# tsnorri/founder-sequences

Hardware: AMD Instinct MI355X
Metric: alignment cells/s (m*n/T) through pBWT+DP (higher is better)
Workload: dtype u32

## Files before the change

### founder-sequences_amd/__init__.py

```python
import ctypes as C
import os

import numpy as np

_HERE = os.path.dirname(os.path.abspath(__file__))
LIB_PATH = os.path.join(_HERE, "libfseq_hip.so")

FSEQ_OK, FSEQ_E_ARG, FSEQ_E_NO_REDUCTION, FSEQ_E_HIP, FSEQ_E_OOM, FSEQ_E_UNSUPPORTED = range(6)


class FseqError(RuntimeError):
    def __init__(self, code, msg):
        super().__init__("fseq error %d: %s" % (code, msg))
        self.code = code


class NoReduction(FseqError):
    """generate_context.cc:192-200: max segment size equals the number of input sequences."""


class Params(C.Structure):
    _fields_ = [("m", C.c_uint32), ("n", C.c_uint64), ("segment_length", C.c_uint64),
                ("pbwt_sample_rate", C.c_uint64), ("block_len", C.c_uint32), ("list_cap", C.c_uint32),
                ("device", C.c_int32)]
# ... 103 lines not shown
                ("junctions_linked", C.c_uint64), ("junctions_novel", C.c_uint64), ("walks", C.c_uint64), ("rows_on_graph", C.c_uint64),
                ("mismatches", C.c_uint64), ("ms_device", C.c_double)]


class GraphNearestInfo(C.Structure):
    _fields_ = [("batches", C.c_uint64), ("packed_words", C.c_uint64), ("query_words", C.c_uint64), ("bits", C.c_uint32), ("reserved", C.c_uint32)]


class DpListsInfo(C.Structure):
    _fields_ = [("unproven", C.c_uint32), ("dp_chunks", C.c_uint32), ("dp_sweeps", C.c_uint32), ("launches", C.c_uint32)]


class MergeListsInfo(C.Structure):
    _fields_ = [("overflow", C.c_uint32), ("tau_separate", C.c_uint32), ("threshold_launches", C.c_uint32), ("count_launches", C.c_uint32)]


class LengthScanSummary(C.Structure):
    _fields_ = [("lists_built", C.c_uint32), ("lists_folded", C.c_uint32), ("short_entries", C.c_uint32), ("retries", C.c_uint32),
                ("ms_phase_a", C.c_double), ("ms_phase_b", C.c_double), ("ms_total", C.c_double)]


LENGTH_SCAN_DTYPE = np.dtype([("segment_length", "<u8"), ("max_segment_size", "<u4"), ("short_path", "<u4"), ("lists", "<u4"), ("list_cap", "<u4"),
                              ("dp_chunks", "<u4"), ("reserved", "<u4"), ("ms_device", "<f8")])
SCAN_LISTS_BUILT, SCAN_LISTS_FOLDED, SCAN_LISTS_NONE = 0, 1, 2

JOIN_SCORE_DTYPE = np.dtype([("rb", "<u8"), ("weight", "<u8"), ("supported", "<u4"), ("unsupported", "<u4"), ("gaps", "<u4"), ("rows_through", "<u4")])
JOIN_SCORE_MAX_SLOTS = 4096
JOIN_SCORE_GAP = 0xFFFF

GRAPH_NODE_DTYPE = np.dtype([("lb", "<u8"), ("rb", "<u8"), ("segment", "<u4"), ("cls", "<u4"), ("rep_row", "<u4"), ("rows", "<u4")])
GRAPH_EDGE_DTYPE = np.dtype([("from", "<u4"), ("to", "<u4"), ("rows", "<u4"), ("junction", "<u4")])
GRAPH_PATHS = 1
GRAPH_NONE = 0xFFFFFFFF
GRAPH_THREAD_ROW_DTYPE = np.dtype([("columns_matched", "<u8"), ("longest_walk_columns", "<u8"), ("segments_matched", "<u4"), ("junctions_linked", "<u4"),
                                   ("junctions_novel", "<u4"), ("walks", "<u4"), ("longest_walk_segments", "<u4"), ("reserved", "<u4")])
GRAPH_THREAD_SEGMENT_DTYPE = np.dtype([("matched", "<u4"), ("linked", "<u4"), ("novel", "<u4"), ("reserved", "<u4")])
GRAPH_THREAD_MAX_CLASSES = 4096
GRAPH_NEAREST_ROW_DTYPE = np.dtype([("columns_admitted", "<u8"), ("longest_walk_columns", "<u8"), ("mismatches_admitted", "<u8"), ("mismatches", "<u8"),
                                    ("segments_admitted", "<u4"), ("segments_exact", "<u4"), ("junctions_linked", "<u4"), ("junctions_novel", "<u4"),
                                    ("walks", "<u4"), ("longest_walk_segments", "<u4"), ("max_distance", "<u4"), ("reserved", "<u4")])
GRAPH_NEAREST_SEGMENT_DTYPE = np.dtype([("mismatches", "<u8"), ("admitted", "<u4"), ("exact", "<u4"), ("linked", "<u4"), ("novel", "<u4"),
                                        ("max_distance", "<u4"), ("reserved", "<u4")])
GRAPH_NEAREST_BATCH_BYTES = 256 << 20

MATCH_PIECE_DTYPE = np.dtype([("lb", "<u8"), ("rb", "<u8"), ("row", "<u4"), ("n_founders", "<u4")])
MATCH_MAX_FOUNDERS = 2048

SEGMENT_DTYPE = np.dtype([("lb", "<u8"), ("rb", "<u8"), ("segment_size", "<u4"), ("reserved", "<u4")])
DPARG_DTYPE = np.dtype([("lb", "<u8"), ("rb", "<u8"), ("segment_max_size", "<u4"), ("segment_size", "<u4")])

EXPORTS = [
    "fseq_abi_version", "fseq_strerror", "fseq_create", "fseq_destroy", "fseq_last_error",
    "fseq_set_rows", "fseq_set_matrix", "fseq_set_device_columns", "fseq_generate_synthetic", "fseq_get_matrix",
    "fseq_run_segmentation", "fseq_get_traceback", "fseq_get_segments", "fseq_boundary_state",
    "fseq_short_path_runs", "fseq_join_greedy", "fseq_greedy_match_host", "fseq_write_founders", "fseq_write_founders_device", "fseq_debug_dp", "fseq_debug_block_state", "fseq_debug_column_list", "fseq_get_timings",
    "fseq_rowshard_xbuf_words", "fseq_rowshard_rows", "fseq_rowshard_pbwt",
    "fseq_debug_rmq", "fseq_shard_xbuf_words", "fseq_set_shard", "fseq_shard_columns", "fseq_shard_owner",
    "fseq_set_device_columns_packed", "fseq_debug_dp_schedule", "fseq_run_segmentation_batch", "fseq_join_bipartite", "fseq_join_random", "fseq_bipartite_match_host", "fseq_random_join_host", "fseq_write_segments",
    "fseq_set_progress", "fseq_step_max", "fseq_current_step", "fseq_set_memory_budget", "fseq_write_segments_host", "fseq_get_join_profile", "fseq_debug_set_tuning",
    "fseq_shard_abort", "fseq_debug_dp_owned", "fseq_debug_clock", "fseq_debug_ranges",
    "fseq_set_list_memory", "fseq_debug_list_windows",
    "fseq_match_founders", "fseq_match_founder_rows", "fseq_get_match", "fseq_write_match",
    "fseq_identity_columns", "fseq_create_without_identity_columns", "fseq_get_identity_columns", "fseq_write_identity_columns", "fseq_write_founders_restored", "fseq_match_founders_restored",
    "fseq_input_begin", "fseq_input_chunk_columns", "fseq_input_scan", "fseq_input_columns", "fseq_input_end", "fseq_set_rows_streamed", "fseq_debug_device_bytes", "fseq_debug_packed_columns",
    "fseq_debug_join_path", "fseq_debug_pass2_paths", "fseq_debug_class_columns", "fseq_debug_bipartite_path",
    "fseq_debug_pass2_step", "fseq_debug_chain_launch", "fseq_debug_chain_launch_wg", "fseq_debug_red_plan", "fseq_debug_column_sources", "fseq_debug_red_cls_direct",
    "fseq_write_segments_device", "fseq_random_join_classes_host", "fseq_debug_segments_file", "fseq_debug_random_path",
    "fseq_set_segment_length", "fseq_scan_segment_lengths", "fseq_debug_scan_plan", "fseq_debug_relump_lists",
    "fseq_match_rows", "fseq_debug_match_split",
    "fseq_create_without_rows", "fseq_get_held_out", "fseq_match_held_out", "fseq_debug_held_out_columns", "fseq_debug_row_split_plan",
    "fseq_debug_dp_lists_check", "fseq_debug_dp_on_lists", "fseq_debug_merge_on_lists", "fseq_debug_traceback_parts",
    "fseq_create_without_identity_columns_held", "fseq_match_held_out_restored", "fseq_match_rows_restored", "fseq_get_match_exceptions",
    "fseq_get_segments_restored", "fseq_write_segments_restored", "fseq_debug_restored_bounds",
    "fseq_input_scan_identity", "fseq_input_reduce", "fseq_input_kept_columns", "fseq_input_columns_kept", "fseq_input_end_kept",
    "fseq_set_rows_streamed_without_identity_columns", "fseq_debug_input_kept_range", "fseq_debug_alphabet",
    "fseq_join_score", "fseq_join_score_host", "fseq_debug_join_score_path", "fseq_debug_join_score",
    "fseq_block_graph", "fseq_write_block_graph", "fseq_debug_graph_file",
    "fseq_debug_local_pass",
    "fseq_graph_thread_rows", "fseq_graph_thread_held_out", "fseq_debug_graph_thread",
    "fseq_graph_nearest_rows", "fseq_graph_nearest_held_out", "fseq_debug_graph_nearest_info", "fseq_debug_graph_nearest_plan", "fseq_debug_graph_nearest",
    "fseq_write_block_graph_restored", "fseq_graph_thread_rows_restored", "fseq_graph_thread_held_out_restored",
    "fseq_debug_chain_launch_wg_keys", "fseq_debug_pass2_step_keys",
    "fseq_debug_chain_plan", "fseq_debug_chain_plan_sharded", "fseq_debug_phase_b",
]
DEBUG_EXPORTS = ["fseq_debug_dp", "fseq_debug_dp_owned", "fseq_debug_clock", "fseq_debug_ranges", "fseq_debug_block_state", "fseq_debug_column_list", "fseq_debug_rmq", "fseq_debug_dp_schedule", "fseq_debug_set_tuning",
                 "fseq_debug_list_windows", "fseq_debug_device_bytes", "fseq_debug_packed_columns", "fseq_debug_join_path", "fseq_debug_pass2_paths",
                 "fseq_debug_class_columns", "fseq_debug_bipartite_path", "fseq_debug_pass2_step", "fseq_debug_chain_launch", "fseq_debug_chain_launch_wg", "fseq_debug_red_plan", "fseq_debug_column_sources", "fseq_debug_red_cls_direct",
                 "fseq_debug_segments_file", "fseq_debug_random_path", "fseq_debug_scan_plan", "fseq_debug_relump_lists", "fseq_debug_match_split",
                 "fseq_debug_held_out_columns", "fseq_debug_row_split_plan", "fseq_debug_dp_lists_check", "fseq_debug_dp_on_lists",
                 "fseq_debug_merge_on_lists", "fseq_debug_traceback_parts",
                 "fseq_debug_restored_bounds", "fseq_debug_input_kept_range", "fseq_debug_alphabet",
                 "fseq_debug_join_score_path", "fseq_debug_join_score", "fseq_debug_graph_file", "fseq_debug_local_pass",
                 "fseq_debug_graph_thread", "fseq_debug_graph_nearest_info", "fseq_debug_graph_nearest_plan", "fseq_debug_graph_nearest",
                 "fseq_debug_chain_launch_wg_keys", "fseq_debug_pass2_step_keys",
                 "fseq_debug_chain_plan", "fseq_debug_chain_plan_sharded", "fseq_debug_phase_b"]

FSEQ_E_PEER = 6
P2_RUN_CAP = 8832
CW_RUN_CAP = 16384
STAGE_TRACEBACK, STAGE_MERGE, STAGE_SAMPLES = 0, 1, 2
PROGRESS_FN = C.CFUNCTYPE(None, C.c_void_p, C.c_int, C.c_uint64, C.c_uint64)

JOIN_GREEDY, JOIN_BIPARTITE, JOIN_RANDOM = 0, 1, 2

ALLREDUCE_FN = C.CFUNCTYPE(C.c_int, C.c_void_p, C.c_uint64, C.c_uint64, C.c_int)

_lib = None


def load_library():
    global _lib
    if _lib is not None:
        return _lib
    if not os.path.exists(LIB_PATH):
        raise ImportError("%s is missing: run `python __graft_entry__.py build` (hipcc --offload-arch=gfx950); "
                          "there is no CPU fallback for the segmentation path" % LIB_PATH)
    L = C.CDLL(LIB_PATH)
    vp, u64, sz = C.c_void_p, C.c_uint64, C.c_size_t
    L.fseq_abi_version.restype = C.c_uint32
    L.fseq_strerror.restype = C.c_char_p
    L.fseq_strerror.argtypes = [C.c_int]
    L.fseq_create.argtypes = [C.POINTER(Params), C.POINTER(vp)]
    L.fseq_destroy.argtypes = [vp]
    L.fseq_destroy.restype = None
    L.fseq_last_error.restype = C.c_char_p
    L.fseq_last_error.argtypes = [vp]
    L.fseq_set_rows.argtypes = [vp, C.POINTER(vp)]
    L.fseq_set_matrix.argtypes = [vp, vp, sz, sz]
    L.fseq_set_device_columns.argtypes = [vp, vp, sz, C.c_uint32]
    L.fseq_set_device_columns_packed.argtypes = [vp, vp, sz, C.c_uint32, C.c_uint32]
    L.fseq_generate_synthetic.argtypes = [vp, C.POINTER(SynthSpec)]
    L.fseq_get_matrix.argtypes = [vp, u64, u64, vp, sz, sz]
    L.fseq_run_segmentation.argtypes = [vp, C.POINTER(Result)]
    L.fseq_get_traceback.argtypes = [vp, vp]
    L.fseq_get_segments.argtypes = [vp, vp]
    L.fseq_boundary_state.argtypes = [vp, u64, vp, vp]
    L.fseq_short_path_runs.argtypes = [vp, vp, vp]
    L.fseq_join_greedy.argtypes = [vp, vp]
    L.fseq_greedy_match_host.argtypes = [C.c_uint32, C.c_uint32, u64, vp, vp, vp, vp, vp]
    L.fseq_write_founders.argtypes = [vp, C.POINTER(vp), vp, C.c_char_p]
    L.fseq_write_founders_device.argtypes = [vp, vp, C.c_char_p]
    L.fseq_run_segmentation_batch.argtypes = [vp, sz, vp, vp]
    L.fseq_debug_dp_schedule.argtypes = [u64, u64, u64, vp, vp, vp, vp]
    L.fseq_join_bipartite.argtypes = [vp, vp]
    L.fseq_join_random.argtypes = [vp, C.c_uint32, vp]
    L.fseq_bipartite_match_host.argtypes = [C.c_uint32, C.c_uint32, u64, vp, vp, vp, vp, vp, vp]
    L.fseq_random_join_host.argtypes = [C.c_uint32, C.c_uint32, u64, vp, vp, vp, vp, C.c_uint32, vp]
    L.fseq_write_segments.argtypes = [vp, C.POINTER(vp), C.c_int, C.c_char_p]
    L.fseq_debug_dp.argtypes = [vp, vp, vp, vp]
    L.fseq_debug_block_state.argtypes = [vp, u64, vp, vp]
    L.fseq_debug_column_list.argtypes = [vp, u64, vp, vp, vp, vp, vp]
    L.fseq_get_timings.argtypes = [vp, C.POINTER(Timings)]
    L.fseq_debug_rmq.argtypes = [C.c_int, vp, C.c_uint32, vp, vp, C.c_uint32, vp, vp]
    L.fseq_shard_xbuf_words.restype = u64
    L.fseq_shard_xbuf_words.argtypes = [vp, C.c_uint32]
    L.fseq_set_shard.argtypes = [vp, C.c_uint32, C.c_uint32, vp, u64, ALLREDUCE_FN, vp]
    L.fseq_shard_columns.argtypes = [vp, C.POINTER(u64), C.POINTER(u64)]
    L.fseq_shard_owner.argtypes = [vp, u64, C.POINTER(C.c_uint32)]
    L.fseq_rowshard_xbuf_words.restype = u64
    L.fseq_rowshard_xbuf_words.argtypes = [C.c_uint32, C.c_uint32, C.c_uint32]
    L.fseq_rowshard_rows.argtypes = [C.c_uint32, C.c_uint32, C.c_uint32, C.c_uint32, C.POINTER(C.c_uint32), C.POINTER(C.c_uint32)]
    L.fseq_rowshard_pbwt.argtypes = [vp, vp, vp, C.POINTER(C.c_uint32), C.POINTER(C.c_uint32), C.POINTER(C.c_double), C.POINTER(u64)]
    L.fseq_write_segments_host.argtypes = [vp, C.POINTER(vp), C.c_int, vp, vp, C.c_char_p]
    L.fseq_get_join_profile.argtypes = [vp, C.POINTER(JoinProfile)]
    L.fseq_debug_set_tuning.argtypes = [vp, C.c_char_p, C.c_char_p]
    L.fseq_set_progress.argtypes = [vp, PROGRESS_FN, vp]
    L.fseq_step_max.restype = u64
    L.fseq_step_max.argtypes = [vp]
    L.fseq_current_step.restype = u64
    L.fseq_current_step.argtypes = [vp]
    L.fseq_set_memory_budget.argtypes = [vp, u64]
    L.fseq_set_list_memory.argtypes = [vp, u64]
    L.fseq_debug_list_windows.argtypes = [vp, C.POINTER(u64), C.POINTER(u64), C.POINTER(C.c_uint32), C.POINTER(C.c_uint32)]
    L.fseq_shard_abort.argtypes = [vp, C.c_int]
    L.fseq_debug_dp_owned.argtypes = [vp, C.POINTER(u64), C.POINTER(u64), C.POINTER(C.c_int), C.POINTER(C.c_int)]
    L.fseq_debug_clock.argtypes = [vp, C.POINTER(C.c_double), C.POINTER(C.c_uint32)]
    L.fseq_debug_ranges.argtypes = [C.POINTER(u64), C.POINTER(u64), C.POINTER(C.c_int)]
    L.fseq_match_founders.argtypes = [vp, vp, u64, C.POINTER(MatchSummary)]
    L.fseq_match_founder_rows.argtypes = [vp, C.POINTER(vp), C.c_uint32, u64, C.POINTER(MatchSummary)]
    L.fseq_get_match.argtypes = [vp, vp, vp]
    L.fseq_write_match.argtypes = [vp, C.c_char_p]
    L.fseq_match_rows.argtypes = [vp, vp, C.POINTER(vp), C.c_uint32, C.POINTER(vp), C.c_uint32, u64, C.POINTER(MatchSummary)]
    L.fseq_debug_match_split.argtypes = [vp, C.POINTER(MatchSplitInfo)]
    L.fseq_identity_columns.argtypes = [vp, vp, C.POINTER(IdentitySummary)]
    L.fseq_create_without_identity_columns.argtypes = [vp, C.POINTER(Params), C.POINTER(vp), C.POINTER(IdentitySummary)]
    L.fseq_get_identity_columns.argtypes = [vp, vp, vp]
    L.fseq_write_identity_columns.argtypes = [vp, C.c_char_p]
    L.fseq_write_founders_restored.argtypes = [vp, vp, C.c_char_p]
    L.fseq_match_founders_restored.argtypes = [vp, vp, u64, C.POINTER(MatchSummary)]
    L.fseq_input_begin.argtypes = [vp, vp, C.c_uint32, u64]
    L.fseq_input_chunk_columns.restype = u64
    L.fseq_input_chunk_columns.argtypes = [vp]
    L.fseq_input_scan.argtypes = [vp, u64, u64, C.POINTER(vp)]
    L.fseq_input_columns.argtypes = [vp, u64, u64, C.POINTER(vp)]
    L.fseq_input_end.argtypes = [vp]
    L.fseq_set_rows_streamed.argtypes = [vp, C.POINTER(vp), u64]
    L.fseq_debug_device_bytes.argtypes = [vp, C.POINTER(u64), C.POINTER(u64), C.c_int]
    L.fseq_debug_packed_columns.argtypes = [vp, u64, u64, vp, C.POINTER(u64), C.POINTER(C.c_uint32)]
    L.fseq_debug_join_path.argtypes = [vp, C.POINTER(C.c_int)]
    L.fseq_debug_bipartite_path.argtypes = [vp, C.POINTER(C.c_int)]
    L.fseq_debug_pass2_paths.argtypes = [vp] + [C.POINTER(C.c_uint32)] * 4 + [vp]
    L.fseq_debug_class_columns.argtypes = [vp, C.POINTER(C.c_uint32), C.POINTER(C.c_uint32), C.c_uint32, C.POINTER(C.c_uint32), C.POINTER(C.c_uint32), C.POINTER(u64), vp, u64]
    L.fseq_debug_column_sources.argtypes = [vp, C.POINTER(C.c_uint32), C.POINTER(C.c_uint32), C.c_uint32, C.POINTER(C.c_uint32)]
    L.fseq_debug_red_cls_direct.argtypes = [C.c_uint32, C.c_uint32, C.c_uint32, u64, C.c_uint32, C.c_uint32, C.c_uint32, C.POINTER(u64), C.POINTER(u64), C.POINTER(C.c_int)]
    L.fseq_debug_pass2_step.argtypes = [C.c_int, C.c_uint32, C.c_uint32, vp, vp, vp, C.c_uint32, C.c_uint32, vp, vp, vp, vp, C.c_uint32, C.c_uint32, vp, vp, vp]
    L.fseq_debug_chain_launch.argtypes = [C.c_int, C.c_uint32, C.c_uint32, C.c_uint32, u64, vp, vp, vp, C.c_uint32, C.c_uint32, vp, vp, vp, vp, vp, vp, vp]
    L.fseq_debug_chain_launch_wg.argtypes = [C.c_int, C.c_uint32, C.c_uint32, C.c_uint32, u64, vp, vp, vp, C.c_uint32, C.c_uint32, vp, vp, C.c_uint32, C.c_uint32, vp, vp, vp, vp, vp, vp]
    L.fseq_debug_chain_launch_wg_keys.argtypes = L.fseq_debug_chain_launch_wg.argtypes + [vp, vp]
    L.fseq_debug_pass2_step_keys.argtypes = [C.c_int, C.c_uint32, C.c_uint32, vp, vp, vp, C.c_uint32, C.c_uint32, vp, vp, vp, vp, C.c_uint32, C.c_uint32, vp, vp, vp, vp, vp, vp]
    L.fseq_debug_red_plan.argtypes = [C.c_uint32, C.c_uint32, C.c_uint32, C.c_int, C.c_uint32, C.c_uint32, C.c_uint32, vp, vp, C.c_int, C.c_int] + [vp] * 11
    L.fseq_write_segments_device.argtypes = [vp, C.c_int, C.c_char_p]
    L.fseq_random_join_classes_host.argtypes = [C.c_uint32, C.c_uint32, u64, vp, vp, vp, C.c_uint32, vp]
    L.fseq_debug_segments_file.argtypes = [vp] + [C.POINTER(u64)] * 4
    L.fseq_debug_random_path.argtypes = [vp, C.POINTER(C.c_int)]
    L.fseq_set_segment_length.argtypes = [vp, u64]
    L.fseq_scan_segment_lengths.argtypes = [vp, vp, sz, C.POINTER(LengthScanSummary)]
    L.fseq_debug_scan_plan.argtypes = [u64, vp, C.c_uint32, vp, C.POINTER(C.c_uint32), vp, C.POINTER(C.c_uint32)]
    L.fseq_debug_relump_lists.argtypes = [C.c_int, u64, C.c_uint32, C.c_uint32, u64, u64, vp, vp]
    L.fseq_create_without_rows.argtypes = [vp, vp, C.c_uint32, C.POINTER(Params), C.POINTER(vp), C.POINTER(HoldOutSummary)]
    L.fseq_get_held_out.argtypes = [vp, vp, vp]
    L.fseq_match_held_out.argtypes = [vp, vp, C.POINTER(vp), C.c_uint32, u64, C.POINTER(MatchSummary)]
    L.fseq_create_without_identity_columns_held.argtypes = [vp, C.POINTER(Params), C.POINTER(vp), C.POINTER(IdentitySummary)]
    L.fseq_match_held_out_restored.argtypes = [vp, vp, u64, C.POINTER(MatchSummary)]
    L.fseq_match_rows_restored.argtypes = [vp, vp, C.POINTER(vp), C.c_uint32, u64, C.POINTER(MatchSummary)]
    L.fseq_get_match_exceptions.argtypes = [vp, vp, vp, C.POINTER(u64)]
    L.fseq_debug_held_out_columns.argtypes = [vp, u64, u64, vp, C.POINTER(u64), C.POINTER(C.c_uint32)]
    L.fseq_debug_row_split_plan.argtypes = [C.c_uint32, C.c_uint32, vp, C.c_uint32, vp, vp, vp, C.POINTER(C.c_uint32), C.POINTER(C.c_uint32)]
    L.fseq_debug_dp_lists_check.argtypes = [C.c_uint32, u64, u64, C.c_uint32, vp, vp, C.POINTER(u64), C.POINTER(C.c_uint32)]
    L.fseq_debug_dp_on_lists.argtypes = [vp, C.c_uint32, vp, vp, vp, C.c_uint32, vp, vp, vp, C.POINTER(DpListsInfo)]
    L.fseq_debug_merge_on_lists.argtypes = [vp, C.c_uint32, vp, vp, vp, vp, vp, C.c_uint32, vp, C.c_uint32, vp, C.POINTER(u64), vp, C.POINTER(u64), vp,
                                            C.POINTER(u64), C.POINTER(MergeListsInfo)]
    L.fseq_debug_traceback_parts.argtypes = [C.c_int, u64, u64, vp, vp, vp, vp, C.c_uint32, vp, vp, C.POINTER(u64), vp, vp, C.POINTER(u64)]
    L.fseq_debug_local_pass.argtypes = [C.c_int, C.c_uint32, C.c_uint32, vp, vp, vp, vp]
    L.fseq_get_segments_restored.argtypes = [vp, vp]
    L.fseq_write_segments_restored.argtypes = [vp, C.c_int, C.c_char_p]
    L.fseq_debug_restored_bounds.argtypes = [vp, u64, u64, vp, vp, u64, vp, vp]
    L.fseq_input_scan_identity.argtypes = [vp, u64, u64, C.POINTER(vp)]
    L.fseq_input_reduce.argtypes = [vp, C.POINTER(Params), C.POINTER(IdentitySummary)]
    L.fseq_input_kept_columns.argtypes = [vp, u64, u64, C.POINTER(u64)]
    L.fseq_input_columns_kept.argtypes = [vp, u64, u64, C.POINTER(vp)]
    L.fseq_input_end_kept.argtypes = [vp, C.POINTER(vp)]
    L.fseq_set_rows_streamed_without_identity_columns.argtypes = [vp, C.POINTER(vp), u64, C.POINTER(Params), C.POINTER(vp), C.POINTER(IdentitySummary)]
    L.fseq_debug_alphabet.argtypes = [vp, C.POINTER(C.c_uint32), C.POINTER(C.c_uint32), vp]
    L.fseq_debug_input_kept_range.argtypes = [vp, u64, u64, u64, C.POINTER(u64), C.POINTER(u64)]
    L.fseq_join_score.argtypes = [vp, vp, vp, vp, vp, C.POINTER(JoinScoreSummary)]
    L.fseq_join_score_host.argtypes = [C.c_uint32, C.c_uint32, u64, vp, vp, vp, vp, vp, vp, vp, vp, C.POINTER(JoinScoreSummary)]
    L.fseq_debug_join_score_path.argtypes = [vp, C.POINTER(C.c_int)]
    L.fseq_debug_join_score.argtypes = [C.c_int, C.c_uint32, C.c_uint32, C.c_uint32, vp, vp, vp, vp, vp, vp, C.POINTER(JoinScoreSummary)]
    L.fseq_block_graph.argtypes = [vp, vp, vp, vp, C.POINTER(GraphSummary)]
    L.fseq_write_block_graph.argtypes = [vp, C.c_uint32, C.c_int, C.c_char_p]
    L.fseq_debug_graph_file.argtypes = [vp, C.POINTER(GraphFileStats)]
    L.fseq_graph_thread_rows.argtypes = [vp, C.POINTER(vp), C.c_uint32, vp, vp, vp, vp, C.POINTER(GraphThreadSummary)]
    L.fseq_graph_thread_held_out.argtypes = [vp, vp, vp, vp, vp, C.POINTER(GraphThreadSummary)]
    L.fseq_debug_graph_thread.argtypes = [vp, C.POINTER(GraphThreadInfo)]
    L.fseq_graph_nearest_rows.argtypes = [vp, C.POINTER(vp), C.c_uint32, C.c_uint32, vp, vp, vp, vp, vp, vp, C.POINTER(GraphNearestSummary)]
    L.fseq_graph_nearest_held_out.argtypes = [vp, C.c_uint32, vp, vp, vp, vp, vp, vp, C.POINTER(GraphNearestSummary)]
    L.fseq_debug_graph_nearest_info.argtypes = [vp, C.POINTER(GraphNearestInfo)]
    L.fseq_debug_graph_nearest_plan.argtypes = [vp, vp, vp, u64, C.c_uint32, u64, vp, vp, C.POINTER(u64)]
    L.fseq_debug_graph_nearest.argtypes = [C.c_int, vp, u64, C.c_uint32, u64, C.c_uint32, vp, vp, vp, vp, C.c_uint32, C.c_uint32, vp, u64, C.c_uint32,
                                           C.c_uint32, C.c_uint32, u64, vp, vp, vp, C.POINTER(GraphNearestInfo)]
    L.fseq_debug_chain_plan.argtypes = [C.c_uint32, C.c_int, C.c_uint32, C.c_uint32, C.c_int, C.c_uint32, u64, C.c_uint32, C.POINTER(ChainPlan)]
    L.fseq_debug_chain_plan_sharded.argtypes = [C.c_uint32, C.c_uint32, C.c_uint32, C.c_uint32, C.c_int, C.c_uint32, C.c_int, u64, C.c_uint32, C.POINTER(ChainPlan)]
    L.fseq_debug_phase_b.argtypes = [vp, C.POINTER(PhaseBInfo)]
    L.fseq_write_block_graph_restored.argtypes = [vp, C.c_uint32, C.c_int, C.c_char_p]
    L.fseq_graph_thread_rows_restored.argtypes = [vp, C.POINTER(vp), C.c_uint32, vp, vp, vp, vp, C.POINTER(GraphThreadSummary)]
    L.fseq_graph_thread_held_out_restored.argtypes = [vp, vp, vp, vp, vp, C.POINTER(GraphThreadSummary)]
    _lib = L
    return L


def synth_threshold(mu):
    if mu <= 0.0:
        return 0
    if mu >= 1.0:
        return 0xFFFFFFFFFFFFFFFF
    return int(mu * 18446744073709551616.0)


def greedy_match_host(m, max_segment_size, lb, rb, a, d):
    L = load_library()
    lb = np.ascontiguousarray(lb, dtype=np.uint64)
    rb = np.ascontiguousarray(rb, dtype=np.uint64)
    a = np.ascontiguousarray(a, dtype=np.uint32)
    d = np.ascontiguousarray(d, dtype=np.uint32)
# ... 1188 lines not shown
        f, w = C.c_int(), C.c_int()
        self._check(self.L.fseq_debug_dp_owned(self.h, C.byref(a), C.byref(b), C.byref(f), C.byref(w)))
        return a.value, b.value, bool(f.value), bool(w.value)

    def debug_clock(self):
        g, n = C.c_double(), C.c_uint32()
        self._check(self.L.fseq_debug_clock(self.h, C.byref(g), C.byref(n)))
        return g.value, n.value

    def debug_block_state(self, b):
        a = np.zeros(self.m, dtype=np.uint32)
        d = np.zeros(self.m, dtype=np.uint32)
        self._check(self.L.fseq_debug_block_state(self.h, b, a.ctypes.data, d.ctypes.data))
        return a, d

    def debug_column_list(self, col):
        cap = self.m + 2
        v = np.zeros(cap, dtype=np.uint32)
        c = np.zeros(cap, dtype=np.uint32)
        ne, c0, comp = C.c_uint32(), C.c_uint32(), C.c_uint32()
        self._check(self.L.fseq_debug_column_list(self.h, col, v.ctypes.data, c.ctypes.data,
                                                  C.byref(ne), C.byref(c0), C.byref(comp)))
        return v[:ne.value].copy(), c[:ne.value].copy(), c0.value, bool(comp.value)

    def debug_dp_on_lists(self, list_cap, ent, hdr, cuts=()):
        ent, hdr = _dp_lists(ent, hdr)
        if ent.shape[0] != self.n or ent.shape[1] != ((int(list_cap) + 3) & ~1):
            raise FseqError(FSEQ_E_ARG, "DP on lists: ent is [n][(list_cap + 3) & ~1][2]")
        cuts = np.ascontiguousarray(cuts, dtype=np.uint32)
        k = self.n - self.segment_length + 1
        lb, mx, sz = (np.zeros(k, dtype=np.uint32) for _ in range(3))
        info = DpListsInfo()
        self.result = None
        self._check(self.L.fseq_debug_dp_on_lists(self.h, int(list_cap), ent.ctypes.data, hdr.ctypes.data, cuts.ctypes.data if len(cuts) else None,
                                                  len(cuts), lb.ctypes.data, mx.ctypes.data, sz.ctypes.data, C.byref(info)))
        return lb, mx, sz, {k_: getattr(info, k_) for k_, _ in DpListsInfo._fields_}

    def debug_merge_on_lists(self, list_cap, ent, hdr, lb, max_size, size, separate=False, col_splits=()):
        ent, hdr = _dp_lists(ent, hdr)
        if ent.shape[0] != self.n or ent.shape[1] != ((int(list_cap) + 3) & ~1):
            raise FseqError(FSEQ_E_ARG, "merge on lists: ent is [n][(list_cap + 3) & ~1][2]")
        lb, max_size, size = _dp_arrays(self.n, self.segment_length, lb, max_size, size)
        splits = np.ascontiguousarray(col_splits, dtype=np.uint64)
        room = self.n // self.segment_length + 2
        tb = np.zeros(room, dtype=DPARG_DTYPE)
        tau = np.zeros((room, 2), dtype=np.uint32)
        seg = np.zeros(room, dtype=SEGMENT_DTYPE)
        n_tb, n_tau, n_seg = C.c_uint64(), C.c_uint64(), C.c_uint64()
        info = MergeListsInfo()
        self.result = None
        self._check(self.L.fseq_debug_merge_on_lists(self.h, int(list_cap), ent.ctypes.data, hdr.ctypes.data, lb.ctypes.data, max_size.ctypes.data,
                                                     size.ctypes.data, 1 if separate else 0, splits.ctypes.data if len(splits) else None, len(splits),
                                                     tb.ctypes.data, C.byref(n_tb), tau.ctypes.data, C.byref(n_tau), seg.ctypes.data, C.byref(n_seg),
                                                     C.byref(info)))
        return (tb[:n_tb.value].copy(), tau[:n_tau.value].copy(), seg[:n_seg.value].copy(),
                {k_: getattr(info, k_) for k_, _ in MergeListsInfo._fields_})

    def set_tuning(self, name, value="1"):
        self._check(self.L.fseq_debug_set_tuning(self.h, name.encode(), None if value is None else str(value).encode()))

    def join_profile(self):
        jp = JoinProfile()
        self._check(self.L.fseq_get_join_profile(self.h, C.byref(jp)))
        return {k: getattr(jp, k) for k, _ in JoinProfile._fields_}

    def join_path(self):
        path = C.c_int()
        self._check(self.L.fseq_debug_join_path(self.h, C.byref(path)))
        return path.value

    def bipartite_path(self):
        path = C.c_int()
        self._check(self.L.fseq_debug_bipartite_path(self.h, C.byref(path)))
        return path.value

    def pass2_paths(self):
        v = [C.c_uint32() for _ in range(4)]
        hist = np.zeros(19, dtype=np.uint32)
        self._check(self.L.fseq_debug_pass2_paths(self.h, *[C.byref(x) for x in v], hist.ctypes.data))
        out = dict(zip(("by_runs", "by_sort", "copies", "max_runs"), (x.value for x in v)))
        out["runs_hist"] = [int(x) for x in hist]
        return out

    def phase_b(self):
        info = PhaseBInfo()
        self._check(self.L.fseq_debug_phase_b(self.h, C.byref(info)))
        out = {f: int(getattr(info, f)) for f in ("cus", "nblocks", "fan", "resident", "fit", "p2_groups", "p2_groups_took_keys", "p2_groups_gathered")}
        out["hand_armed"], out["stats_kept"] = bool(info.hand_armed), bool(info.stats_kept)
        out["launches"] = _chain_launches(info.launches, info.n_launches)
        s = [int(x) for x in info.cw_stats]
        out["cw_stats"] = dict(by_runs=s[0], by_sort=s[1], from_identity=s[2], max_runs=s[3], runs_hist=s[4:]) if info.stats_kept else None
        return out

    def class_column_sources(self):
        a, b = C.c_uint32(), C.c_uint32()
        self._check(self.L.fseq_debug_class_columns(self.h, C.byref(a), C.byref(b), 0xFFFFFFFF, None, None, None, None, 0))
        return {"from_classes": a.value, "from_alignment": b.value}

    def column_sources(self, block=None):
        a, b, s = C.c_uint32(), C.c_uint32(), C.c_uint32()
        self._check(self.L.fseq_debug_column_sources(self.h, C.byref(a), C.byref(b), 0xFFFFFFFF if block is None else block, C.byref(s)))
        out = {"staged": a.value, "gathered": b.value}
        if block is not None:
            out["block_staged"] = bool(s.value)
        return out

    def class_columns(self, block):
        have, nkeys, ldc = C.c_uint32(), C.c_uint32(), C.c_uint64()
        self._check(self.L.fseq_debug_class_columns(self.h, None, None, block, C.byref(have), C.byref(nkeys), C.byref(ldc), None, 0))
        if not have.value:
            return None, ldc.value, nkeys.value
        t = self.timings()
        cols = min(t["block_len"], self.n - block * t["block_len"])
        out = np.zeros((cols, ldc.value), dtype=np.uint8)
        self._check(self.L.fseq_debug_class_columns(self.h, None, None, block, C.byref(have), C.byref(nkeys), C.byref(ldc), out.ctypes.data, out.nbytes))
        return out, ldc.value, nkeys.value

    def timings(self):
        t = Timings()
        self._check(self.L.fseq_get_timings(self.h, C.byref(t)))
        return {k: getattr(t, k) for k, _ in Timings._fields_}
```

### founder-sequences_amd/csrc/fseq_ctx.hpp

```cpp
#pragma once

#include "../../include/fseq.h"
#include "../../include/fseq_debug.h"
#include "fseq_types.hpp"
#include "fseq_chainplan.hpp"

#include <hip/hip_runtime.h>

#include <algorithm>
#include <array>
#include <atomic>
#include <chrono>
#include <climits>
#include <cmath>
#include <cstdio>
#include <cstring>
#include <string>
#include <thread>
#include <unordered_map>
#include <vector>

namespace fseq {

struct KernelSet {
	uint32_t T, E, sigma, cap;
	size_t lds_colblock, lds_snap;
	uint32_t scan_shift;
	void (*rank)(hipStream_t st, uint32_t grid, size_t lds, PhaseAArgs const &keys);
	void (*snap)(hipStream_t st, uint32_t grid, size_t lds, SnapArgs const &tasks);
	size_t (*columns_lds)(uint32_t B);
	void (*columns)(hipStream_t st, uint32_t grid, size_t lds, ColumnsArgs const &cols);
	uint32_t (*columns_resident)(size_t lds);
	size_t lds_chain;
	void (*chain)(hipStream_t st, uint32_t grid, size_t lds, ChainMultiArgs const &chains, uint32_t keyed);
	hipError_t (*prepare)();
	hipError_t (*prepare_columns)(size_t lds_columns);
};

template <typename K>
inline hipError_t allow_lds(K kernel, size_t bytes)
{
	if (bytes <= 64 * 1024) return hipSuccess;
	return hipFuncSetAttribute(reinterpret_cast<void const *>(kernel), hipFuncAttributeMaxDynamicSharedMemorySize, (int) bytes);
}

struct Stream2Config { uint32_t T, E, key_shift; size_t (*lds)(uint32_t colbytes); hipError_t (*prepare)(size_t lds);
	void (*launch)(hipStream_t st, uint32_t grid, size_t lds, ColumnsArgs const &cols);
	uint32_t (*resident)(size_t lds);
	void (*launch_snap)(hipStream_t st, uint32_t grid, size_t lds, SnapArgs const &tasks); };
struct ReducedSet {
	uint32_t T, E, rows, values;
	bool pk, ew;
	size_t (*lds)(uint32_t B, uint32_t symcap);
	hipError_t (*prepare)(size_t lds);
	void (*launch)(hipStream_t st, uint32_t grid, size_t lds, ColumnsArgs const &cols, RedArgs const &red);
	uint32_t (*resident)(size_t lds);
};
int reduced_config_count();
bool reduced_config(int index, ReducedSet *out);
struct ChainSnapSet {
	size_t lds;
	hipError_t (*prepare)();
	void (*launch)(hipStream_t st, uint32_t grid, size_t lds, SnapArgs const &tasks, RedArgs const &red);
};
bool select_chain_snap(uint32_t T, uint32_t E, ChainSnapSet *out);

bool select_kernels(uint32_t m, uint32_t sigma, KernelSet *out);
Stream2Config stream2_config();
void launch_blockkeys(hipStream_t st, uint32_t grid, size_t lds, PhaseAArgs const &keys);
hipError_t prepare_blockkeys(uint32_t T, size_t lds, bool debug);
uint32_t blocktrie_threads(uint32_t m, bool stream);
size_t blocktrie_lds(uint32_t T);
hipError_t launch_blocktrie(hipStream_t st, uint32_t groups, PhaseAArgs const &keys);
hipError_t launch_reduce_prep(hipStream_t, uint32_t grid, RedPrepArgs const &);
void launch_reduce_check(hipStream_t, uint32_t const *cnt, uint32_t const *planned, uint32_t count, uint32_t *flags);
void launch_reduce_msa(hipStream_t st, MsaArgs const &A, ReducedMsaArgs const &red, bool gather_only);
bool launch_reduce_cls(hipStream_t st, MsaArgs const &A, ReducedMsaArgs const &red, ClassColumnArgs const &classes);

inline double now_ms()
{
	using namespace std::chrono;
	return duration<double, std::milli>(steady_clock::now().time_since_epoch()).count();
}


}

struct Tuning {
	bool debug = false;
	bool dp_serial = false;
	int  dp_spec_win = 0, dp_spec_rounds = 0, dp_spec_max_sweeps = 0;
	bool stream_plain_scan = false;
	bool plain_scan = false;
	bool occurrence_keys = false;
	bool phase_a_classic = false;
	int  chain_fan = 0;
	bool blockkeys_wide = false;
	bool blockkeys_single = false;
	bool no_dense_columns = false;
	bool no_blocktrie = false;
	bool blocktrie_always = false;
	int  blockkeys_cap = 0;
	bool ss_unpacked = false;
	bool ss_absolute = false;
	bool poison_lists = false;
	bool join_host = false;
	bool join_wide = false;
	bool join_bip_wide = false;
	int  join_bip_slabs = 0;
	int  segfile_batch = 0;
	int  graph_batch = 0;
	bool shard_dp_full = false;
	int  shard_dp_window = 0;
	int  inject_failure_rank = -1;
	std::string sync_phases;
	bool check_phase_a = false;
	bool no_reduced = false;
	int  reduced_margin = -1;
	bool reduced_always = false;
	bool reduced_msa_gather = false;
	int  reduced_cap = 0;
	bool class_gather = false;
	int  class_columns = 1;
	int  p2_run_cap = -1;
	int  chain_run_cap = -1;
	int  p2_keys = 0;
	int  chain_wg = 0;
	bool scan_rebuild = false;
	int  match_split = 0;
	int  match_overlap = 0;
	int  match_stage = 0;
	int  graph_thread_key_bits = 0;
	int  graph_nearest_batch = 0;

	struct Knob {
		char const *name;
		bool Tuning::*flag;
		int Tuning::*num;
		int lo, off;
		std::string Tuning::*str;
	};
	static std::vector<Knob> const &knobs()
	{
		static std::vector<Knob> const table = {
			{"FSEQ_DEBUG", &Tuning::debug, nullptr, 0, 0, nullptr},
			{"FSEQ_DP_SERIAL", &Tuning::dp_serial, nullptr, 0, 0, nullptr},
			{"FSEQ_DP_SPEC_WIN", nullptr, &Tuning::dp_spec_win, 1, 0, nullptr},
			{"FSEQ_DP_SPEC_ROUNDS", nullptr, &Tuning::dp_spec_rounds, 1, 0, nullptr},
			{"FSEQ_DP_SPEC_MAX_SWEEPS", nullptr, &Tuning::dp_spec_max_sweeps, 1, 0, nullptr},
			{"FSEQ_STREAM_PLAIN_SCAN", &Tuning::stream_plain_scan, nullptr, 0, 0, nullptr},
			{"FSEQ_PLAIN_SCAN", &Tuning::plain_scan, nullptr, 0, 0, nullptr},
			{"FSEQ_OCCURRENCE_KEYS", &Tuning::occurrence_keys, nullptr, 0, 0, nullptr},
			{"FSEQ_PHASE_A_CLASSIC", &Tuning::phase_a_classic, nullptr, 0, 0, nullptr},
			{"FSEQ_CHAIN_FAN", nullptr, &Tuning::chain_fan, 2, 0, nullptr},
			{"FSEQ_BLOCKKEYS_WIDE", &Tuning::blockkeys_wide, nullptr, 0, 0, nullptr},
			{"FSEQ_BLOCKKEYS_SINGLE", &Tuning::blockkeys_single, nullptr, 0, 0, nullptr},
			{"FSEQ_NO_DENSE_COLUMNS", &Tuning::no_dense_columns, nullptr, 0, 0, nullptr},
			{"FSEQ_NO_BLOCKTRIE", &Tuning::no_blocktrie, nullptr, 0, 0, nullptr},
			{"FSEQ_BLOCKTRIE_ALWAYS", &Tuning::blocktrie_always, nullptr, 0, 0, nullptr},
			{"FSEQ_BLOCKKEYS_CAP", nullptr, &Tuning::blockkeys_cap, 2048, 0, nullptr},
			{"FSEQ_SS_UNPACKED", &Tuning::ss_unpacked, nullptr, 0, 0, nullptr},
			{"FSEQ_SS_ABSOLUTE", &Tuning::ss_absolute, nullptr, 0, 0, nullptr},
			{"FSEQ_POISON_LISTS", &Tuning::poison_lists, nullptr, 0, 0, nullptr},
			{"FSEQ_JOIN_HOST", &Tuning::join_host, nullptr, 0, 0, nullptr},
			{"FSEQ_JOIN_WIDE", &Tuning::join_wide, nullptr, 0, 0, nullptr},
			{"FSEQ_JOIN_BIP_WIDE", &Tuning::join_bip_wide, nullptr, 0, 0, nullptr},
			{"FSEQ_JOIN_BIP_SLABS", nullptr, &Tuning::join_bip_slabs, 1, 0, nullptr},
			{"FSEQ_SEGFILE_BATCH", nullptr, &Tuning::segfile_batch, 1, 0, nullptr},
			{"FSEQ_GRAPH_BATCH", nullptr, &Tuning::graph_batch, 1, 0, nullptr},
			{"FSEQ_SHARD_DP_FULL", &Tuning::shard_dp_full, nullptr, 0, 0, nullptr},
			{"FSEQ_SHARD_DP_WINDOW", nullptr, &Tuning::shard_dp_window, 64, 0, nullptr},
			{"FSEQ_INJECT_FAILURE_RANK", nullptr, &Tuning::inject_failure_rank, INT_MIN, -1, nullptr},
			{"FSEQ_SYNC_PHASES", nullptr, nullptr, 0, 0, &Tuning::sync_phases},
			{"FSEQ_CHECK_PHASE_A", &Tuning::check_phase_a, nullptr, 0, 0, nullptr},
			{"FSEQ_NO_REDUCED", &Tuning::no_reduced, nullptr, 0, 0, nullptr},
			{"FSEQ_REDUCED_MARGIN", nullptr, &Tuning::reduced_margin, 0, -1, nullptr},
			{"FSEQ_REDUCED_ALWAYS", &Tuning::reduced_always, nullptr, 0, 0, nullptr},
			{"FSEQ_REDUCED_MSA_GATHER", &Tuning::reduced_msa_gather, nullptr, 0, 0, nullptr},
			{"FSEQ_REDUCED_CAP", nullptr, &Tuning::reduced_cap, 1, 0, nullptr},
			{"FSEQ_P2_RUN_CAP", nullptr, &Tuning::p2_run_cap, 0, -1, nullptr},
			{"FSEQ_CHAIN_RUN_CAP", nullptr, &Tuning::chain_run_cap, 0, -1, nullptr},
			{"FSEQ_CHAIN_WG", nullptr, &Tuning::chain_wg, 0, 0, nullptr},
			{"FSEQ_P2_KEYS", nullptr, &Tuning::p2_keys, 0, 0, nullptr},
			{"FSEQ_CLASS_COLUMNS", nullptr, &Tuning::class_columns, 0, 1, nullptr},
			{"FSEQ_CLASS_GATHER", &Tuning::class_gather, nullptr, 0, 0, nullptr},
			{"FSEQ_SCAN_REBUILD", &Tuning::scan_rebuild, nullptr, 0, 0, nullptr},
			{"FSEQ_MATCH_SPLIT", nullptr, &Tuning::match_split, 1, 0, nullptr},
			{"FSEQ_MATCH_OVERLAP", nullptr, &Tuning::match_overlap, 1, 0, nullptr},
			{"FSEQ_MATCH_STAGE_BYTES", nullptr, &Tuning::match_stage, 64, 0, nullptr},
			{"FSEQ_GRAPH_THREAD_KEY_BITS", nullptr, &Tuning::graph_thread_key_bits, 1, 0, nullptr},
			{"FSEQ_GRAPH_NEAREST_BATCH", nullptr, &Tuning::graph_nearest_batch, 1, 0, nullptr},
		};
		return table;
	}

	void apply(Knob const &k, char const *value)
	{
		bool const on = value != nullptr;
		if (k.flag) this->*k.flag = on;
		else if (k.num) this->*k.num = on ? std::max(k.lo, atoi(value)) : k.off;
		else this->*k.str = on ? value : "";
	}

	bool set(char const *name, char const *value)
	{
		for (Knob const &k : knobs())
			if (!strcmp(k.name, name)) { apply(k, value); return true; }
		return false;
	}

	void from_environment()
	{
		for (Knob const &k : knobs())
			if (char const *v = getenv(k.name)) apply(k, v);
	}
};

struct fseq_ctx;

namespace fseq {

template <typename T>
struct DevBuf {
	T *base = nullptr;
	size_t cap = 0;
	ptrdiff_t shift = 0;
	operator T *() const { return base ? reinterpret_cast<T *>(reinterpret_cast<char *>(base) - shift) : nullptr; }
	template <typename U> U *as() const { return reinterpret_cast<U *>(static_cast<T *>(*this)); }
	void rebase(ptrdiff_t elements) { shift = elements * (ptrdiff_t) sizeof(T); }
	int alloc(fseq_ctx *c, size_t count);
	bool try_alloc(fseq_ctx *c, size_t count);
	int ensure(fseq_ctx *c, size_t count) { return cap >= count ? FSEQ_OK : alloc(c, count); }
	int alloc_range(fseq_ctx *c, size_t lo, size_t hi, size_t per)
	{
		int const rc = alloc(c, (hi > lo ? hi - lo : 0) * per);
		rebase((ptrdiff_t) (lo * per));
		return rc;
	}
	void release(fseq_ctx *c);
};

template <typename T>
struct DevTemp : DevBuf<T> {
	fseq_ctx *const c;
	explicit DevTemp(fseq_ctx *c_) : c(c_) {}
	DevTemp(DevTemp const &) = delete;
	~DevTemp() { this->release(c); }
	int alloc(size_t count) { return DevBuf<T>::alloc(c, count); }
};

template <typename... B>
inline void release_all(fseq_ctx *c, B &...bufs) { (bufs.release(c), ...); }

}

struct Shard {
	bool on = false;
	uint32_t rank = 0, world = 1;
	uint32_t *xbuf = nullptr;
	uint64_t xwords = 0;
	fseq_allreduce_fn fn = nullptr;
	void *user = nullptr;
// ... 83 lines not shown
	DevBuf<uint32_t> d_bstate_a, d_bstate_d;
	DevBuf<uint32_t> d_cshist;
	int dev_cus = -1;
	int cw_resident = 0;
	DevBuf<uint16_t> d_p2keys;
	DevBuf<uint32_t> d_p2keys_flag;
	bool p2keys_live = false;
	uint32_t p2_hand[2]{};
	DevBuf<uint32_t> d_cw_stats;
	std::vector<fseq::ChainLaunch> pb_launches;
	uint32_t pb_cw_stats[fseq::CW_STATS]{};
	bool pb_cw_stats_have = false;
	bool pb_hand = false;
	uint64_t pb_fit = 0;
	uint32_t p2_groups = 0;
	DevBuf<uint32_t> d_hrank, d_hkeyd, d_hnkeys, d_hstate_a, d_hstate_d;
	struct ChainLevel { uint32_t count = 0; uint64_t cols = 0; DevBuf<uint32_t> rank, keyd, nkeys, state_a, state_d; };
	std::vector<ChainLevel> levels;
	uint32_t chain_fan = 0;
	uint32_t shard_k = 0, shard_q = 0;
	uint32_t chain_G = 0, n_super = 0;
	uint32_t chain_G2 = 0, n_hyper = 0;
	DevBuf<uint2> d_ent;
	DevBuf<uint4> d_hdr;
	uint32_t X = 0, stride = 0;
	uint32_t X_hint = 0;
	struct Dp {
		DevBuf<uint32_t> M, LB, SZ, Tb, Tbv;
		DevBuf<unsigned long long> K;
		uint32_t tstride = 0;
		operator fseq::DpArrays() const { return fseq::DpArrays{M, LB, SZ, Tb, Tbv, K, tstride}; }
	} dp;
	DevBuf<uint32_t> d_Mprev;
	DevBuf<uint32_t> d_spec;
	DevBuf<fseq::PathWords> d_flags;
	DevBuf<uint32_t> d_recent;
	uint64_t dp_size = 0;
	DevBuf<uint64_t> d_cols;
	DevBuf<uint2> d_grp;
	DevBuf<uint64_t> d_src;
	uint32_t snap_stride = 16;
	DevBuf<uint32_t> d_ss_a, d_ss_d;
	uint32_t ss_pack = 0;
	bool ss_ids = false;
	DevBuf<uint32_t> d_bs_w;
	DevBuf<uint8_t> d_bs_h;
	DevBuf<uint32_t> d_wgblk;
	DevBuf<uint2> d_wggrp;
	DevBuf<uint32_t> d_snap_a, d_snap_d;

	DevBuf<uint32_t> d_red_cnt, d_red_vmin, d_red_rows, d_red_leaf, d_red_a, d_red_d;
	DevBuf<uint32_t> d_red_invalid, d_red_blocks;
	uint32_t red_cap = 0;
	DevBuf<uint8_t> d_red_msa;
	size_t red_ld = 0;
	DevBuf<uint8_t> d_cls;
	DevBuf<uint32_t> d_cls_have;
	size_t cls_ld = 0;
	bool cls_on = false;
	bool cls_every = false;
	bool cls_read = false;
	DevBuf<uint32_t> d_red_src;
	bool cls_staged = false;
	struct Red {
		fseq::RedPlan plan;
		std::vector<uint8_t> cls_config;
		struct Memory {
			std::vector<uint8_t> force;
			bool plan_holds = false;
			uint32_t plan_X = 0;
			bool declined = false;
			uint32_t declined_X = 0;
			bool cls_unread = false;
			void forget_plan() { plan_holds = false; }
			void forget_verdicts() { plan_holds = false; declined = false; cls_unread = false; }
			void forget_input() { forget_verdicts(); force.clear(); }
		} memory;
	} red;
	bool red_active = false;
	DevBuf<uint32_t> d_red_cls, d_red_headd, d_red_ncls, d_red_taskblk, d_red_wgtasks;
	DevBuf<uint32_t> d_red_p2grp;
	uint32_t p2_stats[fseq::P2_STATS]{};
	bool p2_stats_have = false;
	DevBuf<uint32_t> d_red_ss_a, d_red_ss_d;
	uint32_t red_ss_stride = 0, red_ss_cap = 0;
	uint32_t *h_red_pin = nullptr;
	size_t red_pin_words = 0;
	bool red_direct = false;
	DevBuf<uint32_t> d_red_cnt_plan;
	hipStream_t red_st[2]{};
	struct RedEvents {
		hipEvent_t fork = nullptr;
		hipEvent_t join_stream2 = nullptr, join_side0 = nullptr, join_side1 = nullptr;
		std::array<hipEvent_t *, 3> joins() { return {&join_stream2, &join_side0, &join_side1}; }
		std::array<hipEvent_t *, 4> all() { return {&fork, &join_stream2, &join_side0, &join_side1}; }
	} red_ev;
	uint8_t *h_red_pin2 = nullptr;
	size_t red_pin2_bytes = 0;

	bool have_result = false;
	bool scan_lists = false;
	fseq_result res{};
	DevBuf<uint4> d_tb;
	std::vector<fseq_dp_arg> traceback;
	std::vector<fseq_segment> segments;
	std::vector<uint32_t> sp_first, sp_len;
	fseq_timings tm{};
	struct PathEvents {
		hipEvent_t a_begin = nullptr, a_end_b_begin = nullptr, b_end = nullptr;
		hipEvent_t c_begin = nullptr, c_end = nullptr, dp_begin = nullptr, dp_end = nullptr;
		hipEvent_t pass2_begin = nullptr, pass2_end = nullptr;
		hipEvent_t dp_reset = nullptr;
		std::array<hipEvent_t *, 9> timed() { return {&a_begin, &a_end_b_begin, &b_end, &c_begin, &c_end, &dp_begin, &dp_end, &pass2_begin, &pass2_end}; }
	} ev;
	hipStream_t stream2 = nullptr;
	uint8_t *h_pin = nullptr;
	size_t pin_cap = 0, pin_used = 0;

	struct Match {
		DevBuf<uint8_t> fcols;
		DevBuf<uint32_t> cnt;
		DevBuf<uint64_t> off;
		DevBuf<fseq_match_piece> pieces;
		DevBuf<uint32_t> sets;
		DevBuf<uint8_t> qrows;
		DevBuf<uint32_t> split;
		DevBuf<uint64_t> exc_off;
		DevBuf<uint32_t> exc_cols;
		uint64_t exc_total = 0;
		int exc_from = 0;
		uint32_t exc_rows = 0;
		bool have = false;
		fseq_match_summary sum{};
		fseq_match_split_info split_info{};
		hipEvent_t ev[4]{};
	} match;
	void free_match()
	{
		fseq::release_all(this, match.fcols, match.cnt, match.off, match.pieces, match.sets, match.qrows, match.split, match.exc_off, match.exc_cols);
		for (auto &e : match.ev) if (e) { (void) hipEventDestroy(e); e = nullptr; }
		match.have = false;
		match.exc_from = 0;
	}

	struct Identity {
		bool have = false;
		uint64_t n_src = 0, identity = 0;
		DevBuf<uint8_t> mask;
		DevBuf<uint32_t> kept;
		DevBuf<uint8_t> ref;
	} idn;
	void free_identity()
	{
		fseq::release_all(this, idn.mask, idn.kept, idn.ref);
		idn.have = false;
	}

	struct HeldOut {
		bool have = false;
		uint32_t m_src = 0, n_held = 0;
		size_t ld = 0;
		DevBuf<uint8_t> cols;
		std::vector<uint32_t> kept_rows, held_rows;
		bool have_exc = false;
		DevBuf<uint64_t> exc_off;
		DevBuf<uint32_t> exc_cols;
		uint64_t exc_total = 0;
// ... 144 lines not shown
```

### founder-sequences_amd/csrc/fseq_kernels.hpp

```cpp
#pragma once

#include "fseq_core.hpp"
#include "fseq_types.hpp"

#include <type_traits>

namespace fseq {

constexpr uint32_t PAD_KEY = 0xFFFFFFFFu;

struct Carver {
	char *p;
	template <typename U> __device__ __host__ U *take(size_t n)
	{
		U *r = reinterpret_cast<U *>(p);
		p += (n * sizeof(U) + 15) & ~size_t(15);
		return r;
	}
};

__host__ __device__ inline size_t carve_bytes(size_t n, size_t elem) { return (n * elem + 15) & ~size_t(15); }

struct SynthArgs {
	uint64_t seed;
// ... 537 lines not shown
		uint32_t total;
		uint32_t r = block_excl_add<T>(nf, sscr, &total);
		size_t const ob = (size_t) grp * m;
#pragma unroll
		for (int e = 0; e < E; ++e)
		{
			uint32_t const pos = p0 + e;
			if (pos < m)
			{
				bool const first = (pos == 0 || d[e] > kstart);
				r += first ? 1u : 0u;
				out_rank[ob + a[e]] = r - 1u;
				if (first) out_keyd[ob + r - 1u] = d[e];
			}
		}
		if (tid == 0) out_nkeys[grp] = total;
	}
}

#ifndef FSEQ_PW_MAX_E
#define FSEQ_PW_MAX_E 8
#endif
__host__ __device__ constexpr bool columns_pairwise(int T, int E, int SIGMA, bool PK = false)
{
	if (PK && T == 512 && E == 15) return false;
	return SIGMA == 4 && ((E >= 2 && E <= FSEQ_PW_MAX_E && !(T >= 1024 && E >= 7 && !PK)) || (PK && E >= 9 && T * E <= 10240));
}

__host__ __device__ constexpr bool columns_packed(int T, int E, int SIGMA, bool PK)
{
	if (!PK && T >= 1024 && E == 7) return false;
	return SIGMA == 4 && !columns_pairwise(T, E, SIGMA, PK);
}

__host__ __device__ constexpr bool columns_lookup(int T, int E, int SIGMA, bool PK) { return columns_pairwise(T, E, SIGMA, PK) || (SIGMA == 4 && PK && T * E <= 10240); }
__host__ __device__ constexpr size_t columns_run_words(int T, int E, int SIGMA, bool PK) { return (columns_pairwise(T, E, SIGMA, PK) || (PK && T == 512 && E == 15)) ? 5 * (size_t) T : columns_lookup(T, E, SIGMA, PK) ? 4 * (size_t) T : 0; }

constexpr int SLIM_T = 512, SLIM_E = 15, SLIM_VALUES = 4096;
__host__ __device__ constexpr bool columns_slim(int T, int E, bool PK) { return PK && T == SLIM_T && E == SLIM_E; }
__host__ __device__ constexpr size_t columns_value_cap(int T, int E, bool PK) { return columns_slim(T, E, PK) ? (size_t) SLIM_VALUES : (size_t) T * E; }
__host__ __device__ constexpr int columns_min_waves(int T, int E, bool PK) { return columns_slim(T, E, PK) ? 4 : (PK && T == 512) ? 6 : 4; }

template <int T, int E, int SIGMA, bool PK>
__host__ __device__ inline size_t columns_lds_bytes(uint32_t B)
{
	constexpr size_t CAP = (size_t) T * E, VCAP = columns_value_cap(T, E, PK);
	return 2 * carve_bytes(CAP, PK ? 2 : 4) + 2 * carve_bytes(CAP, 1) + carve_bytes(PK ? (VCAP + B + 9) / 2 : VCAP + B + 8, 4) + carve_bytes(VCAP, 4)
	     + carve_bytes(1, sizeof(StepScratch<T, SIGMA>)) + carve_bytes(T / WAVE + 1, 4) + (columns_run_words(T, E, SIGMA, PK) ? carve_bytes(columns_run_words(T, E, SIGMA, PK), 4) : 0);
}

template <bool PK> __device__ __forceinline__ uint32_t cnt_get(uint32_t const *cnt_l, uint32_t i)
{
	return PK ? ((cnt_l[i >> 1] >> ((i & 1u) * 16u)) & 0xFFFFu) : cnt_l[i];
}
template <bool PK> __device__ __forceinline__ void cnt_inc(uint32_t *cnt_l, uint32_t i)
{
	if (PK) atomicAdd(&cnt_l[i >> 1], 1u << ((i & 1u) * 16u)); else atomicAdd(&cnt_l[i], 1u);
}
template <bool PK> __device__ __forceinline__ void cnt_dec(uint32_t *cnt_l, uint32_t i)
{
	if (PK) atomicSub(&cnt_l[i >> 1], 1u << ((i & 1u) * 16u)); else atomicSub(&cnt_l[i], 1u);
}

template <int T>
__device__ __forceinline__ void bitonic_sort_lds(uint32_t *sb, uint32_t N2)
{
	for (uint32_t k = 2; k <= N2; k <<= 1)
	{
		for (uint32_t j = k >> 1, lj = (uint32_t) __builtin_ctz(k) - 1u; j > 0; j >>= 1, --lj)
		{
			for (uint32_t i = threadIdx.x; i < N2 / 2; i += T)
			{
				uint32_t const lo = ((i >> lj) << (lj + 1u)) | (i & (j - 1u));
				uint32_t const hi = lo + j;
				bool const asc = (lo & k) == 0;
				uint32_t const x = sb[lo], y = sb[hi];
				if ((x > y) == asc) { sb[lo] = y; sb[hi] = x; }
			}
			__syncthreads();
		}
	}
}

template <int T, int E, int SIGMA, bool PK, bool EW, bool DENSE, bool RED>
__device__ __forceinline__ void columns_body(char *smem,
	uint8_t const *__restrict__ msa, size_t ld, uint32_t m, uint64_t n, uint32_t B, uint32_t N2,
	uint32_t const *__restrict__ bstate_a, uint32_t const *__restrict__ bstate_d,
	uint32_t L, uint32_t X, uint32_t stride, uint2 *__restrict__ ent, uint4 *__restrict__ hdr, uint32_t npass, uint32_t bsh,
	uint32_t snap_stride, uint32_t *__restrict__ ss_a, uint32_t *__restrict__ ss_d, uint32_t block0,
	uint32_t *done_host, uint32_t epoch, uint32_t const *__restrict__ colmask, RedArgs const &red, uint32_t const *__restrict__ blocklist = nullptr)
{
	FSEQ_CLOCK_STAMP(blockIdx.x, 0);
	constexpr uint32_t CAP = T * E, VCAP = (uint32_t) columns_value_cap(T, E, PK);
	static_assert(VCAP == CAP || RED, "a value table smaller than the rows: the reduced kernel, which can refuse a block");
	uint32_t const blk = RED ? red.blocks[blockIdx.x] : (blocklist ? blocklist[blockIdx.x] : blockIdx.x + block0);
	uint32_t red_vmin = 0, red_deficit = 0, t_first = 0, t_count = 0, t_next = 0;
	bool const red_snap = RED && red.cls != nullptr;
	if constexpr (RED)
	{
		m = red.cnt[blk];
		if (m == RED_NONE || m > (EW ? (uint32_t) (T - 64) * E : CAP)) return;
		red_vmin = red.vmin[blk];
		red_deficit = red.m_true - m;
		N2 = 2; while (N2 < m + 1u) N2 <<= 1;
		if (red_snap) { t_first = red.wg_tasks[3u * blockIdx.x]; t_count = red.wg_tasks[3u * blockIdx.x + 1u]; }
	}
	bool const red_exact = RED && red_vmin <= 1u;
	bool red_cls = false;
	uint32_t red_nkeys = 0;
	if constexpr (RED)
	{
		if (red.cls_have != nullptr) red_cls = __builtin_amdgcn_readfirstlane(red.cls_src[blk] & red.cls_have[blk]) != 0u;
		if (red_cls) red_nkeys = __builtin_amdgcn_readfirstlane(red.nkeys[blk]);
	}
	using AT = std::conditional_t<PK, uint16_t, uint32_t>;
	Carver cv{smem};
	AT *a_l = cv.take<AT>(CAP);
	AT *d_l = cv.take<AT>(CAP);
	uint8_t *sym0 = cv.take<uint8_t>(RED ? red.symcap : CAP);
	uint8_t *sym1 = cv.take<uint8_t>(RED ? red.symcap : CAP);
	uint32_t *cnt_l = cv.take<uint32_t>(PK ? (VCAP + B + 9) / 2 : VCAP + B + 8);
	uint32_t *V_l = cv.take<uint32_t>(VCAP);
	StepScratch<T, SIGMA> &scr = *cv.take<StepScratch<T, SIGMA>>(1);
	uint32_t *sscr = cv.take<uint32_t>(T / WAVE + 1);
	constexpr bool PW = columns_pairwise(T, E, SIGMA, PK);
	constexpr bool LU = columns_lookup(T, E, SIGMA, PK);
	constexpr bool PL = columns_packed(T, E, SIGMA, PK);
	uint32_t *runs = LU ? cv.take<uint32_t>(columns_run_words(T, E, SIGMA, PK)) : nullptr;
	uint32_t const tid = threadIdx.x;
	uint32_t const p0 = EW ? (tid >= 64u ? (tid - 64u) * E : 0x7FFF0000u) : tid * E;
	bool const rows = !EW || tid >= 64u;
	uint64_t const kblk = (uint64_t) blk * B;
	uint64_t const k0 = red_snap ? (uint64_t) red.wg_tasks[3u * blockIdx.x + 2u] : kblk;
	uint64_t const kend = red_snap ? (uint64_t) red.task_rb[t_first + t_count - 1u] : ((k0 + B < n) ? k0 + B : n);
	uint32_t const nb = (uint32_t) (kend - k0);

	uint32_t a[E], d[E];
	{
		bool const from_ss = RED && k0 != kblk;
		size_t const ob = from_ss ? (size_t) (k0 / red.ss_stride) * red.ss_cap : RED ? (size_t) blk * red.cap : (size_t) blk * m;
		uint32_t const *const sa = from_ss ? red.ss_a : RED ? red.a : bstate_a, *const sd = from_ss ? red.ss_d : RED ? red.d : bstate_d;
#pragma unroll
		for (int e = 0; e < E; ++e)
		{
			uint32_t const pos = p0 + e;
			a[e] = pos < m ? sa[ob + pos] : 0u;
			d[e] = pos < m ? sd[ob + pos] : 0u;
		}
	}

	uint32_t *sb = reinterpret_cast<uint32_t *>(a_l);
	uint32_t D0 = 0;
	bool have_values = false;
	if constexpr (RED)
	{
		uint32_t &hash_fail = scr.has[0];
		uint32_t const avail = (uint32_t) ((reinterpret_cast<char *>(V_l) - reinterpret_cast<char *>(sb)) / 4);
		uint32_t NT = N2;
		while (NT > avail) NT >>= 1;
		uint32_t const hshift = 32u - (uint32_t) __builtin_ctz(NT);
		for (uint32_t i = tid; i < NT; i += T) sb[i] = PAD_KEY;
		if (tid == 0) hash_fail = 0u;
		__syncthreads();
		auto insert = [&](uint32_t v) {
			uint32_t h = (v * 2654435761u) >> hshift;
			for (uint32_t probes = 0; probes < 64u; ++probes)
			{
				uint32_t const old = atomicCAS(&sb[h], PAD_KEY, v);
				if (old == PAD_KEY || old == v) return;
				h = (h + 1u) & (NT - 1u);
			}
			hash_fail = 1u;
		};
#pragma unroll
		for (int e = 0; e < E; ++e)
			if (p0 + e < m) insert(d[e]);
		if (red_exact && tid == 0) insert(0u);
		__syncthreads();
		if (hash_fail == 0u)
		{
			uint32_t const per = (NT + T - 1) / T, start = tid * per;
			uint32_t mine = 0;
			for (uint32_t q = 0; q < per; ++q) mine += (start + q < NT && sb[start + q] != PAD_KEY) ? 1u : 0u;
			uint32_t w = block_excl_add<T>(mine, sscr, &D0);
			uint32_t N2s = 2;
			while (N2s < D0) N2s <<= 1;
			if (N2s <= VCAP)
			{
				for (uint32_t q = 0; q < per; ++q)
					if (start + q < NT && sb[start + q] != PAD_KEY) V_l[w++] = sb[start + q];
				for (uint32_t i = D0 + tid; i < N2s; i += T) V_l[i] = PAD_KEY;
				__syncthreads();
				bitonic_sort_lds<T>(V_l, N2s);
				have_values = true;
			}
		}
		__syncthreads();
		if constexpr (VCAP < CAP)
		{
			if (!have_values)
			{
				if (tid == 0) { red.invalid[blk] = RED_WIDE; red.any_invalid[0] = 1u; }
				return;
			}
		}
	}
	if (!have_values)
	{
	for (uint32_t i = tid; i < N2; i += T) sb[i] = PAD_KEY;
	__syncthreads();
#pragma unroll
	for (int e = 0; e < E; ++e)
		if (p0 + e < m) sb[p0 + e] = d[e];
	if (RED && red_exact && tid == 0) sb[m] = 0u;
	__syncthreads();
	bitonic_sort_lds<T>(sb, N2);
	{
		uint32_t const per = (N2 + T - 1) / T;
		uint32_t const start = tid * per;
		uint32_t nflag = 0;
		for (uint32_t q = 0; q < per; ++q)
		{
			uint32_t const i = start + q;
			if (i < N2)
			{
				uint32_t const v = sb[i];
				nflag += (v != PAD_KEY && (i == 0 || v != sb[i - 1])) ? 1u : 0u;
			}
		}
		uint32_t w = block_excl_add<T>(nflag, sscr, &D0);
		for (uint32_t q = 0; q < per; ++q)
		{
			uint32_t const i = start + q;
			if (i < N2)
			{
				uint32_t const v = sb[i];
				if (v != PAD_KEY && (i == 0 || v != sb[i - 1])) V_l[w++] = v;
			}
		}
	}
	}
	__syncthreads();
	for (uint32_t i = tid; i < (PK ? (D0 + nb + 9u) / 2u : D0 + nb + 8u); i += T) cnt_l[i] = 0;
	__syncthreads();

	uint32_t id[E];
#pragma unroll
	for (int e = 0; e < E; ++e)
	{
		id[e] = 0;
		if (p0 + e < m)
		{
			uint32_t lo = 0, hi = D0;
			uint32_t const key = d[e];
			while (lo < hi)
			{
				uint32_t const mid = (lo + hi) >> 1;
				if (V_l[mid] < key) lo = mid + 1; else hi = mid;
			}
			id[e] = lo;
			cnt_inc<PK>(cnt_l, lo);
		}
	}
#pragma unroll
	for (int e = 0; e < E; ++e)
		if (rows) { a_l[p0 + e] = (AT) a[e]; d_l[p0 + e] = (AT) id[e]; }

	bool const has_chunk = !RED && tid * 16u < sym_bytes(m, bsh);
	uint4 nxt = make_uint4(0, 0, 0, 0);
	if (nb && has_chunk)
	{
		nxt = *reinterpret_cast<uint4 const *>(msa + k0 * ld + tid * 16u);
		*reinterpret_cast<uint4 *>(sym0 + tid * 16u) = nxt;
	}
	uint32_t const red_colbytes = RED ? (red.direct ? red.colbytes : red_cls ? min((uint32_t) red.cls_ld, (sym_bytes(red_nkeys, bsh) + 15u) & ~15u) : sym_bytes(m, bsh)) : 0u;
	uint8_t const *const red_msa = red_cls ? red.cls_msa : msa;
	size_t const red_ld = red_cls ? red.cls_ld : ld;
	auto red_stage = [&](uint64_t k, uint8_t *dstb) {
		uint8_t const *const col = red_msa + k * red_ld;
		for (uint32_t cb = 0; cb < red_colbytes; cb += (uint32_t) T * 16u)
		{
			uint32_t const off = cb + tid * 16u;
			if (cb + wave_id() * 1024u < red_colbytes)
				lds_dma16(col + (off < red_colbytes ? off : 0u), __builtin_amdgcn_readfirstlane((uint32_t) (uintptr_t) (dstb + cb + wave_id() * 1024u)));
		}
	};
	if (RED && nb) { red_stage(k0, sym0); asm volatile("s_waitcnt vmcnt(0)" ::: "memory"); }
	if (RED && red_cls && k0 == kblk)
	{
		__syncthreads();
		uint32_t const *const leaf = red.leaf + (size_t) blk * red.cap;
		for (uint32_t idx = tid; idx < m; idx += T) a_l[idx] = (AT) leaf[a_l[idx]];
	}
	__syncthreads();

	bool const zero_present = (V_l[0] == 0u);
	constexpr bool CARRY_OK = PK && E >= 9 && !columns_slim(T, E, PK);
	bool const carry = CARRY_OK && npass == 2u && bsh == 1u && ((RED && red.direct) ? red.m_true : red_cls ? red_nkeys : m) <= 16384u;
#ifdef FSEQ_KC_STAMPS
	long long kc_work = 0, kc_wait = 0, kc_last = clock64();
	KcStamps kcs{{0, 0, 0, 0, 0, 0, 0, 0}, clock64()};
#endif

	for (uint32_t j = 0; j < nb; ++j)
	{
		uint8_t const *symc = (j & 1u) ? sym1 : sym0;
		uint8_t *symn = (j & 1u) ? sym0 : sym1;
		bool const more = j + 1 < nb;
		if (more && has_chunk)
			nxt = *reinterpret_cast<uint4 const *>(msa + (k0 + j + 1) * ld + tid * 16u);
		if (RED && more) red_stage(k0 + j + 1, symn);
		bool dense = false;
		uint32_t remap = 0;
		if (DENSE && colmask && npass == 2u && bsh == 1u)
		{
			uint32_t const pm = __builtin_amdgcn_readfirstlane(colmask[k0 + j]);
			if (__popc(pm) <= 4)
			{
				dense = true;
				uint32_t idx = 0;
#pragma unroll
				for (uint32_t cde = 0; cde < 16; ++cde) { remap |= (idx & 3u) << (2u * cde); idx += (pm >> cde) & 1u; }
			}
		}

		for (uint32_t pass = 0; pass < npass; ++pass)
		{
			bool const last_pass = (DENSE && dense) || pass + 1 == npass;
			uint32_t s[E], dst[E], dnew[E], hi[CARRY_OK ? E : 1];
			if (rows) read_chunk<T, E>(a_l, d_l, a, d, p0);
			if (carry && pass == 0)
			{
#pragma unroll
				for (int e = 0; e < E; ++e)
				{
					uint32_t const sy = (symc[a[e] >> 1] >> ((a[e] & 1u) * 4u)) & 15u;
					s[e] = (p0 + e < m) ? ((DENSE && dense) ? ((remap >> (2u * sy)) & 3u) : (sy & 3u)) : (uint32_t) SIGMA;
					hi[e] = (DENSE && dense) ? 0u : (sy >> 2);
				}
			}
			else if (DENSE && dense)
			{
#pragma unroll
				for (int e = 0; e < E; ++e)
				{
					uint32_t const sy = (symc[a[e] >> 1] >> ((a[e] & 1u) * 4u)) & 15u;
					s[e] = (p0 + e < m) ? ((remap >> (2u * sy)) & 3u) : (uint32_t) SIGMA;
					if (CARRY_OK) hi[e] = 0;
				}
			}
			else if (carry)
			{
#pragma unroll
				for (int e = 0; e < E; ++e)
				{
					s[e] = (p0 + e < m) ? (a[e] >> 14) : (uint32_t) SIGMA;
					a[e] &= 0x3FFFu;
					hi[e] = 0;
				}
			}
			else
			{
#pragma unroll
				for (int e = 0; e < E; ++e) { s[e] = (p0 + e < m) ? sym_digit(symc, a[e], bsh, pass) : (uint32_t) SIGMA; if (CARRY_OK) hi[e] = 0; }
			}

#ifdef FSEQ_KC_STAMPS
			kcs.last = clock64();
			partition_step<T, E, SIGMA, false, EW, 16, PW, LU, false, PL>(d, s, D0 + j, scr, dst, dnew, nullptr, runs, &kcs);
#else
			partition_step<T, E, SIGMA, false, EW, 16, PW, LU, false, PL>(d, s, D0 + j, scr, dst, dnew, nullptr, runs);
#endif

#pragma unroll
			for (int e = 0; e < E; ++e)
			{
				if (p0 + e < m)
				{
					a_l[dst[e]] = (AT) (CARRY_OK ? (a[e] | (hi[CARRY_OK ? e : 0] << 14)) : a[e]);
					d_l[dst[e]] = (AT) dnew[e];
					if (dnew[e] != d[e])
					{
						cnt_dec<PK>(cnt_l, d[e]);
						cnt_inc<PK>(cnt_l, dnew[e]);
					}
				}
			}
			if (last_pass && more && has_chunk)
				*reinterpret_cast<uint4 *>(symn + tid * 16u) = nxt;
			if (RED && last_pass && more) asm volatile("s_waitcnt vmcnt(0)" ::: "memory");
#ifdef FSEQ_KC_STAMPS
			{ long long const t_ = clock64(); kc_work += t_ - kc_last; kc_last = t_; }
			__syncthreads();
			{ long long const t_ = clock64(); kc_wait += t_ - kc_last; kc_last = t_; }
#else
			__syncthreads();
#endif
			if (DENSE && dense) break;
		}

		if (ss_a && (k0 + j + 1) % snap_stride == 0)
		{
			size_t const ob = (size_t) ((k0 + j + 1) / snap_stride) * m;
#pragma unroll
			for (int i = 0; i < E; ++i)
			{
				uint32_t idx = tid + i * T;
				asm volatile("" : "+v"(idx));
				if (idx < m)
				{
					uint32_t const vid = d_l[idx];
					ss_a[ob + idx] = a_l[idx];
					ss_d[ob + idx] = vid < D0 ? V_l[vid] : (uint32_t) (k0 + (vid - D0) + 1u);
				}
			}
		}

		if (RED && !red_snap && red.ss_a && (k0 + j + 1u) % red.ss_stride == 0u && j + 1u < nb)
		{
			size_t const ob = (size_t) ((k0 + j + 1u) / red.ss_stride) * red.ss_cap;
			for (uint32_t idx = tid; idx < m; idx += T)
			{
				uint32_t const vid = d_l[idx];
				red.ss_a[ob + idx] = a_l[idx];
				red.ss_d[ob + idx] = vid < D0 ? V_l[vid] : (uint32_t) (k0 + (vid - D0) + 1u);
			}
		}
		if (RED && red_snap)
		{
			if (t_next < t_count && red.task_rb[t_first + t_next] == k0 + j + 1u)
			{
				uint32_t const task = t_first + t_next;
				uint32_t id_in = D0;
				if (k0 != kblk)
				{
					uint32_t lo = 0, hi = D0;
					while (lo < hi) { uint32_t const mid = (lo + hi) >> 1; if (V_l[mid] <= (uint32_t) kblk) lo = mid + 1; else hi = mid; }
					id_in = lo;
				}
				uint32_t nf = 0;
				if (rows)
				{
#pragma unroll
					for (int e = 0; e < E; ++e) nf += (p0 + e < m && (uint32_t) d_l[p0 + e] >= id_in) ? 1u : 0u;
				}
				uint32_t total;
				uint32_t r = block_excl_add<T>(nf, sscr, &total);
				size_t const ot = (size_t) task * red.cap;
				uint32_t const *const key_of = red.direct ? red.rank + (size_t) blk * red.m_true : red.leaf + (size_t) blk * red.cap;
				if (rows)
				{
#pragma unroll
					for (int e = 0; e < E; ++e)
					{
						uint32_t const pos = p0 + e;
						if (pos < m)
						{
							uint32_t const vid = d_l[pos];
							bool const first = vid >= id_in;
							r += first ? 1u : 0u;
							uint32_t lf = a_l[pos];
							if (!red_cls) lf = key_of[lf];
							red.cls[ot + lf] = r - 1u;
							if (first) red.headd[ot + r - 1u] = vid < D0 ? V_l[vid] : (uint32_t) (k0 + (vid - D0) + 1u);
						}
					}
				}
				if (tid == 0) red.ncls[task] = total;
				++t_next;
			}
			continue;
		}

		if (wave_id() == 0)
		{
			__builtin_amdgcn_s_setprio(3);
#ifdef FSEQ_KC_STAMPS
			long long const kc_l0 = clock64();
#endif
			uint32_t const lane = lane_id();
			uint64_t const k = k0 + j;
			uint32_t const thr = (k + 2 > (uint64_t) L) ? (uint32_t) (k + 2 - L) : 0u;
			uint2 *out = ent + k * (size_t) stride;
			constexpr int IPL = (RED && T >= 256) ? 8 : 4;
			int32_t const top = (int32_t) (D0 + j);
			uint32_t cumN = 0, nent = 1, R = 0;
			int32_t const id_lo = (RED && red_exact) ? 1 : 0;
			bool red_stopped = false, red_bad = false;
			for (int32_t base = top | (IPL - 1); base >= id_lo; base -= 64 * IPL)
			{
				uint32_t c[IPL], v[IPL];
				uint32_t lane_c = 0, lane_o = 0, lane_rc = 0;
				bool cand[IPL];
#ifdef FSEQ_KC_STAMPS
				kcs.acc[4] += 1;
#endif
				int32_t const hi = base - IPL * (int32_t) lane;
				int32_t const lo = hi - (IPL - 1);
				uint32_t cw[IPL], vw[IPL];
#pragma unroll
				for (int q = 0; q < IPL; ++q) { cw[q] = 0; vw[q] = 0; }
				if (hi >= 0)
				{
					if constexpr (PK)
					{
						uint32_t w[IPL / 2];
						lds_read_words<IPL / 2>(cnt_l + ((uint32_t) lo >> 1), w);
#pragma unroll
						for (int q = 0; q < IPL; ++q) cw[q] = (q & 1) ? (w[q >> 1] >> 16) : (w[q >> 1] & 0xFFFFu);
					}
					else
						lds_read_words<IPL>(cnt_l + lo, cw);
					if ((uint32_t) lo < D0) lds_read_words<IPL>(V_l + lo, vw);
				}
#pragma unroll
				for (int q = 0; q < IPL; ++q)
				{
					int32_t const i = hi - q;
					c[q] = (i >= id_lo) ? cw[IPL - 1 - q] : 0u;
					v[q] = (i < 0) ? 0u : (((uint32_t) i < D0) ? vw[IPL - 1 - q] : (uint32_t) (k0 + ((uint32_t) i - D0) + 1u));
					bool const nz = c[q] > 0;
					bool const rec = nz && v[q] >= thr;
					cand[q] = nz && !rec;
					lane_c += c[q];
					lane_o += cand[q] ? 1u : 0u;
					lane_rc += rec ? c[q] : 0u;
				}
#ifdef FSEQ_KC_STAMPS
				long long const kc_e1 = clock64();
#endif
				uint32_t const inc = wave_incl_add(lane_c | (lane_o << 16));
				uint32_t const r_tot = readlane_u32(wave_incl_add(lane_rc), 63);
				uint32_t const tot_o = readlane_u32(inc, 63) >> 16;
				uint32_t run_c = (inc & 0xFFFFu) - lane_c;
				uint32_t run_o = (inc >> 16) - lane_o;
				uint32_t lastP = 0;
				bool tk[IPL];
#ifdef FSEQ_KC_STAMPS
				long long const kc_e2 = clock64();
#endif
#pragma unroll
				for (int q = 0; q < IPL; ++q)
				{
					uint32_t const excN = cumN + run_c - r_tot;
					tk[q] = cand[q] && excN <= X;
					if (tk[q]) { out[nent + run_o] = make_uint2(v[q], c[q]); lastP = excN + c[q]; }
					if (RED && !red_exact) red_bad = red_bad || (tk[q] && v[q] < red_vmin);
					run_o += cand[q] ? 1u : 0u;
					run_c += c[q];
				}
#ifdef FSEQ_KC_STAMPS
				long long const kc_e3 = clock64();
				kcs.acc[0] += kc_e1 - kc_l0; kcs.acc[1] += kc_e2 - kc_e1; kcs.acc[2] += kc_e3 - kc_e2;
#endif
				uint32_t taken = 0;
#pragma unroll
				for (int q = 0; q < IPL; ++q) taken += (uint32_t) __popcll(__ballot(tk[q]));
				uint32_t mx = lastP;
				mx = max(mx, dpp_mov<DPP_ROW_SHR1, 0xF>(0u, mx));
				mx = max(mx, dpp_mov<DPP_ROW_SHR2, 0xF>(0u, mx));
				mx = max(mx, dpp_mov<DPP_ROW_SHR4, 0xF>(0u, mx));
				mx = max(mx, dpp_mov<DPP_ROW_SHR8, 0xF>(0u, mx));
				mx = max(mx, dpp_mov<DPP_ROW_BCAST15, 0xA>(0u, mx));
				mx = max(mx, dpp_mov<DPP_ROW_BCAST31, 0xC>(0u, mx));
				nent += taken;
				if (taken) cumN = readlane_u32(mx, 63);
				R += r_tot;
				if (taken != tot_o || cumN > X) { red_stopped = true; break; }
			}
			uint32_t cnt0 = zero_present ? cnt_get<PK>(cnt_l, 0u) : 0u;
			if constexpr (RED)
			{
				if (red_exact)
				{
					cnt0 += red_deficit;
					if (!red_stopped && cnt0)
					{
						if (thr == 0u) R += cnt0;
						else { if (lane == 0) out[nent] = make_uint2(0u, cnt0); ++nent; cumN += cnt0; }
					}
				}
				else
				{
					cnt0 = 0;
					if (__ballot(red_bad) != 0ull || (!red_stopped && red_deficit != 0u)) { if (lane == 0) { red.invalid[blk] = 1u; red.any_invalid[0] = 1u; } }
				}
			}
			uint32_t const cum = R + cumN;
			if (lane == 0)
			{
				out[0] = make_uint2((uint32_t) (k + 1), R);
				hdr[k] = make_uint4(nent, cnt0, cum == (RED ? red.m_true : m) ? 1u : 0u, cum);
			}
#ifdef FSEQ_KC_STAMPS
			kcs.acc[5] += clock64() - kc_l0;
			kcs.acc[6] += nent;
#endif
			__builtin_amdgcn_s_setprio(0);
		}
	}
#ifdef FSEQ_KC_STAMPS
	if (lane_id() == 0 && (blockIdx.x == 100 || blockIdx.x == 3000))
		printf("kc stamps block %u wave %u: work %lld wait %lld cycles per column (%u columns); step: to barrier 1 %lld, wait %lld, between %lld, wait 1b %lld\n",
		       blockIdx.x, wave_id(), kc_work / nb, kc_wait / nb, nb, kcs.acc[0] / nb, kcs.acc[1] / nb, kcs.acc[2] / nb, kcs.acc[3] / nb);
	if (lane_id() == 0 && wave_id() == 0 && (blockIdx.x == 100 || blockIdx.x == 3000))
		printf("kc stamps block %u list: %lld rounds x 100 per column, %lld cycles per column, %lld entries x 100 per column, X %u D0 %u; (last round, from the list's start) reads %lld scans %lld stores %lld\n", blockIdx.x, kcs.acc[4] * 100 / nb, kcs.acc[5] / nb, kcs.acc[6] * 100 / nb, X, D0, kcs.acc[0] / nb, kcs.acc[1] / nb, kcs.acc[2] / nb);
#endif
	FSEQ_CLOCK_STAMP(blockIdx.x, 1);
	if constexpr (!RED) publish_block_done(done_host, blk, epoch);
}

template <int T, int E, int SIGMA, bool PK, bool EW = false, bool DENSE = false>
__global__ __launch_bounds__(T, (PK && T == 512) ? 6 : 4) void k_columns(
	uint8_t const *__restrict__ msa, size_t ld, uint32_t m, uint64_t n, uint32_t B, uint32_t N2,
	uint32_t const *__restrict__ bstate_a, uint32_t const *__restrict__ bstate_d,
	uint32_t L, uint32_t X, uint32_t stride, uint2 *__restrict__ ent, uint4 *__restrict__ hdr, uint32_t npass, uint32_t bsh,
	uint32_t snap_stride, uint32_t *__restrict__ ss_a, uint32_t *__restrict__ ss_d, uint32_t block0,
	uint32_t *done_host, uint32_t epoch, uint32_t const *__restrict__ colmask = nullptr, uint32_t const *__restrict__ blocklist = nullptr)
{
	extern __shared__ __attribute__((aligned(16))) char smem[];
	columns_body<T, E, SIGMA, PK, EW, DENSE, false>(smem, msa, ld, m, n, B, N2, bstate_a, bstate_d, L, X, stride, ent, hdr, npass, bsh, snap_stride, ss_a, ss_d, block0,
	                                                 done_host, epoch, colmask, RedArgs{}, blocklist);
}

template <int T, int E, int SIGMA, bool PK, bool EW = false>
__global__ __launch_bounds__(T, columns_min_waves(T, E, PK)) void k_columns_red(
	uint8_t const *__restrict__ msa, size_t ld, uint64_t n, uint32_t B,
	uint32_t L, uint32_t X, uint32_t stride, uint2 *__restrict__ ent, uint4 *__restrict__ hdr, uint32_t npass, uint32_t bsh, RedArgs const red)
{
	extern __shared__ __attribute__((aligned(16))) char smem[];
	columns_body<T, E, SIGMA, PK, EW, false, true>(smem, msa, ld, 0u, n, B, 0u, nullptr, nullptr, L, X, stride, ent, hdr, npass, bsh, 0u, nullptr, nullptr, 0u,
	                                                nullptr, 0u, nullptr, red);
}

static __global__ __launch_bounds__(256) void k_boundary_recent(
	uint32_t const *__restrict__ bstate_d, uint32_t m, uint64_t n, uint32_t B, uint32_t L, uint32_t *__restrict__ out, uint32_t block0)
{
	uint64_t k = (uint64_t) (blockIdx.x + block0) * B;
	if (k > n) k = n;
	if (k < L) { if (threadIdx.x == 0) out[blockIdx.x] = 0xFFFFFFFFu; return; }
	uint32_t const thr = (uint32_t) (k - L);
	uint32_t const *d = bstate_d + (size_t) (blockIdx.x + block0) * m;
	uint32_t cnt = 0;
	for (uint32_t i = threadIdx.x; i < m; i += 256) cnt += d[i] > thr ? 1u : 0u;
	__shared__ uint32_t red[4];
	cnt = readlane_u32(wave_incl_add(cnt), 63);
	if (lane_id() == 0) red[wave_id()] = cnt;
	__syncthreads();
	if (threadIdx.x == 0) out[blockIdx.x] = red[0] + red[1] + red[2] + red[3];
}

static __global__ __launch_bounds__(256) void k_any_nonzero(uint32_t const *__restrict__ v, uint32_t count, uint32_t *__restrict__ out)
{
	uint32_t any = 0;
	for (uint32_t i = threadIdx.x; i < count; i += 256u) any |= v[i];
	__shared__ uint32_t red[4];
	bool const some = __ballot(any != 0u) != 0ull;
	if (lane_id() == 0) red[wave_id()] = some ? 1u : 0u;
	__syncthreads();
	if (threadIdx.x == 0) out[0] = red[0] | red[1] | red[2] | red[3];
}

static __global__ __launch_bounds__(64) void k_gather_lists(
	uint64_t const *__restrict__ cols, uint32_t stride, uint2 const *__restrict__ ent, uint4 const *__restrict__ hdr,
	uint2 *__restrict__ out_ent, uint4 *__restrict__ out_hdr)
{
	uint64_t const k = cols[blockIdx.x];
	uint4 const h = hdr[k];
	if (threadIdx.x == 0) out_hdr[blockIdx.x] = h;
	for (uint32_t i = threadIdx.x; i < h.x; i += 64)
		out_ent[(size_t) blockIdx.x * stride + i] = ent[k * (size_t) stride + i];
}

constexpr uint32_t TB_WIN = 8192;
constexpr uint32_t TB_TERM = 0xFFFFFFFFu;

__device__ __forceinline__ uint32_t tb_next(uint32_t lb, uint32_t t, uint32_t L) { return (lb >= L && lb - L < t) ? lb - L : TB_TERM; }

static __global__ __launch_bounds__(256) void k_tb_windows(uint32_t const *__restrict__ LB, uint32_t dp_size, uint32_t L,
                                                    uint32_t *__restrict__ exit_next, uint32_t *__restrict__ exit_cnt,
                                                    uint32_t vlo = 0, uint32_t vhi = 0xFFFFFFFFu)
{
	__shared__ uint32_t nx[2][TB_WIN];
	__shared__ uint16_t cn[2][TB_WIN];
	uint32_t const wbase = blockIdx.x * TB_WIN;
	if (wbase >= vhi || wbase + TB_WIN <= vlo) return;
	uint32_t const base = wbase;
	for (uint32_t i = threadIdx.x; i < TB_WIN; i += 256u)
	{
		uint32_t const t = base + i;
		nx[0][i] = t < dp_size ? tb_next(LB[t], t, L) : TB_TERM;
		cn[0][i] = 1;
	}
	__syncthreads();
	uint32_t const hops = TB_WIN / (L ? L : 1u) + 2u;
	uint32_t cur = 0;
	for (uint32_t span = 1; span < hops; span <<= 1)
	{
		for (uint32_t i = threadIdx.x; i < TB_WIN; i += 256u)
		{
			uint32_t j = nx[cur][i];
			uint32_t c = cn[cur][i];
			if (j != TB_TERM && j >= base && j >= vlo) { c += cn[cur][j - base]; j = nx[cur][j - base]; }
			nx[cur ^ 1u][i] = j;
			cn[cur ^ 1u][i] = (uint16_t) c;
		}
		cur ^= 1u;
		__syncthreads();
	}
	for (uint32_t i = threadIdx.x; i < TB_WIN; i += 256u)
		if (base + i < dp_size) { exit_next[base + i] = nx[cur][i]; exit_cnt[base + i] = cn[cur][i]; }
}

static __global__ __launch_bounds__(64) void k_tb_chain(uint32_t const *__restrict__ exit_next, uint32_t const *__restrict__ exit_cnt, uint32_t dp_size,
// ... 162 lines not shown
```

### founder-sequences_amd/csrc/fseq_path_pass2.hip

```cpp
#include "fseq_path.hpp"
#include "fseq_stream2.hpp"

namespace fseq {

namespace {

int pass2_sum_cells(fseq_ctx *c, LongRun &R, hipStream_t st)
{
	Shard const &sh = c->sh;
	if (!sh.on) return FSEQ_OK;
	uint32_t slots[2] = {(uint32_t) R.pass2_cells, (uint32_t) (R.pass2_cells >> 32)};
	std::vector<uint32_t> all(2 * sh.world);
	HIP_TRY(c, hipMemsetAsync(sh.xbuf, 0, all.size() * 4, st));
	HIP_TRY(c, hipMemcpyAsync(sh.xbuf + 2 * sh.rank, slots, 8, hipMemcpyHostToDevice, st));
	int rc;
	if ((rc = shard_exchange(c, all.size(), 0))) return rc;
	HIP_TRY(c, hipMemcpy(all.data(), sh.xbuf, all.size() * 4, hipMemcpyDeviceToHost));
	R.pass2_cells = 0;
	for (uint32_t g = 0; g < sh.world; ++g) R.pass2_cells += (uint64_t) all[2 * g] | ((uint64_t) all[2 * g + 1] << 32);
	c->sh.closed = true;
	return FSEQ_OK;
}

int long_pass2_reduced(fseq_ctx *c, LongRun &R)
{
	FSEQ_LONG_LOCALS(c);
	size_t const S2all = c->segments.size();
	if (!S2all) return FSEQ_OK;
	RedPlan const &plan = c->red.plan;
	ChainSnapSet cs{};
	if (!c->use_stream)
	{
		if (!select_chain_snap(ks.T, ks.E, &cs)) return fail(c, FSEQ_E_UNSUPPORTED, "pass 2: no chain step for this configuration");
		HIP_TRY(c, cs.prepare());
	}
	c->snap_slot.assign(S2all, -1);
	std::vector<uint64_t> rbs;
	std::vector<uint32_t> task_blk, ncls0;
	struct Wg { uint32_t blk, first, count, start; };
	std::vector<std::vector<Wg>> wgs((size_t) reduced_config_count());
	std::vector<uint64_t> o_rbs, o_srcs;
	std::vector<uint2> o_grp;
	std::vector<uint32_t> o_slot;
	uint64_t cells = 0;
	for (size_t si = 0; si < S2all; ++si)
	{
		uint64_t const rb = c->segments[si].rb;
		if (sharded)
		{
			uint32_t const owner = (uint32_t) std::min<uint64_t>(rb / ((uint64_t) sh.bpr * c->B), sh.active - 1u);
			if (owner != sh.rank) continue;
		}
		size_t const i = rbs.size();
		c->snap_slot[si] = (int64_t) i;
		rbs.push_back(rb);
		bool const border = rb % c->B == 0;
		uint32_t const blk = border ? (uint32_t) (rb / c->B) : (uint32_t) std::min<uint64_t>(rb / c->B, c->nblocks - 1u);
		task_blk.push_back(blk);
		ncls0.push_back(0u);
		if (border) continue;
		int const cf = blk < plan.config_snap_of.size() ? plan.config_snap_of[blk] : -1;
		if (cf >= 0 && plan.cnt[blk] != RED_NONE)
		{
			uint64_t start = c->red_ss_stride ? (rb - 1u) / c->red_ss_stride * c->red_ss_stride : 0u;
			if (start <= (uint64_t) blk * c->B || plan.full[blk]) start = (uint64_t) blk * c->B;
			auto &v = wgs[(size_t) cf];
			if (!v.empty() && v.back().blk == blk && v.back().start == (uint32_t) start) ++v.back().count;
			else v.push_back(Wg{blk, (uint32_t) i, 1u, (uint32_t) start});
		}
		else
		{
			ncls0[i] = 0xFFFFFFFFu;
			if (!o_srcs.empty() && o_srcs.back() == blk) ++o_grp.back().y;
			else { o_grp.push_back(make_uint2((uint32_t) o_rbs.size(), 1u)); o_srcs.push_back(blk); }
			o_rbs.push_back(rb); o_slot.push_back((uint32_t) i);
		}
	}
	size_t const S2 = rbs.size();
	if (!S2) { R.pass2_cells = 0; return pass2_sum_cells(c, R, st); }
	if ((rc = c->d_snap_a.ensure(c, S2 * (size_t) m))) return rc;
	if ((rc = c->d_snap_d.ensure(c, S2 * (size_t) m))) return rc;
	if ((rc = c->d_red_cls.ensure(c, S2 * (size_t) c->red_cap))) return rc;
	if ((rc = c->d_red_headd.ensure(c, S2 * (size_t) c->red_cap))) return rc;
	if ((rc = c->d_red_ncls.ensure(c, S2))) return rc;
	if ((rc = c->d_red_taskblk.ensure(c, S2))) return rc;
	if ((rc = c->d_red_wgtasks.ensure(c, 4 * S2 + 64))) return rc;
	if ((rc = c->d_red_p2grp.ensure(c, 2 * S2 + 2 + P2_STATS + P2_HAND))) return rc;
	if ((rc = c->d_cols.ensure(c, S2))) return rc;
	std::vector<uint32_t> p2grp;
	if (c->use_stream)
	{
		std::vector<uint2> g;
		for (size_t i = 0; i < S2; ++i)
		{
			if (i == 0 || task_blk[i] != task_blk[i - 1]) g.push_back(make_uint2((uint32_t) i, 0u));
			++g.back().y;
		}
		size_t k = 0;
		for (auto const &x : g)
		{
			bool mine = false;
			for (uint32_t t = x.x; t < x.x + x.y; ++t) mine = mine || ncls0[t] == 0u;
			if (mine) g[k++] = x;
		}
		g.resize(k);
		std::stable_sort(g.begin(), g.end(), [](uint2 const &x, uint2 const &y) { return x.y > y.y; });
		for (auto const &x : g) { p2grp.push_back(x.x); p2grp.push_back(x.y); }
		p2grp.push_back(0u);
		p2grp.insert(p2grp.end(), P2_STATS + P2_HAND, 0u);
	}
	std::vector<uint32_t> hb, hw;
	std::vector<RedLaunch> ls;
	for (size_t cf = 0; cf < wgs.size(); ++cf)
	{
		if (wgs[cf].empty()) continue;
		ls.push_back(RedLaunch{(int) cf, (uint32_t) hb.size(), (uint32_t) wgs[cf].size()});
		for (auto const &w : wgs[cf])
		{
			hb.push_back(w.blk); hw.push_back(w.first); hw.push_back(w.count); hw.push_back(w.start);
			cells += (rbs[w.first + w.count - 1u] - (uint64_t) w.start) * plan.cnt[w.blk];
		}
		if (c->tune.debug)
		{
			ReducedSet rs{};
			(void) reduced_config((int) cf, &rs);
			uint32_t tasks = 0;
			for (auto const &w : wgs[cf]) tasks += w.count;
			fprintf(stderr, "[fseq]   reduced pass 2: configuration of %u rows: %zu workgroups, %u tasks in blocks %u to %u (%u threads x %u rows)\n", rs.rows, wgs[cf].size(), tasks,
			        wgs[cf].front().blk, wgs[cf].back().blk, rs.T, rs.E);
		}
	}
	{
		size_t const need = S2 * 16 + hb.size() * 16 + p2grp.size() * 4 + 256 + (P2_STATS + P2_HAND) * 4;
		if (c->red_pin2_bytes < need)
		{
			if (c->h_red_pin2) (void) hipHostFree(c->h_red_pin2);
			c->h_red_pin2 = nullptr; c->red_pin2_bytes = 0;
			HIP_TRY(c, hipHostMalloc(reinterpret_cast<void **>(&c->h_red_pin2), need * 2, hipHostMallocDefault));
			c->red_pin2_bytes = need * 2;
		}
		uint8_t *pp = c->h_red_pin2;
		auto put = [&](void const *src, size_t bytes) { void *at = pp; memcpy(pp, src, bytes); pp += (bytes + 15) & ~size_t(15); return at; };
		HIP_TRY(c, hipMemcpyAsync(c->d_cols, put(rbs.data(), S2 * 8), S2 * 8, hipMemcpyHostToDevice, st));
		HIP_TRY(c, hipMemcpyAsync(c->d_red_taskblk, put(task_blk.data(), S2 * 4), S2 * 4, hipMemcpyHostToDevice, st));
		HIP_TRY(c, hipMemcpyAsync(c->d_red_ncls, put(ncls0.data(), S2 * 4), S2 * 4, hipMemcpyHostToDevice, st));
		if (!p2grp.empty())
			HIP_TRY(c, hipMemcpyAsync(c->d_red_p2grp, put(p2grp.data(), p2grp.size() * 4), p2grp.size() * 4, hipMemcpyHostToDevice, st));
		if (!hb.empty())
		{
			HIP_TRY(c, hipMemcpyAsync(c->d_red_wgtasks + 3 * S2, put(hb.data(), hb.size() * 4), hb.size() * 4, hipMemcpyHostToDevice, st));
			HIP_TRY(c, hipMemcpyAsync(c->d_red_wgtasks, put(hw.data(), hw.size() * 4), hw.size() * 4, hipMemcpyHostToDevice, st));
		}
	}
	uint32_t *const pin_stats = reinterpret_cast<uint32_t *>(c->h_red_pin2 + c->red_pin2_bytes - (P2_STATS + P2_HAND) * 4);
	c->p2_stats_have = false; c->p2_groups = 0;
	HIP_TRY(c, hipEventRecord(c->ev.pass2_begin, st));
	progress(c, FSEQ_STAGE_SAMPLES, 0, S2);
	RangeScope range_p2("fseq pass 2: boundary states (update_pbwt_task)");
	RedArgs RA;
	red_fill_args(c, RA);
	RA.task_rb = c->d_cols.as<unsigned long long const>();
	RA.cls = c->d_red_cls; RA.headd = c->d_red_headd; RA.ncls = c->d_red_ncls;
	RA.blocks = c->d_red_wgtasks + 3 * S2; RA.wg_tasks = c->d_red_wgtasks;
	if (!ls.empty())
	{
		std::stable_sort(ls.begin(), ls.end(), [](RedLaunch const &x, RedLaunch const &y) { return x.count > y.count; });
		if ((rc = red_launch_all(c, ls, RA, ListArgs{(uint32_t) L}))) return rc;
	}
	SnapArgs tasks;
	tasks.A = msa_args(c);
	tasks.bstate_a = c->d_bstate_a; tasks.bstate_d = c->d_bstate_d; tasks.task_blk = c->d_red_taskblk;
	tasks.snap_a = c->d_snap_a; tasks.snap_d = c->d_snap_d; tasks.ss.snap_stride = c->snap_stride; tasks.keyed = scan_keyed(c);
	if (!c->use_stream)
		cs.launch(st, (uint32_t) S2, cs.lds, tasks, RA);
	else
	{
		uint32_t const ngrp = (uint32_t) ((p2grp.size() - 1 - P2_STATS - P2_HAND) / 2);
		if (ngrp)
		{
			uint32_t *const stats = c->d_red_p2grp + 2 * (size_t) ngrp + 1;
			if ((rc = launch_chain_snap_grouped(c, ngrp, stats))) return rc;
			HIP_TRY(c, hipMemcpyAsync(pin_stats, stats, (P2_STATS + P2_HAND) * 4, hipMemcpyDeviceToHost, st));
			c->p2_stats_have = true; c->p2_groups = ngrp;
		}
	}
	for (size_t i = 0; i < S2; ++i)
		if (ncls0[i] == 0u && rbs[i] % c->B != 0) cells += (uint64_t) m * 4u;
	if (!o_grp.empty())
	{
		size_t const So = o_rbs.size();
		DevTemp<uint32_t> tmp_a(c), tmp_d(c);
		DevTemp<uint64_t> d_orb(c), d_osrc(c);
		DevTemp<uint2> d_ogrp(c);
		if ((rc = tmp_a.alloc(So * (size_t) m)) || (rc = tmp_d.alloc(So * (size_t) m)) ||
		    (rc = d_orb.alloc(So)) || (rc = d_osrc.alloc(o_srcs.size())) || (rc = d_ogrp.alloc(o_grp.size()))) return rc;
		HIP_TRY(c, hipMemcpyAsync(d_orb, o_rbs.data(), So * 8, hipMemcpyHostToDevice, st));
		HIP_TRY(c, hipMemcpyAsync(d_osrc, o_srcs.data(), o_srcs.size() * 8, hipMemcpyHostToDevice, st));
		HIP_TRY(c, hipMemcpyAsync(d_ogrp, o_grp.data(), o_grp.size() * sizeof(uint2), hipMemcpyHostToDevice, st));
		tasks.task_rb = d_orb; tasks.task_grp = d_ogrp; tasks.task_src = d_osrc; tasks.snap_a = tmp_a; tasks.snap_d = tmp_d;
		if (!c->use_stream) ks.snap(st, (uint32_t) o_grp.size(), ks.lds_snap, tasks);
		else launch_replay_stream(c, o_grp.size(), tasks);
		for (size_t j = 0; j < So; ++j)
		{
			HIP_TRY(c, hipMemcpyAsync(c->d_snap_a + (size_t) o_slot[j] * m, tmp_a + j * (size_t) m, (size_t) m * 4, hipMemcpyDeviceToDevice, st));
			HIP_TRY(c, hipMemcpyAsync(c->d_snap_d + (size_t) o_slot[j] * m, tmp_d + j * (size_t) m, (size_t) m * 4, hipMemcpyDeviceToDevice, st));
		}
		for (size_t g = 0; g < o_grp.size(); ++g) cells += (o_rbs[o_grp[g].x + o_grp[g].y - 1] - o_srcs[g] * c->B) * m;
		HIP_TRY(c, hipStreamSynchronize(st));
	}
	HIP_TRY(c, hipEventRecord(c->ev.pass2_end, st));
	HIP_TRY(c, hipGetLastError());
	HIP_TRY(c, hipStreamSynchronize(st));
	range_p2.end();
	if (c->p2_stats_have)
	{
		memcpy(c->p2_stats, pin_stats, sizeof(c->p2_stats));
		memcpy(c->p2_hand, pin_stats + P2_STATS, sizeof(c->p2_hand));
		if (c->tune.debug) fprintf(stderr, "[fseq] pass 2 chain steps: %u groups took the keys phase B handed over, %u gathered their own\n", c->p2_hand[0], c->p2_hand[1]);
	}
	progress(c, FSEQ_STAGE_SAMPLES, S2, S2);
	float f = 0;
	HIP_TRY(c, hipEventElapsedTime(&f, c->ev.pass2_begin, c->ev.pass2_end)); R.ms_p2 = f;
	R.pass2_cells = cells;
	return pass2_sum_cells(c, R, st);
}

}

int long_pass2(fseq_ctx *c, LongRun &R)
{
	FSEQ_LONG_LOCALS(c);
	c->p2_stats_have = false;
	if (c->red_active) return long_pass2_reduced(c, R);
	uint64_t &pass2_cells = R.pass2_cells;
	double &ms_p2 = R.ms_p2;
	size_t const S2 = c->segments.size();
	if (S2)
	{
		if ((rc = c->d_cols.ensure(c, S2))) return rc;
		std::vector<uint64_t> rbs, srcs;
		std::vector<uint2> grp;
		uint64_t const sstr = c->snap_stride;
		std::vector<uint64_t> starts;
		std::vector<uint32_t> grp_blk;
		c->snap_slot.assign(S2, -1);
		for (size_t i = 0; i < S2; ++i)
		{
			uint64_t const rb = c->segments[i].rb;
			if (sharded)
			{
				uint32_t const owner = (uint32_t) std::min<uint64_t>(rb / ((uint64_t) sh.bpr * c->B), sh.active - 1u);
				if (owner != sh.rank) continue;
			}
			c->snap_slot[i] = (int64_t) rbs.size();
			rbs.push_back(rb);
			uint64_t const blk = std::min<uint64_t>(rb / c->B, c->ss_ids ? c->nblocks - 1u : c->nblocks);
			uint64_t const q = rb / sstr;
			uint64_t src = blk, p0 = blk * c->B;
			if (c->d_ss_a && q >= 1 && q * sstr > p0) { src = q | (1ull << 63); p0 = q * sstr; }
			if (grp.empty() || srcs.back() != src) { grp.push_back(make_uint2((uint32_t) (rbs.size() - 1), 1u)); srcs.push_back(src); starts.push_back(p0); grp_blk.push_back((uint32_t) blk); }
			else ++grp.back().y;
		}
		for (size_t g = 0; g < grp.size(); ++g)
			pass2_cells += (rbs[grp[g].x + grp[g].y - 1] - starts[g]) * m;
		size_t const S2m = rbs.size();
		if ((rc = c->d_snap_a.ensure(c, S2m * (size_t) m))) return rc;
		if ((rc = c->d_snap_d.ensure(c, S2m * (size_t) m))) return rc;
		if ((rc = c->d_src.ensure(c, srcs.size()))) return rc;
		if ((rc = c->d_grp.ensure(c, grp.size()))) return rc;
		{
			if ((rc = pin_reserve(c, (srcs.size() + S2m + grp.size()) * 8 + 256))) return rc;
			uint64_t *const psrc = pin_take<uint64_t>(c, srcs.size());
			uint64_t *const prb = pin_take<uint64_t>(c, S2m);
			uint2 *const pgrp = pin_take<uint2>(c, grp.size());
			std::copy(srcs.begin(), srcs.end(), psrc);
			std::copy(rbs.begin(), rbs.end(), prb);
			std::copy(grp.begin(), grp.end(), pgrp);
			if (!srcs.empty()) HIP_TRY(c, hipMemcpyAsync(c->d_src, psrc, srcs.size() * 8, hipMemcpyHostToDevice, st));
			if (S2m) HIP_TRY(c, hipMemcpyAsync(c->d_cols, prb, S2m * 8, hipMemcpyHostToDevice, st));
			if (!grp.empty()) HIP_TRY(c, hipMemcpyAsync(c->d_grp, pgrp, grp.size() * sizeof(uint2), hipMemcpyHostToDevice, st));
		}
		HIP_TRY(c, hipEventRecord(c->ev.pass2_begin, st));
		progress(c, FSEQ_STAGE_SAMPLES, 0, S2);
		RangeScope range_p2("fseq pass 2: boundary states (update_pbwt_task)");
		SnapArgs tasks;
		tasks.A = msa_args(c);
		tasks.bstate_a = c->d_bstate_a; tasks.bstate_d = c->d_bstate_d; tasks.task_rb = c->d_cols; tasks.task_grp = c->d_grp; tasks.task_src = c->d_src;
		tasks.snap_a = c->d_snap_a; tasks.snap_d = c->d_snap_d; tasks.ss = stride_states(c); tasks.keyed = scan_keyed(c);
		if (!grp.empty() && c->use_stream && c->ss_ids)
		{
			std::vector<uint32_t> wgb;
			std::vector<uint2> wgg;
			std::vector<uint64_t> wgw;
			for (size_t g = 0; g < grp.size(); ++g)
			{
				if (wgb.empty() || wgb.back() != grp_blk[g]) { wgb.push_back(grp_blk[g]); wgg.push_back(make_uint2((uint32_t) g, 1u)); wgw.push_back(0); }
				else ++wgg.back().y;
				wgw.back() += rbs[grp[g].x + grp[g].y - 1] - starts[g] + 2;
			}
			{
				std::vector<uint32_t> order(wgb.size());
				for (uint32_t i = 0; i < order.size(); ++i) order[i] = i;
				std::stable_sort(order.begin(), order.end(), [&](uint32_t x, uint32_t y) { return wgw[x] > wgw[y]; });
				std::vector<uint32_t> b2(wgb.size());
				std::vector<uint2> g2(wgg.size());
				for (size_t i = 0; i < order.size(); ++i) { b2[i] = wgb[order[i]]; g2[i] = wgg[order[i]]; }
				wgb.swap(b2); wgg.swap(g2);
			}
			if ((rc = c->d_wgblk.ensure(c, wgb.size()))) return rc;
			if ((rc = c->d_wggrp.ensure(c, wgb.size()))) return rc;
			HIP_TRY(c, hipMemcpyAsync(c->d_wgblk, wgb.data(), wgb.size() * 4, hipMemcpyHostToDevice, st));
			HIP_TRY(c, hipMemcpyAsync(c->d_wggrp, wgg.data(), wgg.size() * sizeof(uint2), hipMemcpyHostToDevice, st));
			tasks.ws = c->d_ws; tasks.wg_block = c->d_wgblk; tasks.wg_groups = c->d_wggrp; tasks.bs_w = c->d_bs_w; tasks.bs_h = c->d_bs_h;
			c->s2.launch_snap(st, (uint32_t) wgb.size(), c->s2_lds, tasks);
			HIP_TRY(c, hipStreamSynchronize(st));
		}
		else if (c->use_stream) launch_replay_stream(c, grp.size(), tasks);
		else if (!grp.empty()) ks.snap(st, (uint32_t) grp.size(), ks.lds_snap, tasks);
		HIP_TRY(c, hipEventRecord(c->ev.pass2_end, st));
		HIP_TRY(c, hipGetLastError());
		HIP_TRY(c, hipStreamSynchronize(st));
		range_p2.end();
		progress(c, FSEQ_STAGE_SAMPLES, S2, S2);
		float f = 0;
		HIP_TRY(c, hipEventElapsedTime(&f, c->ev.pass2_begin, c->ev.pass2_end)); ms_p2 = f;
		if ((rc = pass2_sum_cells(c, R, st))) return rc;
	}

	return FSEQ_OK;
}

}
```

### founder-sequences_amd/csrc/fseq_path_reduced.hip

```cpp
#include "fseq_path.hpp"

namespace fseq {

namespace {

uint32_t red_symcap(uint32_t m, uint32_t bsh, ReducedSet const &rs, bool direct, size_t cls_ld = 0)
{
	uint32_t const bytes = direct ? sym_bytes(m, bsh) : std::max<uint32_t>(sym_bytes(rs.rows, bsh), (uint32_t) cls_ld);
	return (bytes + 1023u) & ~1023u;
}

bool columns_fit_reduced(uint32_t m, uint32_t B, uint32_t bsh, ReducedSet const &rs, bool direct)
{
	return rs.lds(B, red_symcap(m, bsh, rs, direct)) <= LDS_LIMIT && (uint64_t) rs.rows + B + 1u <= 65535u;
}

std::vector<RedConfig> red_configs(uint32_t m, uint32_t B, uint32_t bsh, bool direct, size_t cls_ld = 0)
{
	std::vector<RedConfig> out;
	for (int i = 0; i < reduced_config_count(); ++i)
	{
		ReducedSet rs;
		(void) reduced_config(i, &rs);
		RedConfig f{rs.rows, rs.values, rs.T, rs.E, rs.ew, columns_fit_reduced(m, B, bsh, rs, direct)};
		if (cls_ld && !direct && f.fits)
		{
			size_t const lds_rows = rs.lds(B, red_symcap(m, bsh, rs, false)), lds_cls = rs.lds(B, red_symcap(m, bsh, rs, false, cls_ld));
			if (lds_cls == lds_rows) f.cls = true;
			else if (lds_cls <= LDS_LIMIT && rs.prepare(lds_cls) == hipSuccess)
				f.cls = red_cls_direct(lds_cls, LDS_LIMIT, rs.resident(lds_rows), rs.resident(lds_cls));
		}
		out.push_back(f);
	}
	return out;
}

bool red_cls_stageable(fseq_ctx const *c)
{
	return c->cls_on && !c->red_direct && !c->tune.class_gather && ((uint64_t) c->cls_ld << c->bsh) <= 16384u;
}

bool red_needs_msa(fseq_ctx const *c)
{
	return !c->red_direct && !(red_cls_stageable(c) && c->cls_every && c->red.plan.gathered == 0u);
}

}

void red_fill_args(fseq_ctx *c, RedArgs &RA)
{
	RA.cnt = c->d_red_cnt; RA.vmin = c->d_red_vmin; RA.a = c->d_red_a; RA.d = c->d_red_d; RA.leaf = c->d_red_leaf;
	RA.invalid = c->d_red_invalid; RA.any_invalid = &red_flags(c)->unproven; RA.cap = c->red_cap; RA.m_true = c->p.m;
	RA.direct = c->red_direct ? 1u : 0u; RA.colbytes = sym_bytes(c->p.m, c->bsh); RA.rank = c->d_rank;
	RA.ss_a = c->d_red_ss_a; RA.ss_d = c->d_red_ss_d; RA.ss_stride = c->red_ss_stride; RA.ss_cap = c->red_ss_cap;
	RA.blocks = c->d_red_blocks;
	RA.cls_src = c->d_red_src; RA.nkeys = c->d_nkeys; RA.cls_msa = c->d_cls; RA.cls_ld = c->cls_ld;
}

namespace {


int red_ensure_block_buffers(fseq_ctx *c, uint32_t cap)
{
	FSEQ_LONG_LOCALS(c);
	uint32_t const nbk = c->nblocks;
	if (c->d_red_cnt && c->red_cap == cap) return FSEQ_OK;
	if ((rc = c->d_red_cnt.alloc(c, nbk))) return rc;
	if ((rc = c->d_red_cnt_plan.alloc(c, nbk))) return rc;
	if ((rc = c->d_red_vmin.alloc(c, nbk))) return rc;
	if ((rc = c->d_red_invalid.alloc(c, nbk + 2))) return rc;
	if ((rc = c->d_red_blocks.alloc(c, 3 * (size_t) nbk))) return rc;
	if ((rc = c->d_red_src.alloc(c, nbk))) return rc;
	if ((rc = c->d_red_rows.alloc_range(c, b_lo, b_hi, cap))) return rc;
	if ((rc = c->d_red_leaf.alloc_range(c, b_lo, b_hi, cap))) return rc;
	if ((rc = c->d_red_a.alloc_range(c, b_lo, b_hi, cap))) return rc;
	if ((rc = c->d_red_d.alloc_range(c, b_lo, b_hi, cap))) return rc;
	c->red_cap = cap;
	c->red.memory.forget_plan();
	return FSEQ_OK;
}

int red_ensure_host(fseq_ctx *c)
{
	size_t const words = 6 * (size_t) c->nblocks + 64;
	if (c->red_pin_words < words)
	{
		if (c->h_red_pin) (void) hipHostFree(c->h_red_pin);
		c->h_red_pin = nullptr; c->red_pin_words = 0;
		HIP_TRY(c, hipHostMalloc(reinterpret_cast<void **>(&c->h_red_pin), words * 4, hipHostMallocDefault));
		c->red_pin_words = words;
	}
	if (!c->red_ev.fork)
		for (hipEvent_t *evt : c->red_ev.all()) HIP_TRY(c, hipEventCreateWithFlags(evt, hipEventDisableTiming));
	return FSEQ_OK;
}

int red_launch_prep(fseq_ctx *c, uint32_t X, uint32_t cap)
{
	FSEQ_LONG_LOCALS(c);
	c->red_direct = !c->use_stream;
	RedPrepArgs A{};
	A.bstate_a = c->d_bstate_a; A.bstate_d = c->d_bstate_d; A.rank = c->d_rank; A.blocks = nullptr;
	A.m = m; A.B = c->B; A.L = (uint32_t) L; A.cap = cap; A.block0 = b_lo; A.leaf_only = 0; A.n = n; A.direct = c->red_direct ? 1u : 0u;
	A.Xp = X + (c->tune.reduced_margin >= 0 ? (uint32_t) c->tune.reduced_margin : X / 4u + 8u);
	A.cnt = c->d_red_cnt; A.vmin = c->d_red_vmin; A.rows = c->d_red_rows; A.leaf = c->d_red_leaf; A.a = c->d_red_a; A.d = c->d_red_d;
	A.invalid = c->d_red_invalid; A.flags = &red_flags(c)->unproven;
	HIP_TRY(c, launch_reduce_prep(st, my_blocks, A));
	return FSEQ_OK;
}

int red_reduce_msa(fseq_ctx *c)
{
	FSEQ_LONG_LOCALS(c);
	c->cls_staged = red_cls_stageable(c);
	if (!red_needs_msa(c)) { c->cls_read = true; return FSEQ_OK; }
	{
		uint32_t const max_rows = c->red.plan.max_rows;
		size_t const ldr = ((size_t) sym_bytes(max_rows ? max_rows : 1u, c->bsh) + 15) & ~size_t(15);
		uint64_t const k_lo = (uint64_t) b_lo * c->B, k_hi = std::min<uint64_t>(n, (uint64_t) b_hi * c->B);
		size_t const need = (size_t) (k_hi - k_lo) * ldr + 64;
		if (c->red_ld != ldr || c->d_red_msa.cap < need)
		{
			if ((rc = c->d_red_msa.ensure(c, need))) return rc;
			c->red_ld = ldr;
		}
		c->d_red_msa.rebase((ptrdiff_t) ((size_t) k_lo * c->red_ld));
	}
	ReducedMsaArgs D{c->d_red_msa, c->red_ld, c->d_red_cnt, c->d_red_rows, c->red_cap, c->d_red_blocks, c->red.plan.listed, c->red.plan.max_rows};
	if (c->cls_staged && c->red.plan.gathered == 0u) c->cls_read = true;
	else
	{
		D.skip = c->cls_staged ? (uint32_t const *) c->d_red_src : nullptr;
		c->cls_read = c->cls_on && launch_reduce_cls(st, msa_args(c), D, ClassColumnArgs{c->d_cls, c->cls_ld, c->d_cls_have, c->d_red_leaf, c->d_rank});
		D.skip = nullptr;
		if (!c->cls_read) c->cls_staged = false;
	}
	if (c->cls_read && c->cls_every) return FSEQ_OK;
	if (c->cls_read) { D.flag = c->d_cls_have; D.want = 0u; }
	launch_reduce_msa(st, msa_args(c), D, c->tune.reduced_msa_gather);
	return FSEQ_OK;
}

int red_queue_remembered(fseq_ctx *c)
{
	FSEQ_LONG_LOCALS(c);
	launch_reduce_check(st, c->d_red_cnt + b_lo, c->d_red_cnt_plan + b_lo, my_blocks, &red_flags(c)->unproven);
	if (!c->red_direct && (rc = red_reduce_msa(c))) return rc;
	c->tm.reduced_blocks = c->red.plan.reduced_blocks; c->tm.reduced_rows_mean = c->red.plan.rows_mean;
	return FSEQ_OK;
}

int red_read_counts(fseq_ctx *c, RedPlanInput &in)
{
	FSEQ_LONG_LOCALS(c);
	uint32_t const nbk = c->nblocks;
	fseq_ctx::Red::Memory &M = c->red.memory;
	M.forget_plan();
	uint32_t *const h_cnt = c->h_red_pin;
	HIP_TRY(c, hipMemcpyAsync(h_cnt + b_lo, c->d_red_cnt + b_lo, (size_t) my_blocks * 4, hipMemcpyDeviceToHost, st));
	HIP_TRY(c, hipMemcpyAsync(c->d_red_cnt_plan + b_lo, c->d_red_cnt + b_lo, (size_t) my_blocks * 4, hipMemcpyDeviceToDevice, st));
	uint32_t *const h_have = c->h_red_pin + 4 * (size_t) nbk;
	bool const ask_have = c->cls_on && !c->cls_every;
	if (ask_have) HIP_TRY(c, hipMemcpyAsync(h_have + b_lo, c->d_cls_have + b_lo, (size_t) my_blocks * 4, hipMemcpyDeviceToHost, st));
	HIP_TRY(c, hipStreamSynchronize(st));
	if (ask_have) c->cls_every = std::all_of(h_have + b_lo, h_have + b_hi, [](uint32_t h) { return h != 0u; });
	if (M.force.size() != nbk) M.force.assign(nbk, 0);
	in.m = m; in.nblocks = nbk; in.b_lo = b_lo; in.b_hi = b_hi;
	in.cnt.assign(nbk, RED_NONE);
	std::copy(h_cnt + b_lo, h_cnt + b_hi, in.cnt.begin() + b_lo);
	in.force = M.force;
	in.configs = red_configs(m, c->B, c->bsh, c->red_direct, red_cls_stageable(c) ? c->cls_ld : 0);
	in.reduced_always = c->tune.reduced_always;
	in.no_block_list = c->use_stream && !c->s2.T;
	return FSEQ_OK;
}

bool red_config_cls(fseq_ctx const *c, int config)
{
	return red_cls_stageable(c) && (size_t) config < c->red.cls_config.size() && c->red.cls_config[(size_t) config];
}

void red_report(fseq_ctx const *c, RedPlan const &P)
{
	uint32_t const m = c->p.m, my_blocks = P.reduced_blocks + P.nfull;
	fprintf(stderr, "[fseq] reduced phase C: %u of %u blocks on their representatives (mean %u of %u rows, most %u), %u on all rows\n", P.reduced_blocks, my_blocks,
	        P.rows_mean, m, P.max_rows, P.nfull);
	for (RedBin const &bin : P.bins)
	{
		uint64_t sr = 0;
		for (uint32_t i = 0; i < bin.count; ++i) sr += P.cnt[P.blocks[bin.first + i]];
		ReducedSet rs;
		(void) reduced_config(bin.config, &rs);
		bool const cls = red_config_cls(c, bin.config);
		size_t const lds = rs.lds(c->B, red_symcap(m, c->bsh, rs, c->red_direct, cls ? c->cls_ld : 0));
		uint32_t const res = rs.prepare(lds) == hipSuccess ? rs.resident(lds) : 0u;
		uint32_t staged = 0;
		for (uint32_t i = 0; i < bin.count; ++i) staged += P.from_cls[P.blocks[bin.first + i]];
		fprintf(stderr, "[fseq]   configuration of %u rows: %zu blocks, %llu representatives on average (%u threads x %u rows, %u distinct values, %zu bytes of LDS, %u workgroups per CU); columns: %s (%u of its blocks)\n",
		        rs.rows, (size_t) bin.count, (unsigned long long) (sr / bin.count), rs.T, rs.E, rs.values, lds, res,
		        c->red_direct ? "the alignment's own" : cls ? "phase A's class columns, staged by the kernel" : c->cls_on && c->tune.class_columns ? "the reduced alignment, gathered from the class columns" : "the reduced alignment, gathered from the alignment",
		        c->red_direct ? bin.count : cls ? staged : bin.count - staged);
	}
}

int red_size_buffers(fseq_ctx *c)
{
	FSEQ_LONG_LOCALS(c);
	uint32_t const max_rows = c->red.plan.max_rows;
	{
		uint32_t const stride_ = c->use_stream ? 32u : 16u;
		uint32_t const scap = (std::max(max_rows, 1u) + 63u) & ~63u;
		uint64_t const q_lo = (uint64_t) b_lo * c->B / stride_, q_hi = std::min<uint64_t>(n, (uint64_t) b_hi * c->B) / stride_;
		size_t const words = ((size_t) (q_hi - q_lo) + 2) * scap;
		if ((rc = c->d_red_ss_a.ensure(c, words))) return rc;
		if ((rc = c->d_red_ss_d.ensure(c, words))) return rc;
		c->red_ss_stride = stride_; c->red_ss_cap = scap;
		c->d_red_ss_a.rebase((ptrdiff_t) ((size_t) q_lo * scap));
		c->d_red_ss_d.rebase((ptrdiff_t) ((size_t) q_lo * scap));
	}
	return FSEQ_OK;
}

int red_upload_blocks(fseq_ctx *c)
{
	std::vector<uint32_t> const &blocks = c->red.plan.blocks;
	uint32_t *const h_blocks = c->h_red_pin + c->nblocks;
	std::copy(blocks.begin(), blocks.end(), h_blocks);
	HIP_TRY(c, hipMemcpyAsync(c->d_red_blocks, h_blocks, blocks.size() * 4, hipMemcpyHostToDevice, c->stream));
	uint32_t *const h_src = c->h_red_pin + 5 * (size_t) c->nblocks;
	std::copy(c->red.plan.from_cls.begin(), c->red.plan.from_cls.end(), h_src);
	HIP_TRY(c, hipMemcpyAsync(c->d_red_src, h_src, (size_t) c->nblocks * 4, hipMemcpyHostToDevice, c->stream));
	return FSEQ_OK;
}

}

int red_plan(fseq_ctx *c, uint32_t X, bool *use)
{
	FSEQ_LONG_LOCALS(c);
	fseq_ctx::Red::Memory &M = c->red.memory;
	*use = false;
	uint32_t cap = std::min<uint32_t>(m, 11264u);
	if (c->tune.reduced_cap) cap = std::min<uint32_t>(cap, (uint32_t) c->tune.reduced_cap);
	if ((rc = red_ensure_block_buffers(c, cap))) return rc;
	if (!my_blocks) return FSEQ_OK;
	if (M.declined && M.declined_X == X && !c->tune.reduced_always) return FSEQ_OK;
	if ((rc = red_ensure_host(c))) return rc;
	if ((rc = red_launch_prep(c, X, cap))) return rc;
	if (M.plan_holds && M.plan_X == X && M.force.size() == c->nblocks)
	{
		if ((rc = red_queue_remembered(c))) return rc;
		*use = true;
		return FSEQ_OK;
	}
	RedPlanInput in;
	if ((rc = red_read_counts(c, in))) return rc;
	c->red.plan = plan_reduced(in);
	c->red.cls_config.assign(in.configs.size(), 0);
	for (size_t i = 0; i < in.configs.size(); ++i) c->red.cls_config[i] = in.configs[i].cls ? 1 : 0;
	RedPlan const &plan = c->red.plan;
	c->tm.reduced_blocks = plan.reduced_blocks; c->tm.reduced_rows_mean = plan.rows_mean;
	if (c->tune.debug) red_report(c, plan);
	switch (plan.verdict)
	{
	case RedVerdict::Declined:
		M.declined = true; M.declined_X = X;
		c->d_cls.release(c); c->cls_on = false;
		return FSEQ_OK;
	case RedVerdict::NoBlockList:
		c->d_cls.release(c); c->cls_on = false; M.cls_unread = true;
		return FSEQ_OK;
	case RedVerdict::Use:
		break;
	}
	if ((rc = red_size_buffers(c))) return rc;
	if ((rc = red_upload_blocks(c))) return rc;
	if (!c->red_direct && (rc = red_reduce_msa(c))) return rc;
	M.plan_holds = true; M.plan_X = X;
	*use = true;
	return FSEQ_OK;
}


int red_launch_all(fseq_ctx *c, std::vector<RedLaunch> const &ls, RedArgs const &base, ListArgs const &lists)
{
	FSEQ_LONG_LOCALS(c);
	if (ls.empty()) return FSEQ_OK;
	size_t const nside = std::min<size_t>(ls.size() - 1, RED_SIDE_STREAMS);
	auto const joins = c->red_ev.joins();
	if (nside) HIP_TRY(c, hipEventRecord(c->red_ev.fork, st));
	size_t main_i = 0;
	for (size_t i = 1; i < ls.size(); ++i) if (ls[i].count > ls[main_i].count) main_i = i;
	size_t side = 0;
	ColumnsArgs C;
	C.A = msa_args(c);
	if (!c->red_direct) { C.A.msa = c->d_red_msa; C.A.ld = c->red_ld; }
	C.lists = lists;
	for (size_t i = 0; i < ls.size(); ++i)
	{
		ReducedSet rs;
		(void) reduced_config(ls[i].config, &rs);
		RedArgs RA = base;
		bool const cls = c->cls_staged && red_config_cls(c, ls[i].config);
		RA.symcap = red_symcap(m, c->bsh, rs, c->red_direct, cls ? c->cls_ld : 0);
		RA.cls_have = cls ? (uint32_t const *) c->d_cls_have : nullptr;
		size_t const lds = rs.lds(c->B, RA.symcap);
		HIP_TRY(c, rs.prepare(lds));
		RA.blocks = base.blocks + ls[i].first;
		if (base.wg_tasks) RA.wg_tasks = base.wg_tasks + 3 * (size_t) ls[i].first;
		hipStream_t s_ = st;
		size_t const slot = (i != main_i && side < nside) ? side++ : nside;
		if (slot < nside)
		{
			if (slot >= 1 && !c->red_st[slot - 1]) HIP_TRY(c, hipStreamCreateWithFlags(&c->red_st[slot - 1], hipStreamNonBlocking));
			s_ = slot == 0 ? c->stream2 : c->red_st[slot - 1];
			HIP_TRY(c, hipStreamWaitEvent(s_, c->red_ev.fork, 0));
		}
		rs.launch(s_, ls[i].count, lds, C, RA);
		if (slot < nside) HIP_TRY(c, hipEventRecord(*joins[slot], s_));
	}
	for (size_t i = 0; i < nside; ++i) HIP_TRY(c, hipStreamWaitEvent(st, *joins[i], 0));
	HIP_TRY(c, hipGetLastError());
	return FSEQ_OK;
}

int red_columns(fseq_ctx *c)
{
	RedArgs RA;
	red_fill_args(c, RA);
	std::vector<RedLaunch> ls;
	for (auto const &bin : c->red.plan.bins) ls.push_back(RedLaunch{bin.config, bin.first, bin.count});
	std::reverse(ls.begin(), ls.end());
	return red_launch_all(c, ls, RA, list_args(c));
}

int red_take_invalid(fseq_ctx *c, uint32_t b_lo, uint32_t b_hi, uint32_t *count, uint32_t *wide)
{
	std::vector<uint32_t> inv(c->nblocks);
	HIP_TRY(c, hipMemcpy(inv.data(), c->d_red_invalid, (size_t) c->nblocks * 4, hipMemcpyDeviceToHost));
	*count = *wide = 0;
	for (uint32_t b = b_lo; b < b_hi; ++b)
		if (inv[b] && !c->red.plan.full[b]) { c->red.memory.force[b] = inv[b] == RED_WIDE ? RED_FORCE_WIDE : RED_FORCE_FULL; ++*count; *wide += inv[b] == RED_WIDE ? 1u : 0u; }
	if (*count) c->red.memory.forget_plan();
	return FSEQ_OK;
}

}

using namespace fseq;

extern "C" {

int fseq_debug_red_plan(uint32_t m, uint32_t B, uint32_t bits, int direct, uint32_t nblocks, uint32_t b_lo, uint32_t b_hi, uint32_t const *cnt,
                        uint8_t const *force, int reduced_always, int no_block_list, uint32_t *configs, uint32_t *n_configs, int *verdict,
                        uint8_t *full, int32_t *config_of, int32_t *config_snap_of, uint32_t *blocks, uint32_t *n_blocks, uint32_t *bins,
                        uint32_t *n_bins, uint32_t *summary)
{
	if (!m || !B || (bits != 2 && bits != 4 && bits != 8) || (!cnt && nblocks) || b_lo > b_hi || b_hi > nblocks || nblocks > (1u << 24)) return FSEQ_E_ARG;
	for (uint32_t b = 0; b < nblocks; ++b)
		if ((cnt[b] > m && cnt[b] != RED_NONE) || (force && force[b] > RED_FORCE_WIDE)) return FSEQ_E_ARG;
	RedPlanInput in;
	in.m = m; in.nblocks = nblocks; in.b_lo = b_lo; in.b_hi = b_hi;
	in.cnt.assign(cnt, cnt + nblocks);
	if (force) in.force.assign(force, force + nblocks);
	else in.force.assign(nblocks, 0);
	in.configs = red_configs(m, B, bits == 2 ? 2u : bits == 4 ? 1u : 0u, direct != 0);
	in.reduced_always = reduced_always != 0;
	in.no_block_list = no_block_list != 0;
	if (in.configs.size() > FSEQ_DEBUG_RED_CONFIGS) return FSEQ_E_UNSUPPORTED;
	RedPlan const P = plan_reduced(in);
	if (n_configs) *n_configs = (uint32_t) in.configs.size();
	for (size_t i = 0; configs && i < in.configs.size(); ++i)
	{
		RedConfig const &f = in.configs[i];
		uint32_t const row[6] = {f.rows, f.values, f.T, f.E, f.ew ? 1u : 0u, f.fits ? 1u : 0u};
		std::copy(row, row + 6, configs + 6 * i);
	}
	if (verdict) *verdict = (int) P.verdict;
	if (full) std::copy(P.full.begin(), P.full.end(), full);
	if (config_of) std::copy(P.config_of.begin(), P.config_of.end(), config_of);
	if (config_snap_of) std::copy(P.config_snap_of.begin(), P.config_snap_of.end(), config_snap_of);
	if (blocks) std::copy(P.blocks.begin(), P.blocks.end(), blocks);
	if (n_blocks) *n_blocks = (uint32_t) P.blocks.size();
	for (size_t i = 0; bins && i < P.bins.size(); ++i)
	{
		bins[3 * i] = (uint32_t) P.bins[i].config; bins[3 * i + 1] = P.bins[i].first; bins[3 * i + 2] = P.bins[i].count;
	}
	if (n_bins) *n_bins = (uint32_t) P.bins.size();
	if (summary)
	{
		uint32_t const s[6] = {P.full_at, P.nfull, P.listed, P.max_rows, P.reduced_blocks, P.rows_mean};
		std::copy(s, s + 6, summary);
	}
	return FSEQ_OK;
}

int fseq_debug_red_cls_direct(uint32_t m, uint32_t B, uint32_t bits, uint64_t cls_ld, uint32_t config, uint32_t resident_rows, uint32_t resident_cls,
                              uint64_t *lds_rows, uint64_t *lds_cls, int *direct)
{
	if (!m || !B || (bits != 2 && bits != 4 && bits != 8) || !cls_ld || cls_ld > (1u << 20) || config >= (uint32_t) reduced_config_count()) return FSEQ_E_ARG;
	uint32_t const bsh = bits == 2 ? 2u : bits == 4 ? 1u : 0u;
// ... 11 lines not shown
```

### founder-sequences_amd/csrc/fseq_reduced.hip

```cpp
#include "fseq_ctx.hpp"
#include "fseq_reduced.hpp"

namespace fseq {

namespace {

template <int T, int E, bool PK, bool EW>
struct LaunchRed {
	static size_t lds(uint32_t B, uint32_t symcap)
	{
		return columns_lds_bytes<T, E, 4, PK>(B) - 2 * carve_bytes((size_t) T * E, 1) + 2 * carve_bytes(symcap, 1);
	}
	static hipError_t prepare(size_t bytes) { return allow_lds(k_columns_red<T, E, 4, PK, EW>, bytes); }
	static void launch(hipStream_t st, uint32_t grid, size_t bytes, ColumnsArgs const &C, RedArgs const &red)
	{
		MsaArgs const &A = C.A;
		hipLaunchKernelGGL((k_columns_red<T, E, 4, PK, EW>), dim3(grid), dim3(T), bytes, st, A.msa, A.ld, A.n, A.B, C.lists.L, C.lists.X, C.lists.stride, C.lists.ent, C.lists.hdr,
		                   A.npass, A.bsh, red);
	}
	static uint32_t resident(size_t bytes)
	{
		int nb = 0;
		if (hipOccupancyMaxActiveBlocksPerMultiprocessor(&nb, k_columns_red<T, E, 4, PK, EW>, T, bytes) != hipSuccess || nb < 1) nb = 1;
		return (uint32_t) nb;
	}
	static ReducedSet make() { return ReducedSet{(uint32_t) T, (uint32_t) E, EW ? (uint32_t) (T - 64) * E : (uint32_t) T * E, (uint32_t) columns_value_cap(T, E, PK), PK, EW, &lds, &prepare, &launch, &resident}; }
};

#define FSEQ_RED_CONFIGS(X) \
	X(64, 3, false, false) X(64, 5, false, false) X(64, 7, false, false) \
	X(256, 3, false, true) X(256, 3, false, false) X(256, 5, false, true) X(256, 5, false, false) X(512, 5, false, true) X(512, 5, false, false) \
	X(512, 7, false, true) X(512, 7, false, false) X(1024, 5, false, true) X(1024, 5, false, false) X(512, 15, true, true) X(1024, 7, true, true) X(1024, 7, true, false) \
	X(1024, 8, true, true) X(1024, 9, true, true) X(1024, 9, true, false) X(1024, 10, true, true) X(1024, 10, true, false) X(1024, 11, true, true) \
	X(1024, 11, true, false) X(1024, 12, true, true)

template <int T, int E, bool PK>
struct LaunchChainSnap {
	static hipError_t prepare() { return allow_lds(k_chain_snap<T, E, PK>, chain_snap_lds_bytes<T, E, PK>()); }
	static void launch(hipStream_t st, uint32_t grid, size_t bytes, SnapArgs const &S, RedArgs const &red)
	{
		hipLaunchKernelGGL((k_chain_snap<T, E, PK>), dim3(grid), dim3(T), bytes, st, S.bstate_a, S.bstate_d, red.rank, red.m_true, S.task_blk, (uint32_t const *) red.cls,
		                   (uint32_t const *) red.headd, (uint32_t const *) red.ncls, red.cap, S.snap_a, S.snap_d, S.keyed);
	}
	static ChainSnapSet make() { return ChainSnapSet{chain_snap_lds_bytes<T, E, PK>(), &prepare, &launch}; }
};

#define FSEQ_CHAIN_SNAP_CONFIGS(X) \
	X(64, 1, false) X(64, 7, false) X(256, 5, false) X(512, 5, false) X(512, 7, false) X(1024, 5, false) X(1024, 7, false) X(1024, 9, true) X(1024, 10, true) X(1024, 11, true)

}

int reduced_config_count()
{
	int n = 0;
#define X(T_, E_, PK_, EW_) ++n;
	FSEQ_RED_CONFIGS(X)
#undef X
	return n;
}

bool reduced_config(int index, ReducedSet *out)
{
	int i = 0;
#define X(T_, E_, PK_, EW_) if (i++ == index) { *out = LaunchRed<T_, E_, PK_, EW_>::make(); return true; }
	FSEQ_RED_CONFIGS(X)
#undef X
	return false;
}

bool select_chain_snap(uint32_t T, uint32_t E, ChainSnapSet *out)
{
#define X(T_, E_, PK_) if (T == T_ && E == E_) { *out = LaunchChainSnap<T_, E_, PK_>::make(); return true; }
	FSEQ_CHAIN_SNAP_CONFIGS(X)
#undef X
	return false;
}

hipError_t launch_reduce_prep(hipStream_t st, uint32_t grid, RedPrepArgs const &A)
{
	size_t const bytes = reduce_prep_lds_bytes(A.m);
	if (bytes > 160 * 1024) return hipErrorInvalidValue;
	hipError_t const e = allow_lds(k_reduce_prep, bytes);
	if (e != hipSuccess) return e;
	hipLaunchKernelGGL(k_reduce_prep, dim3(grid), dim3(RED_PREP_T), bytes, st, A);
	return hipSuccess;
}

void launch_reduce_check(hipStream_t st, uint32_t const *cnt, uint32_t const *planned, uint32_t count, uint32_t *flags)
{
	if (count) hipLaunchKernelGGL(k_reduce_check, dim3((count + 255u) / 256u), dim3(256), 0, st, cnt, planned, count, flags);
}

template <int BSH, int R>
static bool launch_reduce_msa_lds(hipStream_t st, MsaArgs const &A, ReducedMsaArgs const &D, uint32_t colbytes)
{
	static bool prepared = false;
	size_t const lds = (size_t) 2 * R * 16384;
	if (!prepared)
	{
		if (hipFuncSetAttribute(reinterpret_cast<void const *>(&k_reduce_msa_lds<BSH, R>), hipFuncAttributeMaxDynamicSharedMemorySize, (int) lds) != hipSuccess)
		{
			(void) hipGetLastError();
			return false;
		}
		prepared = true;
	}
	hipLaunchKernelGGL((k_reduce_msa_lds<BSH, R>), dim3(D.nlisted, 4), dim3(1024), lds, st, A.msa, A.ld, D.red, D.ldr, D.cnt, D.rows, D.cap, A.n, A.B, D.blocks, colbytes, D.flag, D.want, D.pad, D.pad_per, D.skip);
	return true;
}
// ... 40 lines not shown
```

### founder-sequences_amd/csrc/fseq_types.hpp

```cpp
#pragma once

#include "fseq_redplan.hpp"

#include <hip/hip_runtime.h>
#include <stddef.h>
#include <stdint.h>

namespace fseq {

struct DpArrays {
	uint32_t *M, *LB, *SZ, *Tb, *Tbv;
	unsigned long long *K;
	uint32_t tstride;
};

struct PhaseACounters {
	uint32_t tree_sliced;
	uint32_t tree_given_up;
	uint32_t trie_given_up;
};
struct PathWords {
	uint32_t dp[4];
	PhaseACounters phase_a;
	uint32_t dense_columns;
// ... 80 lines not shown
	uint32_t keyed = 0;
	uint32_t const *task_blk = nullptr;
	uint32_t *ws = nullptr;
	uint32_t const *wg_block = nullptr;
	uint2 const *wg_groups = nullptr;
	uint32_t const *bs_w = nullptr;
	uint8_t const *bs_h = nullptr;
};

struct ColumnsArgs {
	MsaArgs A;
	uint32_t const *bstate_a = nullptr, *bstate_d = nullptr;
	ListArgs lists;
	StrideStates ss;
	uint32_t *ws = nullptr;
	uint32_t block0 = 0;
	uint32_t *done_host = nullptr;
	uint32_t epoch = 0;
	uint32_t const *blocklist = nullptr;
	uint32_t const *colmask = nullptr;
};

struct ChainMultiArgs {
	uint32_t const *rank, *keyd, *nkeys;
	uint32_t m, nb_total, G;
	uint64_t cols_per_block;
	uint32_t *ws;
	uint32_t *hist;
	uint32_t const *start_a, *start_d;
	uint32_t *out_state_a, *out_state_d, *out_rank, *out_keyd, *out_nkeys;
	uint32_t grp0;
	uint32_t step;
	uint32_t pass;
	uint32_t nchains;
	uint16_t *hand_keys;
	uint32_t *hand_flag;
};

struct ReducedMsaArgs {
	uint8_t *red = nullptr;
	size_t ldr = 0;
	uint32_t const *cnt = nullptr, *rows = nullptr;
	uint32_t cap = 0;
	uint32_t const *blocks = nullptr;
	uint32_t nlisted = 0, max_rows = 0;
	uint32_t const *flag = nullptr;
	uint32_t want = 0;
	uint32_t const *pad = nullptr;
	size_t pad_per = 0;
	uint32_t const *skip = nullptr;
};

struct ClassColumnArgs {
	uint8_t const *cls = nullptr;
	size_t ldc = 0;
	uint32_t const *have = nullptr, *leaf = nullptr;
	uint32_t const *rank = nullptr;
};

constexpr uint32_t P2_HIST = 19;
constexpr uint32_t CW_STATS = 4 + P2_HIST;
constexpr uint32_t P2_STATS = 4 + P2_HIST;
constexpr uint32_t P2_HAND = 2;
constexpr uint32_t RED_WIDE = 2u;
struct RedArgs {
	uint32_t const *cnt = nullptr;
	uint32_t const *vmin = nullptr;
	uint32_t const *a = nullptr;
	uint32_t const *d = nullptr;
	uint32_t const *leaf = nullptr;
	uint32_t const *blocks = nullptr;
	uint32_t *invalid = nullptr;
	uint32_t cap = 0;
	uint32_t m_true = 0;
	uint32_t direct = 0;
	uint32_t colbytes = 0;
	uint32_t symcap = 0;
	uint32_t const *rank = nullptr;
	uint32_t *any_invalid = nullptr;
	uint32_t const *cls_have = nullptr, *cls_src = nullptr, *nkeys = nullptr;
	uint8_t const *cls_msa = nullptr;
	size_t cls_ld = 0;
	uint32_t const *wg_tasks = nullptr;
	uint32_t *ss_a = nullptr, *ss_d = nullptr;
	uint32_t ss_stride = 0, ss_cap = 0;
	unsigned long long const *task_rb = nullptr;
	uint32_t *cls = nullptr;
	uint32_t *headd = nullptr;
	uint32_t *ncls = nullptr;
};

struct RedPrepArgs {
	uint32_t const *bstate_a, *bstate_d;
	uint32_t const *rank;
	uint32_t const *blocks;
	uint32_t m, B, L, Xp, cap, block0, leaf_only, direct;
	uint32_t *invalid, *flags;
	uint64_t n;
	uint32_t *cnt, *vmin, *rows, *leaf, *a, *d;
};

}
```

### include/fseq_debug.h

```cpp
#ifndef FSEQ_DEBUG_H
#define FSEQ_DEBUG_H

#include "fseq.h"

#ifdef __cplusplus
extern "C" {
#endif

int  fseq_debug_dp_schedule(uint64_t segment_length, uint64_t n, uint64_t col_hi, uint32_t *n_rounds, uint32_t *cells_per_round,
                            uint32_t *rounds_within, int *pipelined);
int  fseq_debug_dp(fseq_ctx *ctx, uint32_t *lb, uint32_t *max_size, uint32_t *size);
int  fseq_debug_dp_owned(fseq_ctx *ctx, uint64_t *first, uint64_t *last, int *final_cell, int *whole_arrays);
int  fseq_debug_block_state(fseq_ctx *ctx, uint64_t block_idx, uint32_t *a_out, uint32_t *d_out);
int  fseq_debug_column_list(fseq_ctx *ctx, uint64_t c, uint32_t *values, uint32_t *counts,
                            uint32_t *n_entries, uint32_t *cnt0, uint32_t *complete);
int  fseq_debug_list_windows(fseq_ctx *ctx, uint64_t *bytes_held, uint64_t *columns_per_window, uint32_t *windows,
                             uint32_t *merge_windows);

int  fseq_debug_rmq(int device, uint32_t const *keys, uint32_t count, uint32_t const *beg, uint32_t const *end, uint32_t n_queries,
                    uint32_t *index_hbm, uint32_t *index_lds);

int  fseq_debug_ranges(uint64_t *pushes, uint64_t *pops, int *with_roctx);

int  fseq_debug_clock(fseq_ctx *ctx, double *ghz, uint32_t *workgroups);

int  fseq_debug_set_tuning(fseq_ctx *ctx, char const *name, char const *value);

int  fseq_debug_join_path(fseq_ctx *ctx, int *path);

int  fseq_debug_bipartite_path(fseq_ctx *ctx, int *path);

int  fseq_debug_device_bytes(fseq_ctx *ctx, uint64_t *now, uint64_t *peak, int reset_peak);

int  fseq_debug_alphabet(fseq_ctx *ctx, uint32_t *sigma, uint32_t *bits, uint8_t *code_to_byte);

int  fseq_debug_packed_columns(fseq_ctx *ctx, uint64_t c0, uint64_t c1, uint8_t *out, uint64_t *ld, uint32_t *bits);

int  fseq_debug_pass2_paths(fseq_ctx *ctx, uint32_t *by_runs, uint32_t *by_sort, uint32_t *copies, uint32_t *max_runs, uint32_t *runs_hist);

int  fseq_debug_class_columns(fseq_ctx *ctx, uint32_t *from_classes, uint32_t *from_alignment, uint32_t block, uint32_t *have, uint32_t *nkeys,
                              uint64_t *ldc, uint8_t *out, uint64_t out_bytes);

int  fseq_debug_column_sources(fseq_ctx *ctx, uint32_t *staged, uint32_t *gathered, uint32_t block, uint32_t *block_staged);

int  fseq_debug_red_cls_direct(uint32_t m, uint32_t B, uint32_t bits, uint64_t cls_ld, uint32_t config, uint32_t resident_rows, uint32_t resident_cls,
                               uint64_t *lds_rows, uint64_t *lds_cls, int *direct);

int  fseq_debug_random_path(fseq_ctx *ctx, int *path);

int  fseq_debug_join_score_path(fseq_ctx *ctx, int *path);

int  fseq_debug_join_score(int device, uint32_t m, uint32_t X, uint32_t S, uint16_t const *of, uint16_t const *perm_cls_left,
                           uint16_t const *perm_cls_right, fseq_join_score_entry *junctions, uint32_t *breaks, uint32_t *support,
                           fseq_join_score_summary *summary);

int  fseq_debug_restored_bounds(uint64_t const *kept, uint64_t n, uint64_t n_src, uint64_t const *lb, uint64_t const *rb, uint64_t n_segments,
                                uint64_t *src_lb, uint64_t *src_rb);

int  fseq_debug_input_kept_range(uint64_t const *kept, uint64_t n_kept, uint64_t c0, uint64_t ncols, uint64_t *k0, uint64_t *k1);

int  fseq_debug_segments_file(fseq_ctx *ctx, uint64_t *batches, uint64_t *bytes, uint64_t *longest_line, uint64_t *lines);

typedef struct fseq_graph_file_stats {
	uint64_t batches[3], lines[3], bytes[3];
} fseq_graph_file_stats;
int  fseq_debug_graph_file(fseq_ctx *ctx, fseq_graph_file_stats *stats);

typedef struct fseq_graph_thread_info {
	uint32_t key_bits, table_slots;
	uint64_t candidates_verified, candidates_rejected, queries_out_of_alphabet;
} fseq_graph_thread_info;
int  fseq_debug_graph_thread(fseq_ctx *ctx, fseq_graph_thread_info *info);

typedef struct fseq_graph_nearest_info {
	uint64_t batches, packed_words, query_words;
	uint32_t bits, reserved;
} fseq_graph_nearest_info;
int  fseq_debug_graph_nearest_info(fseq_ctx *ctx, fseq_graph_nearest_info *info);
int  fseq_debug_graph_nearest_plan(uint64_t const *lb, uint64_t const *rb, uint32_t const *count, uint64_t n_segments, uint32_t bits,
                                   uint64_t budget_bytes, uint64_t *words, uint64_t *first, uint64_t *n_batches);
int  fseq_debug_graph_nearest(int device, uint8_t const *cols, uint64_t ld, uint32_t m, uint64_t n, uint32_t bits,
                              uint64_t const *seg_lb, uint64_t const *seg_rb, uint32_t const *count, uint32_t const *rep,
                              uint32_t n_segments, uint32_t X, uint8_t const *qcols, uint64_t qld, uint32_t n_queries, uint32_t qbits,
                              uint32_t sigma, uint64_t batch_bytes, uint32_t *nodes, uint32_t *distances, uint32_t *ties,
                              fseq_graph_nearest_info *info);

int  fseq_debug_pass2_step(int device, uint32_t m, uint32_t nblocks, uint32_t const *a0, uint32_t const *d0, uint32_t const *rank, uint32_t cap,
                           uint32_t ntasks, uint32_t const *task_blk, uint32_t const *cls, uint32_t const *headd, uint32_t const *ncls,
                           uint32_t run_cap, uint32_t workgroups, uint32_t *snap_a, uint32_t *snap_d, uint32_t *stats);

int  fseq_debug_chain_launch(int device, uint32_t m, uint32_t nb_total, uint32_t G, uint64_t cols_per_block, uint32_t const *rank, uint32_t const *keyd,
                             uint32_t const *nkeys, uint32_t first_chain, uint32_t chains, uint32_t const *start_a, uint32_t const *start_d,
                             uint32_t *out_state_a, uint32_t *out_state_d, uint32_t *out_rank, uint32_t *out_keyd, uint32_t *out_nkeys);

int  fseq_debug_chain_launch_wg(int device, uint32_t m, uint32_t nb_total, uint32_t G, uint64_t cols_per_block, uint32_t const *rank, uint32_t const *keyd,
                                uint32_t const *nkeys, uint32_t first_chain, uint32_t chains, uint32_t const *start_a, uint32_t const *start_d,
                                uint32_t run_cap, uint32_t workgroups, uint32_t *out_state_a, uint32_t *out_state_d, uint32_t *out_rank,
                                uint32_t *out_keyd, uint32_t *out_nkeys, uint32_t *stats);

int  fseq_debug_chain_launch_wg_keys(int device, uint32_t m, uint32_t nb_total, uint32_t G, uint64_t cols_per_block, uint32_t const *rank,
                                     uint32_t const *keyd, uint32_t const *nkeys, uint32_t first_chain, uint32_t chains, uint32_t const *start_a,
                                     uint32_t const *start_d, uint32_t run_cap, uint32_t workgroups, uint32_t *out_state_a, uint32_t *out_state_d,
                                     uint32_t *out_rank, uint32_t *out_keyd, uint32_t *out_nkeys, uint32_t *stats, uint16_t *hand_keys,
                                     uint32_t *hand_flag);

int  fseq_debug_pass2_step_keys(int device, uint32_t m, uint32_t nblocks, uint32_t const *a0, uint32_t const *d0, uint32_t const *rank, uint32_t cap,
                                uint32_t ntasks, uint32_t const *task_blk, uint32_t const *cls, uint32_t const *headd, uint32_t const *ncls,
                                uint32_t run_cap, uint32_t workgroups, uint16_t const *hand_keys, uint32_t const *hand_flag, uint32_t *snap_a,
                                uint32_t *snap_d, uint32_t *stats, uint32_t *hand_stats);

typedef struct fseq_chain_launch_info {
	uint32_t level, kind, chains, blocks, first_chain, workgroups;
} fseq_chain_launch_info;
#define FSEQ_DEBUG_CHAIN_LEVELS 40
#define FSEQ_DEBUG_CHAIN_LAUNCHES 80
typedef struct fseq_chain_plan {
	uint32_t fan;
	uint32_t fan_round5;
	uint32_t turns;
	uint32_t shard_k, shard_q;
	uint32_t blocks_per_rank;
// ... 71 lines not shown
```

Measured before the change: 2221 billion.

## Add sweep-form reduced kernel for class tables with 16-bit snapshot states

Adds a SWEEP template variant of the reduced columns kernel used when building class tables. It skips the value table, histogram and list-wave work, and stores divergence snapshots as column offsets relative to the block, in 16-bit form. The snapshot stride is halved, and snapshots are written with packed vector stores. The intent is to cut LDS use, global snapshot traffic and per-column work in the class-table pass, at the cost of an extra kernel instantiation and tighter limits on value ranges (rows and offsets must fit in 16 bits).

After: 2324 billion, median of 6. 1.05x the previous value.

```diff
diff --git a/founder-sequences_amd/__init__.py b/founder-sequences_amd/__init__.py
--- a/founder-sequences_amd/__init__.py
+++ b/founder-sequences_amd/__init__.py
@@ -209,6 +209,7 @@
     "fseq_write_block_graph_restored", "fseq_graph_thread_rows_restored", "fseq_graph_thread_held_out_restored",
     "fseq_debug_chain_launch_wg_keys", "fseq_debug_pass2_step_keys",
     "fseq_debug_chain_plan", "fseq_debug_chain_plan_sharded", "fseq_debug_phase_b",
+    "fseq_debug_class_tables",
 ]
 DEBUG_EXPORTS = ["fseq_debug_dp", "fseq_debug_dp_owned", "fseq_debug_clock", "fseq_debug_ranges", "fseq_debug_block_state", "fseq_debug_column_list", "fseq_debug_rmq", "fseq_debug_dp_schedule", "fseq_debug_set_tuning",
                  "fseq_debug_list_windows", "fseq_debug_device_bytes", "fseq_debug_packed_columns", "fseq_debug_join_path", "fseq_debug_pass2_paths",
@@ -220,7 +221,7 @@
                  "fseq_debug_join_score_path", "fseq_debug_join_score", "fseq_debug_graph_file", "fseq_debug_local_pass",
                  "fseq_debug_graph_thread", "fseq_debug_graph_nearest_info", "fseq_debug_graph_nearest_plan", "fseq_debug_graph_nearest",
                  "fseq_debug_chain_launch_wg_keys", "fseq_debug_pass2_step_keys",
-                 "fseq_debug_chain_plan", "fseq_debug_chain_plan_sharded", "fseq_debug_phase_b"]
+                 "fseq_debug_chain_plan", "fseq_debug_chain_plan_sharded", "fseq_debug_phase_b", "fseq_debug_class_tables"]
 
 FSEQ_E_PEER = 6
 P2_RUN_CAP = 8832
@@ -327,6 +328,7 @@
     L.fseq_debug_join_path.argtypes = [vp, C.POINTER(C.c_int)]
     L.fseq_debug_bipartite_path.argtypes = [vp, C.POINTER(C.c_int)]
     L.fseq_debug_pass2_paths.argtypes = [vp] + [C.POINTER(C.c_uint32)] * 4 + [vp]
+    L.fseq_debug_class_tables.argtypes = [vp, vp, C.c_uint32, vp, vp, vp]
     L.fseq_debug_class_columns.argtypes = [vp, C.POINTER(C.c_uint32), C.POINTER(C.c_uint32), C.c_uint32, C.POINTER(C.c_uint32), C.POINTER(C.c_uint32), C.POINTER(u64), vp, u64]
     L.fseq_debug_column_sources.argtypes = [vp, C.POINTER(C.c_uint32), C.POINTER(C.c_uint32), C.c_uint32, C.POINTER(C.c_uint32)]
     L.fseq_debug_red_cls_direct.argtypes = [C.c_uint32, C.c_uint32, C.c_uint32, u64, C.c_uint32, C.c_uint32, C.c_uint32, C.POINTER(u64), C.POINTER(u64), C.POINTER(C.c_int)]
@@ -1681,6 +1683,14 @@
         out["runs_hist"] = [int(x) for x in hist]
         return out
 
+    def class_tables(self, columns):
+        cols = np.ascontiguousarray(columns, dtype=np.uint64)
+        cls = np.empty((len(cols), self.m), dtype=np.uint32)
+        headd = np.empty((len(cols), self.m), dtype=np.uint32)
+        ncls = np.empty(len(cols), dtype=np.uint32)
+        self._check(self.L.fseq_debug_class_tables(self.h, cols.ctypes.data, len(cols), cls.ctypes.data, headd.ctypes.data, ncls.ctypes.data))
+        return cls, headd, ncls
+
     def phase_b(self):
         info = PhaseBInfo()
         self._check(self.L.fseq_debug_phase_b(self.h, C.byref(info)))
diff --git a/founder-sequences_amd/csrc/fseq_ctx.hpp b/founder-sequences_amd/csrc/fseq_ctx.hpp
--- a/founder-sequences_amd/csrc/fseq_ctx.hpp
+++ b/founder-sequences_amd/csrc/fseq_ctx.hpp
@@ -52,9 +52,11 @@
 	uint32_t T, E, rows, values;
 	bool pk, ew;
 	size_t (*lds)(uint32_t B, uint32_t symcap);
-	hipError_t (*prepare)(size_t lds);
-	void (*launch)(hipStream_t st, uint32_t grid, size_t lds, ColumnsArgs const &cols, RedArgs const &red);
+	size_t (*lds_sweep)(uint32_t B, uint32_t symcap);
+	hipError_t (*prepare)(size_t lds, bool sweep);
+	hipError_t (*launch)(hipStream_t st, uint32_t grid, size_t lds, ColumnsArgs const &cols, RedArgs const &red);
 	uint32_t (*resident)(size_t lds);
+	bool phase_form() const { return T <= 128u || ew; }
 };
 int reduced_config_count();
 bool reduced_config(int index, ReducedSet *out);
@@ -119,6 +121,7 @@
 	int  reduced_margin = -1;
 	bool reduced_always = false;
 	bool reduced_msa_gather = false;
+	int  red_ss_stride = 0;
 	int  reduced_cap = 0;
 	bool class_gather = false;
 	int  class_columns = 1;
@@ -178,6 +181,7 @@
 			{"FSEQ_REDUCED_ALWAYS", &Tuning::reduced_always, nullptr, 0, 0, nullptr},
 			{"FSEQ_REDUCED_MSA_GATHER", &Tuning::reduced_msa_gather, nullptr, 0, 0, nullptr},
 			{"FSEQ_REDUCED_CAP", nullptr, &Tuning::reduced_cap, 1, 0, nullptr},
+			{"FSEQ_RED_SS_STRIDE", nullptr, &Tuning::red_ss_stride, 4, 0, nullptr},
 			{"FSEQ_P2_RUN_CAP", nullptr, &Tuning::p2_run_cap, 0, -1, nullptr},
 			{"FSEQ_CHAIN_RUN_CAP", nullptr, &Tuning::chain_run_cap, 0, -1, nullptr},
 			{"FSEQ_CHAIN_WG", nullptr, &Tuning::chain_wg, 0, 0, nullptr},
@@ -427,7 +431,7 @@
 	DevBuf<uint32_t> d_red_p2grp;
 	uint32_t p2_stats[fseq::P2_STATS]{};
 	bool p2_stats_have = false;
-	DevBuf<uint32_t> d_red_ss_a, d_red_ss_d;
+	DevBuf<uint16_t> d_red_ss_a, d_red_ss_d;
 	uint32_t red_ss_stride = 0, red_ss_cap = 0;
 	uint32_t *h_red_pin = nullptr;
 	size_t red_pin_words = 0;
diff --git a/founder-sequences_amd/csrc/fseq_kernels.hpp b/founder-sequences_amd/csrc/fseq_kernels.hpp
--- a/founder-sequences_amd/csrc/fseq_kernels.hpp
+++ b/founder-sequences_amd/csrc/fseq_kernels.hpp
@@ -643,7 +643,7 @@
 	}
 }
 
-template <int T, int E, int SIGMA, bool PK, bool EW, bool DENSE, bool RED>
+template <int T, int E, int SIGMA, bool PK, bool EW, bool DENSE, bool RED, bool SWEEP = false>
 __device__ __forceinline__ void columns_body(char *smem,
 	uint8_t const *__restrict__ msa, size_t ld, uint32_t m, uint64_t n, uint32_t B, uint32_t N2,
 	uint32_t const *__restrict__ bstate_a, uint32_t const *__restrict__ bstate_d,
@@ -654,9 +654,9 @@
 	FSEQ_CLOCK_STAMP(blockIdx.x, 0);
 	constexpr uint32_t CAP = T * E, VCAP = (uint32_t) columns_value_cap(T, E, PK);
 	static_assert(VCAP == CAP || RED, "a value table smaller than the rows: the reduced kernel, which can refuse a block");
+	static_assert(!SWEEP || (RED && !EW && !DENSE), "the sweep form: representatives, no list wave");
 	uint32_t const blk = RED ? red.blocks[blockIdx.x] : (blocklist ? blocklist[blockIdx.x] : blockIdx.x + block0);
 	uint32_t red_vmin = 0, red_deficit = 0, t_first = 0, t_count = 0, t_next = 0;
-	bool const red_snap = RED && red.cls != nullptr;
 	if constexpr (RED)
 	{
 		m = red.cnt[blk];
@@ -664,7 +664,7 @@
 		red_vmin = red.vmin[blk];
 		red_deficit = red.m_true - m;
 		N2 = 2; while (N2 < m + 1u) N2 <<= 1;
-		if (red_snap) { t_first = red.wg_tasks[3u * blockIdx.x]; t_count = red.wg_tasks[3u * blockIdx.x + 1u]; }
+		if constexpr (SWEEP) { t_first = red.wg_tasks[3u * blockIdx.x]; t_count = red.wg_tasks[3u * blockIdx.x + 1u]; }
 	}
 	bool const red_exact = RED && red_vmin <= 1u;
 	bool red_cls = false;
@@ -680,8 +680,8 @@
 	AT *d_l = cv.take<AT>(CAP);
 	uint8_t *sym0 = cv.take<uint8_t>(RED ? red.symcap : CAP);
 	uint8_t *sym1 = cv.take<uint8_t>(RED ? red.symcap : CAP);
-	uint32_t *cnt_l = cv.take<uint32_t>(PK ? (VCAP + B + 9) / 2 : VCAP + B + 8);
-	uint32_t *V_l = cv.take<uint32_t>(VCAP);
+	uint32_t *cnt_l = SWEEP ? nullptr : cv.take<uint32_t>(PK ? (VCAP + B + 9) / 2 : VCAP + B + 8);
+	uint32_t *V_l = SWEEP ? nullptr : cv.take<uint32_t>(VCAP);
 	StepScratch<T, SIGMA> &scr = *cv.take<StepScratch<T, SIGMA>>(1);
 	uint32_t *sscr = cv.take<uint32_t>(T / WAVE + 1);
 	constexpr bool PW = columns_pairwise(T, E, SIGMA, PK);
@@ -692,27 +692,48 @@
 	uint32_t const p0 = EW ? (tid >= 64u ? (tid - 64u) * E : 0x7FFF0000u) : tid * E;
 	bool const rows = !EW || tid >= 64u;
 	uint64_t const kblk = (uint64_t) blk * B;
-	uint64_t const k0 = red_snap ? (uint64_t) red.wg_tasks[3u * blockIdx.x + 2u] : kblk;
-	uint64_t const kend = red_snap ? (uint64_t) red.task_rb[t_first + t_count - 1u] : ((k0 + B < n) ? k0 + B : n);
+	uint64_t const k0 = SWEEP ? (uint64_t) red.wg_tasks[3u * blockIdx.x + 2u] : kblk;
+	uint64_t const kend = SWEEP ? (uint64_t) red.task_rb[t_first + t_count - 1u] : ((k0 + B < n) ? k0 + B : n);
 	uint32_t const nb = (uint32_t) (kend - k0);
 
+#ifdef FSEQ_KC_STAMPS
+	long long kc_p[5], kc_tab = 0, kc_tab0 = 0;
+	kc_p[0] = clock64();
+#endif
 	uint32_t a[E], d[E];
-	{
-		bool const from_ss = RED && k0 != kblk;
-		size_t const ob = from_ss ? (size_t) (k0 / red.ss_stride) * red.ss_cap : RED ? (size_t) blk * red.cap : (size_t) blk * m;
-		uint32_t const *const sa = from_ss ? red.ss_a : RED ? red.a : bstate_a, *const sd = from_ss ? red.ss_d : RED ? red.d : bstate_d;
+	if (SWEEP && k0 != kblk)
+	{
+		size_t const ob = (size_t) (k0 / red.ss_stride) * red.ss_cap;
+#pragma unroll
+		for (int e = 0; e < E; ++e)
+		{
+			uint32_t const pos = p0 + e;
+			a[e] = pos < m ? (uint32_t) red.ss_a[ob + pos] : 0u;
+			d[e] = pos < m ? (uint32_t) red.ss_d[ob + pos] : 0u;
+		}
+	}
+	else
+	{
+		size_t const ob = RED ? (size_t) blk * red.cap : (size_t) blk * m;
+		uint32_t const *const sa = RED ? red.a : bstate_a, *const sd = RED ? red.d : bstate_d;
 #pragma unroll
 		for (int e = 0; e < E; ++e)
 		{
 			uint32_t const pos = p0 + e;
 			a[e] = pos < m ? sa[ob + pos] : 0u;
-			d[e] = pos < m ? sd[ob + pos] : 0u;
-		}
-	}
-
+			d[e] = (!SWEEP && pos < m) ? sd[ob + pos] : 0u;
+		}
+	}
+
+#ifdef FSEQ_KC_STAMPS
+	asm volatile("s_waitcnt vmcnt(0)" ::: "memory");
+	kc_p[1] = clock64();
+#endif
 	uint32_t *sb = reinterpret_cast<uint32_t *>(a_l);
-	uint32_t D0 = 0;
+	uint32_t D0 = SWEEP ? (uint32_t) (k0 - kblk) + 1u : 0u;
 	bool have_values = false;
+	if constexpr (!SWEEP)
+	{
 	if constexpr (RED)
 	{
 		uint32_t &hash_fail = scr.has[0];
@@ -804,13 +825,17 @@
 	__syncthreads();
 	for (uint32_t i = tid; i < (PK ? (D0 + nb + 9u) / 2u : D0 + nb + 8u); i += T) cnt_l[i] = 0;
 	__syncthreads();
-
+	}
+
+#ifdef FSEQ_KC_STAMPS
+	kc_p[2] = clock64();
+#endif
 	uint32_t id[E];
 #pragma unroll
 	for (int e = 0; e < E; ++e)
 	{
-		id[e] = 0;
-		if (p0 + e < m)
+		id[e] = SWEEP ? d[e] : 0u;
+		if (!SWEEP && p0 + e < m)
 		{
 			uint32_t lo = 0, hi = D0;
 			uint32_t const key = d[e];
@@ -855,10 +880,11 @@
 	}
 	__syncthreads();
 
-	bool const zero_present = (V_l[0] == 0u);
+	bool const zero_present = !SWEEP && (V_l[0] == 0u);
 	constexpr bool CARRY_OK = PK && E >= 9 && !columns_slim(T, E, PK);
 	bool const carry = CARRY_OK && npass == 2u && bsh == 1u && ((RED && red.direct) ? red.m_true : red_cls ? red_nkeys : m) <= 16384u;
 #ifdef FSEQ_KC_STAMPS
+	kc_p[3] = clock64();
 	long long kc_work = 0, kc_wait = 0, kc_last = clock64();
 	KcStamps kcs{{0, 0, 0, 0, 0, 0, 0, 0}, clock64()};
 #endif
@@ -940,7 +966,7 @@
 				{
 					a_l[dst[e]] = (AT) (CARRY_OK ? (a[e] | (hi[CARRY_OK ? e : 0] << 14)) : a[e]);
 					d_l[dst[e]] = (AT) dnew[e];
-					if (dnew[e] != d[e])
+					if (!SWEEP && dnew[e] != d[e])
 					{
 						cnt_dec<PK>(cnt_l, d[e]);
 						cnt_inc<PK>(cnt_l, dnew[e]);
@@ -960,7 +986,7 @@
 			if (DENSE && dense) break;
 		}
 
-		if (ss_a && (k0 + j + 1) % snap_stride == 0)
+		if constexpr (!RED) if (ss_a && (k0 + j + 1) % snap_stride == 0)
 		{
 			size_t const ob = (size_t) ((k0 + j + 1) / snap_stride) * m;
 #pragma unroll
@@ -977,28 +1003,43 @@
 			}
 		}
 
-		if (RED && !red_snap && red.ss_a && (k0 + j + 1u) % red.ss_stride == 0u && j + 1u < nb)
-		{
-			size_t const ob = (size_t) ((k0 + j + 1u) / red.ss_stride) * red.ss_cap;
-			for (uint32_t idx = tid; idx < m; idx += T)
-			{
-				uint32_t const vid = d_l[idx];
-				red.ss_a[ob + idx] = a_l[idx];
-				red.ss_d[ob + idx] = vid < D0 ? V_l[vid] : (uint32_t) (k0 + (vid - D0) + 1u);
-			}
-		}
-		if (RED && red_snap)
+		if constexpr (RED && !SWEEP)
+		{
+			if (red.ss_a && (k0 + j + 1u) % red.ss_stride == 0u && j + 1u < nb)
+			{
+				size_t const ob = (size_t) ((k0 + j + 1u) / red.ss_stride) * red.ss_cap;
+				auto into = [&](uint32_t vid) { return vid < D0 ? 0u : vid - D0 + 1u; };
+				for (uint32_t idx = tid * 8u; idx < m; idx += (uint32_t) T * 8u)
+				{
+					uint4 aw, dw;
+					if constexpr (PK)
+					{
+						aw = *reinterpret_cast<uint4 const *>(a_l + idx);
+						uint4 const w = *reinterpret_cast<uint4 const *>(d_l + idx);
+						dw.x = into(w.x & 0xFFFFu) | (into(w.x >> 16) << 16); dw.y = into(w.y & 0xFFFFu) | (into(w.y >> 16) << 16);
+						dw.z = into(w.z & 0xFFFFu) | (into(w.z >> 16) << 16); dw.w = into(w.w & 0xFFFFu) | (into(w.w >> 16) << 16);
+					}
+					else
+					{
+						uint4 const a0 = *reinterpret_cast<uint4 const *>(a_l + idx), a1 = *reinterpret_cast<uint4 const *>(a_l + idx + 4u);
+						uint4 const d0 = *reinterpret_cast<uint4 const *>(d_l + idx), d1 = *reinterpret_cast<uint4 const *>(d_l + idx + 4u);
+						aw = make_uint4(a0.x | (a0.y << 16), a0.z | (a0.w << 16), a1.x | (a1.y << 16), a1.z | (a1.w << 16));
+						dw = make_uint4(into(d0.x) | (into(d0.y) << 16), into(d0.z) | (into(d0.w) << 16), into(d1.x) | (into(d1.y) << 16), into(d1.z) | (into(d1.w) << 16));
+					}
+					*reinterpret_cast<uint4 *>(red.ss_a + ob + idx) = aw;
+					*reinterpret_cast<uint4 *>(red.ss_d + ob + idx) = dw;
+				}
+			}
+		}
+		if constexpr (SWEEP)
 		{
 			if (t_next < t_count && red.task_rb[t_first + t_next] == k0 + j + 1u)
 			{
 				uint32_t const task = t_first + t_next;
-				uint32_t id_in = D0;
-				if (k0 != kblk)
-				{
-					uint32_t lo = 0, hi = D0;
-					while (lo < hi) { uint32_t const mid = (lo + hi) >> 1; if (V_l[mid] <= (uint32_t) kblk) lo = mid + 1; else hi = mid; }
-					id_in = lo;
-				}
+#ifdef FSEQ_KC_STAMPS
+				kc_tab0 = clock64();
+#endif
+				constexpr uint32_t id_in = 1u;
 				uint32_t nf = 0;
 				if (rows)
 				{
@@ -1023,17 +1064,19 @@
 							uint32_t lf = a_l[pos];
 							if (!red_cls) lf = key_of[lf];
 							red.cls[ot + lf] = r - 1u;
-							if (first) red.headd[ot + r - 1u] = vid < D0 ? V_l[vid] : (uint32_t) (k0 + (vid - D0) + 1u);
+							if (first) red.headd[ot + r - 1u] = (uint32_t) kblk + vid;
 						}
 					}
 				}
 				if (tid == 0) red.ncls[task] = total;
 				++t_next;
-			}
-			continue;
-		}
-
-		if (wave_id() == 0)
+#ifdef FSEQ_KC_STAMPS
+				kc_tab += clock64() - kc_tab0;
+#endif
+			}
+		}
+
+		else if (wave_id() == 0)
 		{
 			__builtin_amdgcn_s_setprio(3);
 #ifdef FSEQ_KC_STAMPS
@@ -1161,6 +1204,10 @@
 		}
 	}
 #ifdef FSEQ_KC_STAMPS
+	kc_p[4] = clock64();
+	if (RED && tid == 0 && (blockIdx.x == 100 || blockIdx.x == 1000))
+		printf("kc stamps reduced workgroup %u (%d x %d, %u rows, %u columns from column %llu, %u tasks): state load %lld, value table %lld, ids and histogram %lld, column loop %lld cycles, of which class tables %lld\n",
+		       blockIdx.x, T, E, m, nb, (unsigned long long) k0, t_count, kc_p[1] - kc_p[0], kc_p[2] - kc_p[1], kc_p[3] - kc_p[2], kc_p[4] - kc_p[3], kc_tab);
 	if (lane_id() == 0 && (blockIdx.x == 100 || blockIdx.x == 3000))
 		printf("kc stamps block %u wave %u: work %lld wait %lld cycles per column (%u columns); step: to barrier 1 %lld, wait %lld, between %lld, wait 1b %lld\n",
 		       blockIdx.x, wave_id(), kc_work / nb, kc_wait / nb, nb, kcs.acc[0] / nb, kcs.acc[1] / nb, kcs.acc[2] / nb, kcs.acc[3] / nb);
@@ -1184,13 +1231,13 @@
 	                                                 done_host, epoch, colmask, RedArgs{}, blocklist);
 }
 
-template <int T, int E, int SIGMA, bool PK, bool EW = false>
+template <int T, int E, int SIGMA, bool PK, bool EW = false, bool SW = false>
 __global__ __launch_bounds__(T, columns_min_waves(T, E, PK)) void k_columns_red(
 	uint8_t const *__restrict__ msa, size_t ld, uint64_t n, uint32_t B,
 	uint32_t L, uint32_t X, uint32_t stride, uint2 *__restrict__ ent, uint4 *__restrict__ hdr, uint32_t npass, uint32_t bsh, RedArgs const red)
 {
 	extern __shared__ __attribute__((aligned(16))) char smem[];
-	columns_body<T, E, SIGMA, PK, EW, false, true>(smem, msa, ld, 0u, n, B, 0u, nullptr, nullptr, L, X, stride, ent, hdr, npass, bsh, 0u, nullptr, nullptr, 0u,
+	columns_body<T, E, SIGMA, PK, EW, false, true, SW>(smem, msa, ld, 0u, n, B, 0u, nullptr, nullptr, L, X, stride, ent, hdr, npass, bsh, 0u, nullptr, nullptr, 0u,
 	                                                nullptr, 0u, nullptr, red);
 }
 
diff --git a/founder-sequences_amd/csrc/fseq_path_pass2.hip b/founder-sequences_amd/csrc/fseq_path_pass2.hip
--- a/founder-sequences_amd/csrc/fseq_path_pass2.hip
+++ b/founder-sequences_amd/csrc/fseq_path_pass2.hip
@@ -22,6 +22,38 @@
 	return FSEQ_OK;
 }
 
+struct SweepWg { uint32_t blk, first, count, start; };
+
+bool sweep_add_task(fseq_ctx const *c, std::vector<std::vector<SweepWg>> &wgs, uint32_t blk, uint64_t rb, uint32_t i)
+{
+	RedPlan const &plan = c->red.plan;
+	int const cf = blk < plan.config_snap_of.size() ? plan.config_snap_of[blk] : -1;
+	if (cf < 0 || plan.cnt[blk] == RED_NONE) return false;
+	uint64_t start = c->red_ss_stride ? (rb - 1u) / c->red_ss_stride * c->red_ss_stride : 0u;
+	if (start <= (uint64_t) blk * c->B || plan.full[blk]) start = (uint64_t) blk * c->B;
+	auto &v = wgs[(size_t) cf];
+	if (!v.empty() && v.back().blk == blk && v.back().start == (uint32_t) start) ++v.back().count;
+	else v.push_back(SweepWg{blk, i, 1u, (uint32_t) start});
+	return true;
+}
+
+void sweep_launch_lists(std::vector<std::vector<SweepWg>> const &wgs, std::vector<RedLaunch> &ls, std::vector<uint32_t> &hb, std::vector<uint32_t> &hw)
+{
+	for (size_t cf = 0; cf < wgs.size(); ++cf)
+	{
+		if (wgs[cf].empty()) continue;
+		ls.push_back(RedLaunch{(int) cf, (uint32_t) hb.size(), (uint32_t) wgs[cf].size()});
+		for (auto const &w : wgs[cf]) { hb.push_back(w.blk); hw.push_back(w.first); hw.push_back(w.count); hw.push_back(w.start); }
+	}
+}
+
+int sweep_class_tables(fseq_ctx *c, std::vector<RedLaunch> ls, RedArgs const &RA)
+{
+	if (ls.empty()) return FSEQ_OK;
+	std::stable_sort(ls.begin(), ls.end(), [](RedLaunch const &x, RedLaunch const &y) { return x.count > y.count; });
+	return red_launch_all(c, ls, RA, ListArgs{(uint32_t) c->p.segment_length});
+}
+
 int long_pass2_reduced(fseq_ctx *c, LongRun &R)
 {
 	FSEQ_LONG_LOCALS(c);
@@ -37,8 +69,7 @@
 	c->snap_slot.assign(S2all, -1);
 	std::vector<uint64_t> rbs;
 	std::vector<uint32_t> task_blk, ncls0;
-	struct Wg { uint32_t blk, first, count, start; };
-	std::vector<std::vector<Wg>> wgs((size_t) reduced_config_count());
+	std::vector<std::vector<SweepWg>> wgs((size_t) reduced_config_count());
 	std::vector<uint64_t> o_rbs, o_srcs;
 	std::vector<uint2> o_grp;
 	std::vector<uint32_t> o_slot;
@@ -59,16 +90,7 @@
 		task_blk.push_back(blk);
 		ncls0.push_back(0u);
 		if (border) continue;
-		int const cf = blk < plan.config_snap_of.size() ? plan.config_snap_of[blk] : -1;
-		if (cf >= 0 && plan.cnt[blk] != RED_NONE)
-		{
-			uint64_t start = c->red_ss_stride ? (rb - 1u) / c->red_ss_stride * c->red_ss_stride : 0u;
-			if (start <= (uint64_t) blk * c->B || plan.full[blk]) start = (uint64_t) blk * c->B;
-			auto &v = wgs[(size_t) cf];
-			if (!v.empty() && v.back().blk == blk && v.back().start == (uint32_t) start) ++v.back().count;
-			else v.push_back(Wg{blk, (uint32_t) i, 1u, (uint32_t) start});
-		}
-		else
+		if (!sweep_add_task(c, wgs, blk, rb, (uint32_t) i))
 		{
 			ncls0[i] = 0xFFFFFFFFu;
 			if (!o_srcs.empty() && o_srcs.back() == blk) ++o_grp.back().y;
@@ -111,15 +133,11 @@
 	}
 	std::vector<uint32_t> hb, hw;
 	std::vector<RedLaunch> ls;
+	sweep_launch_lists(wgs, ls, hb, hw);
 	for (size_t cf = 0; cf < wgs.size(); ++cf)
 	{
 		if (wgs[cf].empty()) continue;
-		ls.push_back(RedLaunch{(int) cf, (uint32_t) hb.size(), (uint32_t) wgs[cf].size()});
-		for (auto const &w : wgs[cf])
-		{
-			hb.push_back(w.blk); hw.push_back(w.first); hw.push_back(w.count); hw.push_back(w.start);
-			cells += (rbs[w.first + w.count - 1u] - (uint64_t) w.start) * plan.cnt[w.blk];
-		}
+		for (auto const &w : wgs[cf]) cells += (rbs[w.first + w.count - 1u] - (uint64_t) w.start) * plan.cnt[w.blk];
 		if (c->tune.debug)
 		{
 			ReducedSet rs{};
@@ -162,11 +180,7 @@
 	RA.task_rb = c->d_cols.as<unsigned long long const>();
 	RA.cls = c->d_red_cls; RA.headd = c->d_red_headd; RA.ncls = c->d_red_ncls;
 	RA.blocks = c->d_red_wgtasks + 3 * S2; RA.wg_tasks = c->d_red_wgtasks;
-	if (!ls.empty())
-	{
-		std::stable_sort(ls.begin(), ls.end(), [](RedLaunch const &x, RedLaunch const &y) { return x.count > y.count; });
-		if ((rc = red_launch_all(c, ls, RA, ListArgs{(uint32_t) L}))) return rc;
-	}
+	if ((rc = sweep_class_tables(c, ls, RA))) return rc;
 	SnapArgs tasks;
 	tasks.A = msa_args(c);
 	tasks.bstate_a = c->d_bstate_a; tasks.bstate_d = c->d_bstate_d; tasks.task_blk = c->d_red_taskblk;
@@ -331,3 +345,60 @@
 }
 
 }
+
+using namespace fseq;
+
+extern "C" {
+
+int fseq_debug_class_tables(fseq_ctx *c, uint64_t const *columns, uint32_t count, uint32_t *cls, uint32_t *headd, uint32_t *ncls)
+{
+	if (!c || !columns || !count || !cls || !headd || !ncls) return FSEQ_E_ARG;
+	if (int const rc0 = need_result(c, true)) return rc0;
+	if (!c->red_active || c->sh.on) return fail(c, FSEQ_E_UNSUPPORTED, "class tables: the last run did not go through the representatives on one rank");
+	FSEQ_LONG_LOCALS(c);
+	(void) hipSetDevice(p.device);
+	uint32_t const cap = c->red_cap;
+	std::vector<std::vector<SweepWg>> wgs((size_t) reduced_config_count());
+	std::vector<uint32_t> task_blk(count);
+	for (uint32_t i = 0; i < count; ++i)
+	{
+		uint64_t const rb = columns[i];
+		if (rb == 0 || rb >= n || rb % c->B == 0 || (i && rb <= columns[i - 1])) return fail(c, FSEQ_E_ARG, "class tables: ascending columns strictly inside blocks");
+		task_blk[i] = (uint32_t) (rb / c->B);
+		if (!sweep_add_task(c, wgs, task_blk[i], rb, i)) return fail(c, FSEQ_E_UNSUPPORTED, "class tables: a column of a block without representatives");
+	}
+	std::vector<RedLaunch> ls;
+	std::vector<uint32_t> hb, hw;
+	sweep_launch_lists(wgs, ls, hb, hw);
+	DevTemp<uint64_t> d_rb(c);
+	DevTemp<uint32_t> d_wg(c), d_blk(c), d_cls(c), d_headd(c), d_ncls(c);
+	if ((rc = d_rb.alloc(count)) || (rc = d_wg.alloc(hw.size())) || (rc = d_blk.alloc(hb.size())) || (rc = d_cls.alloc((size_t) count * cap)) ||
+	    (rc = d_headd.alloc((size_t) count * cap)) || (rc = d_ncls.alloc(count))) return rc;
+	HIP_TRY(c, hipMemcpyAsync(d_rb, columns, (size_t) count * 8, hipMemcpyHostToDevice, st));
+	HIP_TRY(c, hipMemcpyAsync(d_wg, hw.data(), hw.size() * 4, hipMemcpyHostToDevice, st));
+	HIP_TRY(c, hipMemcpyAsync(d_blk, hb.data(), hb.size() * 4, hipMemcpyHostToDevice, st));
+	HIP_TRY(c, hipMemsetAsync(d_cls, 0xFF, (size_t) count * cap * 4, st));
+	HIP_TRY(c, hipMemsetAsync(d_headd, 0xFF, (size_t) count * cap * 4, st));
+	HIP_TRY(c, hipMemsetAsync(d_ncls, 0, (size_t) count * 4, st));
+	HIP_TRY(c, hipStreamSynchronize(st));
+	RedArgs RA;
+	red_fill_args(c, RA);
+	RA.task_rb = d_rb.as<unsigned long long const>();
+	RA.cls = d_cls; RA.headd = d_headd; RA.ncls = d_ncls;
+	RA.blocks = d_blk; RA.wg_tasks = d_wg;
+	if ((rc = sweep_class_tables(c, ls, RA))) return rc;
+	HIP_TRY(c, hipStreamSynchronize(st));
+	std::vector<uint32_t> tab(cap), hd(cap), rank(m);
+	HIP_TRY(c, hipMemcpy(ncls, d_ncls, (size_t) count * 4, hipMemcpyDeviceToHost));
+	for (uint32_t i = 0; i < count; ++i)
+	{
+		if (i == 0 || task_blk[i] != task_blk[i - 1]) HIP_TRY(c, hipMemcpy(rank.data(), c->d_rank + (size_t) task_blk[i] * m, (size_t) m * 4, hipMemcpyDeviceToHost));
+		HIP_TRY(c, hipMemcpy(tab.data(), d_cls + (size_t) i * cap, (size_t) cap * 4, hipMemcpyDeviceToHost));
+		HIP_TRY(c, hipMemcpy(hd.data(), d_headd + (size_t) i * cap, (size_t) cap * 4, hipMemcpyDeviceToHost));
+		for (uint32_t r = 0; r < m; ++r) cls[(size_t) i * m + r] = rank[r] < cap ? tab[rank[r]] : 0xFFFFFFFFu;
+		for (uint32_t r = 0; r < m; ++r) headd[(size_t) i * m + r] = r < cap ? hd[r] : 0xFFFFFFFFu;
+	}
+	return FSEQ_OK;
+}
+
+}
diff --git a/founder-sequences_amd/csrc/fseq_path_reduced.hip b/founder-sequences_amd/csrc/fseq_path_reduced.hip
--- a/founder-sequences_amd/csrc/fseq_path_reduced.hip
+++ b/founder-sequences_amd/csrc/fseq_path_reduced.hip
@@ -27,7 +27,7 @@
 		{
 			size_t const lds_rows = rs.lds(B, red_symcap(m, bsh, rs, false)), lds_cls = rs.lds(B, red_symcap(m, bsh, rs, false, cls_ld));
 			if (lds_cls == lds_rows) f.cls = true;
-			else if (lds_cls <= LDS_LIMIT && rs.prepare(lds_cls) == hipSuccess)
+			else if (lds_cls <= LDS_LIMIT && rs.prepare(lds_cls, !rs.phase_form()) == hipSuccess)
 				f.cls = red_cls_direct(lds_cls, LDS_LIMIT, rs.resident(lds_rows), rs.resident(lds_cls));
 		}
 		out.push_back(f);
@@ -193,7 +193,7 @@
 		(void) reduced_config(bin.config, &rs);
 		bool const cls = red_config_cls(c, bin.config);
 		size_t const lds = rs.lds(c->B, red_symcap(m, c->bsh, rs, c->red_direct, cls ? c->cls_ld : 0));
-		uint32_t const res = rs.prepare(lds) == hipSuccess ? rs.resident(lds) : 0u;
+		uint32_t const res = rs.prepare(lds, !rs.phase_form()) == hipSuccess ? rs.resident(lds) : 0u;
 		uint32_t staged = 0;
 		for (uint32_t i = 0; i < bin.count; ++i) staged += P.from_cls[P.blocks[bin.first + i]];
 		fprintf(stderr, "[fseq]   configuration of %u rows: %zu blocks, %llu representatives on average (%u threads x %u rows, %u distinct values, %zu bytes of LDS, %u workgroups per CU); columns: %s (%u of its blocks)\n",
@@ -208,12 +208,13 @@
 	FSEQ_LONG_LOCALS(c);
 	uint32_t const max_rows = c->red.plan.max_rows;
 	{
-		uint32_t const stride_ = c->use_stream ? 32u : 16u;
+		uint32_t stride_ = c->use_stream ? 16u : 8u;
+		if (c->tune.red_ss_stride) { stride_ = 4u; while (stride_ * 2u <= (uint32_t) std::min(c->tune.red_ss_stride, 64)) stride_ *= 2u; }
 		uint32_t const scap = (std::max(max_rows, 1u) + 63u) & ~63u;
 		uint64_t const q_lo = (uint64_t) b_lo * c->B / stride_, q_hi = std::min<uint64_t>(n, (uint64_t) b_hi * c->B) / stride_;
-		size_t const words = ((size_t) (q_hi - q_lo) + 2) * scap;
-		if ((rc = c->d_red_ss_a.ensure(c, words))) return rc;
-		if ((rc = c->d_red_ss_d.ensure(c, words))) return rc;
+		size_t const halfwords = ((size_t) (q_hi - q_lo) + 2) * scap;
+		if ((rc = c->d_red_ss_a.ensure(c, halfwords))) return rc;
+		if ((rc = c->d_red_ss_d.ensure(c, halfwords))) return rc;
 		c->red_ss_stride = stride_; c->red_ss_cap = scap;
 		c->d_red_ss_a.rebase((ptrdiff_t) ((size_t) q_lo * scap));
 		c->d_red_ss_d.rebase((ptrdiff_t) ((size_t) q_lo * scap));
@@ -304,8 +305,9 @@
 		bool const cls = c->cls_staged && red_config_cls(c, ls[i].config);
 		RA.symcap = red_symcap(m, c->bsh, rs, c->red_direct, cls ? c->cls_ld : 0);
 		RA.cls_have = cls ? (uint32_t const *) c->d_cls_have : nullptr;
-		size_t const lds = rs.lds(c->B, RA.symcap);
-		HIP_TRY(c, rs.prepare(lds));
+		bool const sweep = RA.cls != nullptr;
+		size_t const lds = sweep ? rs.lds_sweep(c->B, RA.symcap) : rs.lds(c->B, RA.symcap);
+		HIP_TRY(c, rs.prepare(lds, sweep));
 		RA.blocks = base.blocks + ls[i].first;
 		if (base.wg_tasks) RA.wg_tasks = base.wg_tasks + 3 * (size_t) ls[i].first;
 		hipStream_t s_ = st;
@@ -316,7 +318,7 @@
 			s_ = slot == 0 ? c->stream2 : c->red_st[slot - 1];
 			HIP_TRY(c, hipStreamWaitEvent(s_, c->red_ev.fork, 0));
 		}
-		rs.launch(s_, ls[i].count, lds, C, RA);
+		HIP_TRY(c, rs.launch(s_, ls[i].count, lds, C, RA));
 		if (slot < nside) HIP_TRY(c, hipEventRecord(*joins[slot], s_));
 	}
 	for (size_t i = 0; i < nside; ++i) HIP_TRY(c, hipStreamWaitEvent(st, *joins[i], 0));
diff --git a/founder-sequences_amd/csrc/fseq_reduced.hip b/founder-sequences_amd/csrc/fseq_reduced.hip
--- a/founder-sequences_amd/csrc/fseq_reduced.hip
+++ b/founder-sequences_amd/csrc/fseq_reduced.hip
@@ -11,20 +11,53 @@
 	{
 		return columns_lds_bytes<T, E, 4, PK>(B) - 2 * carve_bytes((size_t) T * E, 1) + 2 * carve_bytes(symcap, 1);
 	}
-	static hipError_t prepare(size_t bytes) { return allow_lds(k_columns_red<T, E, 4, PK, EW>, bytes); }
-	static void launch(hipStream_t st, uint32_t grid, size_t bytes, ColumnsArgs const &C, RedArgs const &red)
+	static constexpr bool PHASE = T <= 128 || EW, SWEEP = !EW;
+	static size_t lds_sweep(uint32_t, uint32_t symcap)
+	{
+		size_t const runs = columns_run_words(T, E, 4, PK);
+		return 2 * carve_bytes((size_t) T * E, PK ? 2 : 4) + 2 * carve_bytes(symcap, 1) + carve_bytes(1, sizeof(StepScratch<T, 4>)) + carve_bytes(T / WAVE + 1, 4)
+		     + (runs ? carve_bytes(runs, 4) : 0);
+	}
+	static hipError_t prepare(size_t bytes, bool sweep)
+	{
+		if constexpr (SWEEP) { if (sweep) return allow_lds(k_columns_red<T, E, 4, PK, EW, true>, bytes); }
+		if constexpr (PHASE) { if (!sweep) return allow_lds(k_columns_red<T, E, 4, PK, EW>, bytes); }
+		return hipErrorInvalidDeviceFunction;
+	}
+	static hipError_t launch(hipStream_t st, uint32_t grid, size_t bytes, ColumnsArgs const &C, RedArgs const &red)
 	{
 		MsaArgs const &A = C.A;
-		hipLaunchKernelGGL((k_columns_red<T, E, 4, PK, EW>), dim3(grid), dim3(T), bytes, st, A.msa, A.ld, A.n, A.B, C.lists.L, C.lists.X, C.lists.stride, C.lists.ent, C.lists.hdr,
-		                   A.npass, A.bsh, red);
+		bool launched = false;
+		if constexpr (SWEEP)
+		{
+			if (red.cls)
+			{
+				launched = true;
+				hipLaunchKernelGGL((k_columns_red<T, E, 4, PK, EW, true>), dim3(grid), dim3(T), bytes, st, A.msa, A.ld, A.n, A.B, C.lists.L, C.lists.X, C.lists.stride, C.lists.ent,
+				                   C.lists.hdr, A.npass, A.bsh, red);
+			}
+		}
+		if constexpr (PHASE)
+		{
+			if (!red.cls)
+			{
+				launched = true;
+				hipLaunchKernelGGL((k_columns_red<T, E, 4, PK, EW>), dim3(grid), dim3(T), bytes, st, A.msa, A.ld, A.n, A.B, C.lists.L, C.lists.X, C.lists.stride, C.lists.ent, C.lists.hdr,
+				                   A.npass, A.bsh, red);
+			}
+		}
+		return launched ? hipSuccess : hipErrorInvalidDeviceFunction;
 	}
 	static uint32_t resident(size_t bytes)
 	{
 		int nb = 0;
-		if (hipOccupancyMaxActiveBlocksPerMultiprocessor(&nb, k_columns_red<T, E, 4, PK, EW>, T, bytes) != hipSuccess || nb < 1) nb = 1;
+		if (hipOccupancyMaxActiveBlocksPerMultiprocessor(&nb, k_columns_red<T, E, 4, PK, EW, !PHASE>, T, bytes) != hipSuccess || nb < 1) nb = 1;
 		return (uint32_t) nb;
 	}
-	static ReducedSet make() { return ReducedSet{(uint32_t) T, (uint32_t) E, EW ? (uint32_t) (T - 64) * E : (uint32_t) T * E, (uint32_t) columns_value_cap(T, E, PK), PK, EW, &lds, &prepare, &launch, &resident}; }
+	static ReducedSet make()
+	{
+		return ReducedSet{(uint32_t) T, (uint32_t) E, EW ? (uint32_t) (T - 64) * E : (uint32_t) T * E, (uint32_t) columns_value_cap(T, E, PK), PK, EW, &lds, &lds_sweep, &prepare, &launch, &resident};
+	}
 };
 
 #define FSEQ_RED_CONFIGS(X) \
diff --git a/founder-sequences_amd/csrc/fseq_types.hpp b/founder-sequences_amd/csrc/fseq_types.hpp
--- a/founder-sequences_amd/csrc/fseq_types.hpp
+++ b/founder-sequences_amd/csrc/fseq_types.hpp
@@ -186,7 +186,7 @@
 	uint8_t const *cls_msa = nullptr;
 	size_t cls_ld = 0;
 	uint32_t const *wg_tasks = nullptr;
-	uint32_t *ss_a = nullptr, *ss_d = nullptr;
+	uint16_t *ss_a = nullptr, *ss_d = nullptr;
 	uint32_t ss_stride = 0, ss_cap = 0;
 	unsigned long long const *task_rb = nullptr;
 	uint32_t *cls = nullptr;
diff --git a/include/fseq_debug.h b/include/fseq_debug.h
--- a/include/fseq_debug.h
+++ b/include/fseq_debug.h
@@ -37,6 +37,8 @@
 int  fseq_debug_packed_columns(fseq_ctx *ctx, uint64_t c0, uint64_t c1, uint8_t *out, uint64_t *ld, uint32_t *bits);
 
 int  fseq_debug_pass2_paths(fseq_ctx *ctx, uint32_t *by_runs, uint32_t *by_sort, uint32_t *copies, uint32_t *max_runs, uint32_t *runs_hist);
+
+int  fseq_debug_class_tables(fseq_ctx *ctx, uint64_t const *columns, uint32_t count, uint32_t *cls, uint32_t *headd, uint32_t *ncls);
 
 int  fseq_debug_class_columns(fseq_ctx *ctx, uint32_t *from_classes, uint32_t *from_alignment, uint32_t block, uint32_t *have, uint32_t *nkeys,
                               uint64_t *ldc, uint8_t *out, uint64_t out_bytes);
```
